# AdamCodd/local-hyperDB

Hardware: AMD Instinct MI355X
Metric: queries/sec, N=10M d=384 fp16 top-100 (single-query stream; p50 latency alongside) (higher is better)
Workload: dtype f16; 1 GPU; N=10000000 d=384 fp16 Q=1 cosine_similarity top-100, row-sharded x1; rows_per_gpu=10000000, accumulate=f32, exchange=none

## Files before the change

### local-hyperdb_amd/csrc/hdb_api.hip

```cpp
#include "hdb_common.h"
#include "hdb_quant.h"
#include "hdb_ws.h"
#include "hdb_plan.h"
#include "../../include/hyperdb_hip.h"
#include <string>
#include <cmath>
#include <cstring>
#include <cstdio>
#include <algorithm>
#include <vector>
#include <chrono>
#include <atomic>

static thread_local std::string g_err;
static int fail(int code, const std::string& msg) { g_err = msg; return code; }
#define HIP_TRY(expr)                                                                              \
    do {                                                                                           \
        hipError_t e_ = (expr);                                                                    \
        if (e_ != hipSuccess)                                                                      \
            return fail(HDB_ERR_HIP, std::string(#expr) + ": " + hipGetErrorString(e_));           \
    } while (0)
#define LAUNCH_TRY(expr)                                                                           \
    do {                                                                                           \
        int e_ = (expr);                                                                           \
        if (e_ != 0) return fail(HDB_ERR_HIP, std::string(#expr) + ": " + hipGetErrorString((hipError_t)e_)); \
    } while (0)

struct hdb_index {
    const void* V = nullptr;
    int64_t n = 0;
    int32_t d = 0;
    int dtype = HDB_F32;
    int device = 0;
    int64_t row_base = 0;
    float* inv_norm = nullptr;
    float* sqnorm = nullptr;
    int64_t cache_rows = 0;
    int* nan_flag = nullptr;
    hipStream_t build_stream = nullptr;
    uint32_t* bits = nullptr;
    int64_t bits_npad = 0;
    int W = 0;
    bool bits_valid = false;
    int64_t bits_done = 0;
    float* pscale = nullptr;
    int64_t pscale_rows = 0;
    bool pscale_valid = false;
    int64_t pscale_done = 0;
    const float* bias = nullptr;
    const uint8_t* mask = nullptr;
    const int64_t* rows = nullptr;
    int64_t subset_m = 0;
    float* mbias = nullptr;
    int64_t mbias_rows = 0;
    char* fctl = nullptr;
    uint32_t fused_epoch = 0;
    char* bctl = nullptr;
    char* rec = nullptr;
    size_t rec_bytes = 0;
    int qmode = HDB_QUANT_NONE;
    int8_t* qcodes = nullptr;
    float* qaux = nullptr;
    int64_t q_rows = 0;
    int32_t qP = 0;
    int* qstat = nullptr;
    uint8_t* pnib = nullptr;
    uint32_t* pbit = nullptr;
    float* prec = nullptr;
    int32_t pU = 0;
    bool plane_declined = false;
    bool qauto = false;
    bool qauto_declined = false;
    char* ws = nullptr;
    size_t ws_bytes = 0;
    hdb_options opt;
    int flags_host = -1;
    TopkStats st;
    int64_t st_host_direct = 0;
    const uint32_t* qb_cnt = nullptr;
    int qb_cnt_n = 0;
    int64_t ht_pre_ns = 0, ht_launch_ns = 0, ht_wait_ns = 0, ht_calls = 0;
    std::chrono::steady_clock::time_point ht_l0, ht_l1;
    int64_t ht_attr_ns = 0;
    int64_t profile = 0;
    std::vector<hipEvent_t> ev_pool;
    size_t ev_used = 0;
};

static int ensure_ws(hdb_index* ix, size_t bytes) {
    if (bytes <= ix->ws_bytes) return HDB_OK;
    if (ix->ws) { HIP_TRY(hipDeviceSynchronize()); HIP_TRY(hipFree(ix->ws)); ix->ws = nullptr; ix->ws_bytes = 0; }
    bytes = align_up(bytes + (bytes >> 2), 1 << 20);
    HIP_TRY(hipMalloc((void**)&ix->ws, bytes));
    ix->ws_bytes = bytes;
    return HDB_OK;
}
template <typename WS, typename... Ext>
static int ws_lay(hdb_index* ix, WS& w, Ext... ext) {
    const int rc = ensure_ws(ix, ws_bytes_for<WS>(ext...));
    if (rc) return rc;
    Bump b(ix->ws, ix->ws_bytes);
    w.lay(b, ext...);
    if (b.off > b.cap) return fail(HDB_ERR_NOMEM, "workspace: a layout ran past the size it reported");
    return HDB_OK;
}

extern "C" int hdb_version(void) { return 103; }
extern "C" const char* hdb_last_error(void) { return g_err.c_str(); }

static int build_caches(hdb_index* ix, hipStream_t st) {
    if (ix->n > ix->cache_rows) {
        if (ix->inv_norm) { HIP_TRY(hipDeviceSynchronize()); HIP_TRY(hipFree(ix->inv_norm)); HIP_TRY(hipFree(ix->sqnorm)); }
        const int64_t rows = ix->n + ix->n / 4 + 64;
        HIP_TRY(hipMalloc((void**)&ix->inv_norm, rows * sizeof(float)));
        HIP_TRY(hipMalloc((void**)&ix->sqnorm, rows * sizeof(float)));
        ix->cache_rows = rows;
    }
    HIP_TRY(hipMemsetAsync(ix->nan_flag, 0, sizeof(int), st));
    if (ix->n > 0) LAUNCH_TRY(hdb_launch_rownorm(ix->V, ix->n, ix->d, ix->dtype, ix->inv_norm, ix->sqnorm, ix->nan_flag, st));
    ix->flags_host = -1;
    ix->bits_valid = false; ix->bits_done = 0;
    ix->pscale_valid = false; ix->pscale_done = 0;
    ix->build_stream = st;
    return HDB_OK;
}

static double quant_gamma(int d) {
    const double u = std::ldexp(1.0, -24), m = (double)(d + 8) * u;
    return m / (1.0 - m) * (1.0 + std::ldexp(1.0, -20));
}
static double quant_gamma_m(int d) { return (double)(d + 8) * std::ldexp(1.0, -22); }
static double quant_gamma_rows(int d) { return std::max(quant_gamma(d), quant_gamma_m(d)); }
static size_t quant_elem(const hdb_index* ix) { return (size_t)hdb_elem_bytes(ix->dtype); }
#define HDB_QSTAT_WORDS 4
static hipError_t qstat_alloc(hdb_index* ix, hipStream_t st) {
    if (ix->qstat) return hipSuccess;
    const hipError_t e = hipMalloc((void**)&ix->qstat, HDB_QSTAT_WORDS * sizeof(int));
    if (e != hipSuccess) { ix->qstat = nullptr; return e; }
    return hipMemsetAsync(ix->qstat, 0, HDB_QSTAT_WORDS * sizeof(int), st);
}
static void plane_free(hdb_index* ix) {
    if (ix->pnib) (void)hipFree(ix->pnib);
    if (ix->pbit) (void)hipFree(ix->pbit);
    if (ix->prec) (void)hipFree(ix->prec);
    ix->pnib = nullptr; ix->pbit = nullptr; ix->prec = nullptr;
}
static void quant_free(hdb_index* ix) {
    if (ix->qcodes) (void)hipFree(ix->qcodes);
    if (ix->qaux) (void)hipFree(ix->qaux);
    ix->qcodes = nullptr; ix->qaux = nullptr; ix->q_rows = 0;
    plane_free(ix);
}
static size_t plane_row_bytes(int P) { return (size_t)hdb_quant_plane_units(P) * 20 + 16; }
static bool plane_alloc(hdb_index* ix, int64_t rows, uint8_t** nib, uint32_t** bit, float** rec) {
    const size_t U = (size_t)hdb_quant_plane_units(ix->qP);
    *nib = nullptr; *bit = nullptr; *rec = nullptr;
    if (hipMalloc((void**)nib, (size_t)rows * U * 16) == hipSuccess && hipMalloc((void**)bit, (size_t)rows * U * 4) == hipSuccess &&
        hipMalloc((void**)rec, (size_t)rows * 16) == hipSuccess) return true;
    (void)hipGetLastError();
    if (*nib) (void)hipFree(*nib);
    if (*bit) (void)hipFree(*bit);
    if (*rec) (void)hipFree(*rec);
    *nib = nullptr; *bit = nullptr; *rec = nullptr;
    return false;
}
static int plane_rows(hdb_index* ix, int64_t row0, int64_t m, hipStream_t st) {
    if (!plane_possible(ix->d) || ix->plane_declined) return HDB_OK;
    if (!ix->pnib && !plane_wanted(ix->d, ix->opt)) return HDB_OK;
    if (!ix->pnib) {
        size_t free_b = 0, total_b = 0;
        if (hipMemGetInfo(&free_b, &total_b) != hipSuccess) { (void)hipGetLastError(); ix->plane_declined = true; return HDB_OK; }
        if (free_b < (size_t)ix->q_rows * plane_row_bytes(ix->qP) + ((size_t)1 << 30)) { ix->plane_declined = true; return HDB_OK; }
        if (!plane_alloc(ix, ix->q_rows, &ix->pnib, &ix->pbit, &ix->prec)) { ix->plane_declined = true; return HDB_OK; }
        ix->pU = hdb_quant_plane_units(ix->qP);
        m = row0 + m; row0 = 0;
    }
    LAUNCH_TRY(hdb_launch_quant_plane_rows(ix->qcodes, ix->qaux, row0, m, ix->d, ix->qP, ix->pnib, ix->pbit, ix->prec, st));
    return HDB_OK;
}
static int quant_reserve(hdb_index* ix, int64_t need, int64_t keep, hipStream_t st, bool tight = false) {
    if (need <= ix->q_rows && ix->qcodes) return HDB_OK;
    const int64_t rows = tight ? need + 64 : need + need / 2 + 64;
    int8_t* c2 = nullptr; float* a2 = nullptr;
    HIP_TRY(hipMalloc((void**)&c2, (size_t)rows * ix->qP));
    hipError_t e = hipMalloc((void**)&a2, (size_t)rows * 3 * sizeof(float));
    if (e != hipSuccess) { (void)hipFree(c2); return fail(HDB_ERR_NOMEM, std::string("hdb_index_quantize: ") + hipGetErrorString(e)); }
    if (keep > 0 && ix->qcodes) {
        HIP_TRY(hipMemcpyAsync(c2, ix->qcodes, (size_t)keep * ix->qP, hipMemcpyDeviceToDevice, st));
        HIP_TRY(hipMemcpyAsync(a2, ix->qaux, (size_t)keep * 3 * sizeof(float), hipMemcpyDeviceToDevice, st));
    }
    HIP_TRY(hipStreamSynchronize(st));
    quant_free(ix);
    ix->qcodes = c2; ix->qaux = a2; ix->q_rows = rows;
    return HDB_OK;
}
static int quant_rows(hdb_index* ix, int64_t row0, int64_t m, hipStream_t st) {
    if (m <= 0) return HDB_OK;
    const char* src = (const char*)ix->V + (size_t)row0 * ix->d * quant_elem(ix);
    LAUNCH_TRY(hdb_launch_quant_rows(src, m, ix->d, ix->dtype, ix->qP, ix->qcodes + (size_t)row0 * ix->qP, ix->qaux + (size_t)row0 * 3,
                                     ix->nan_flag, quant_gamma_rows(ix->d), st));
    return plane_rows(ix, row0, m, st);
}

extern "C" int hdb_index_quantize(hdb_index* ix, int mode, void* stream) {
    if (!ix) return fail(HDB_ERR_ARG, "hdb_index_quantize: null index");
    if (mode != HDB_QUANT_NONE && mode != HDB_QUANT_I8) return fail(HDB_ERR_ARG, "hdb_index_quantize: mode must be HDB_QUANT_NONE or HDB_QUANT_I8");
    HIP_TRY(hipSetDevice(ix->device));
    hipStream_t st = (hipStream_t)stream;
    if (mode == HDB_QUANT_NONE) {
        if (ix->qcodes) HIP_TRY(hipStreamSynchronize(st));
        quant_free(ix);
        ix->qmode = HDB_QUANT_NONE;
        ix->qauto = false;
        ix->opt.auto_quant = 0;
        return HDB_OK;
    }
    if (ix->dtype == HDB_BF16) return fail(HDB_ERR_UNSUPPORTED, "hdb_index_quantize: bfloat16 (bf16) matrices have no int8 shadow");
    if (ix->dtype != HDB_F16 && ix->dtype != HDB_F32) return fail(HDB_ERR_UNSUPPORTED, "hdb_index_quantize: only float16 / float32 matrices have an int8 shadow");
    HIP_TRY(qstat_alloc(ix, st));
    ix->qP = (int32_t)align_up((size_t)ix->d, 16);
    ix->plane_declined = false;
    int rc = quant_reserve(ix, std::max<int64_t>(ix->n, 1), 0, st);
    if (rc) return rc;
    rc = quant_rows(ix, 0, ix->n, st);
    if (rc) return rc;
    ix->qmode = HDB_QUANT_I8;
    ix->qauto = false;
    ix->build_stream = st;
    return HDB_OK;
}

static bool quant_auto_build(hdb_index* ix, size_t ws_need, hipStream_t st) {
    if (ix->qauto_declined) return false;
    const int32_t P = (int32_t)align_up((size_t)ix->d, 16);
    const size_t shadow = (size_t)(ix->n + 64) * ((size_t)P + 12);
    size_t free_b = 0, total_b = 0;
    if (hipMemGetInfo(&free_b, &total_b) != hipSuccess) { (void)hipGetLastError(); ix->qauto_declined = true; return false; }
    const size_t ws_grow = ws_need > ix->ws_bytes ? ws_need + (ws_need >> 2) + ((size_t)1 << 20) : 0;
    if (free_b < shadow + ws_grow + ((size_t)1 << 30)) { ix->qauto_declined = true; return false; }
    const size_t plane = plane_possible(ix->d) ? (size_t)(ix->n + 64) * plane_row_bytes(P) : 0;
    ix->plane_declined = plane_wanted(ix->d, ix->opt) && free_b < shadow + plane + ws_grow + ((size_t)1 << 30);
    if (qstat_alloc(ix, st) != hipSuccess && !ix->qstat) { (void)hipGetLastError(); ix->qauto_declined = true; return false; }
    ix->qP = P;
    if (quant_reserve(ix, std::max<int64_t>(ix->n, 1), 0, st, true) != HDB_OK || quant_rows(ix, 0, ix->n, st) != HDB_OK) {
        (void)hipGetLastError();
        quant_free(ix);
        ix->qauto_declined = true;
        return false;
    }
    ix->qmode = HDB_QUANT_I8;
    ix->qauto = true;
    return true;
}

extern "C" int hdb_index_create(hdb_index** out, const void* dev_V, int64_t n, int32_t d, int dtype, int device,
                                int64_t row_base, void* stream) {
    if (!out) return fail(HDB_ERR_ARG, "hdb_index_create: out is null");
    if (n < 0 || d <= 0) return fail(HDB_ERR_ARG, "hdb_index_create: need n >= 0 and d > 0");
    if (n > 0 && !dev_V) return fail(HDB_ERR_ARG, "hdb_index_create: matrix pointer is null");
    if (dtype != HDB_F16 && dtype != HDB_F32 && dtype != HDB_F64 && dtype != HDB_BF16) return fail(HDB_ERR_ARG, "hdb_index_create: dtype must be f16/f32/f64/bf16");
    if (n >= ((int64_t)1 << 32) - 1) return fail(HDB_ERR_ARG, "hdb_index_create: at most 2^32-2 rows per shard");
    if ((int64_t)d * 8 > 60 * 1024) return fail(HDB_ERR_ARG, "hdb_index_create: d too large for the query LDS tile");
    HIP_TRY(hipSetDevice(device));
    hdb_index* ix = new hdb_index();
    ix->V = dev_V; ix->n = n; ix->d = d; ix->dtype = dtype; ix->device = device; ix->row_base = row_base;
    hipError_t e = hipMalloc((void**)&ix->nan_flag, sizeof(int));
    if (e != hipSuccess) { delete ix; return fail(HDB_ERR_HIP, std::string("hipMalloc: ") + hipGetErrorString(e)); }
    int rc = build_caches(ix, (hipStream_t)stream);
    if (rc != HDB_OK) { hdb_index_destroy(ix); return rc; }
    *out = ix;
    return HDB_OK;
}

extern "C" int hdb_index_update(hdb_index* ix, const void* dev_V, int64_t n, void* stream) {
    if (!ix) return fail(HDB_ERR_ARG, "hdb_index_update: null index");
    if (n < 0 || (n > 0 && !dev_V)) return fail(HDB_ERR_ARG, "hdb_index_update: bad matrix");
    if (n >= ((int64_t)1 << 32) - 1) return fail(HDB_ERR_ARG, "hdb_index_update: at most 2^32-2 rows per shard");
    HIP_TRY(hipSetDevice(ix->device));
    ix->V = dev_V; ix->n = n;
    ix->bias = nullptr; ix->mask = nullptr; ix->rows = nullptr; ix->subset_m = 0;
    ix->qauto_declined = false;
    ix->plane_declined = false;
    int rc = build_caches(ix, (hipStream_t)stream);
    if (rc == HDB_OK && ix->qmode == HDB_QUANT_I8) {
        rc = quant_reserve(ix, std::max<int64_t>(n, 1), 0, (hipStream_t)stream);
        if (rc == HDB_OK) rc = quant_rows(ix, 0, n, (hipStream_t)stream);
    }
    return rc;
}

extern "C" int hdb_index_rebase(hdb_index* ix, const void* dev_V) {
    if (!ix) return fail(HDB_ERR_ARG, "hdb_index_rebase: null index");
    if (ix->n > 0 && !dev_V) return fail(HDB_ERR_ARG, "hdb_index_rebase: matrix pointer is null");
    ix->V = dev_V;
    return HDB_OK;
}

extern "C" int hdb_index_set_row_base(hdb_index* ix, int64_t row_base) {
    if (!ix) return fail(HDB_ERR_ARG, "hdb_index_set_row_base: null index");
    if (row_base < 0) return fail(HDB_ERR_ARG, "hdb_index_set_row_base: row_base must be >= 0");
    ix->row_base = row_base;
    return HDB_OK;
}

extern "C" int hdb_index_extend(hdb_index* ix, int64_t new_n, void* stream) {
    if (!ix) return fail(HDB_ERR_ARG, "hdb_index_extend: null index");
    if (new_n < ix->n) return fail(HDB_ERR_ARG, "hdb_index_extend: new_n must not shrink the matrix (use hdb_index_update)");
    if (new_n >= ((int64_t)1 << 32) - 1) return fail(HDB_ERR_ARG, "hdb_index_extend: at most 2^32-2 rows per shard");
    if (new_n == ix->n) return HDB_OK;
    if (!ix->V) return fail(HDB_ERR_ARG, "hdb_index_extend: no matrix registered");
    HIP_TRY(hipSetDevice(ix->device));
    hipStream_t st = (hipStream_t)stream;
    const int64_t old_n = ix->n;
    if (new_n > ix->cache_rows) {
        const int64_t rows = new_n + new_n / 2 + 64;
        float *inv2 = nullptr, *sq2 = nullptr;
        HIP_TRY(hipMalloc((void**)&inv2, rows * sizeof(float)));
        HIP_TRY(hipMalloc((void**)&sq2, rows * sizeof(float)));
        if (old_n > 0) {
            HIP_TRY(hipMemcpyAsync(inv2, ix->inv_norm, old_n * sizeof(float), hipMemcpyDeviceToDevice, st));
            HIP_TRY(hipMemcpyAsync(sq2, ix->sqnorm, old_n * sizeof(float), hipMemcpyDeviceToDevice, st));
        }
        HIP_TRY(hipStreamSynchronize(st));
        if (ix->inv_norm) { HIP_TRY(hipFree(ix->inv_norm)); HIP_TRY(hipFree(ix->sqnorm)); }
        ix->inv_norm = inv2; ix->sqnorm = sq2; ix->cache_rows = rows;
    }
    const size_t elem = (size_t)hdb_elem_bytes(ix->dtype);
    const char* tail = (const char*)ix->V + (size_t)old_n * ix->d * elem;
    LAUNCH_TRY(hdb_launch_rownorm(tail, new_n - old_n, ix->d, ix->dtype, ix->inv_norm + old_n, ix->sqnorm + old_n, ix->nan_flag, st));
    ix->n = new_n;
    if (ix->qmode == HDB_QUANT_I8) {
        int rc = quant_reserve(ix, new_n, old_n, st);
        if (rc == HDB_OK) rc = quant_rows(ix, old_n, new_n - old_n, st);
        if (rc) return rc;
    }
    ix->flags_host = -1;
    ix->bits_valid = false;
    ix->pscale_valid = false;
    ix->bias = nullptr; ix->mask = nullptr;
    ix->rows = nullptr; ix->subset_m = 0;
    ix->build_stream = st;
    return HDB_OK;
}

extern "C" int hdb_index_gather(hdb_index* ix, const int64_t* dev_rows, int64_t m, void* dev_V_out, void* stream) {
    if (!ix) return fail(HDB_ERR_ARG, "hdb_index_gather: null index");
    if (m < 0 || m > ix->n) return fail(HDB_ERR_ARG, "hdb_index_gather: m must be in [0, n]");
    if (m > 0 && (!dev_rows || !dev_V_out)) return fail(HDB_ERR_ARG, "hdb_index_gather: null argument");
    if (m > 0 && dev_V_out == ix->V) return fail(HDB_ERR_ARG, "hdb_index_gather: the gather is out of place");
    HIP_TRY(hipSetDevice(ix->device));
    hipStream_t st = (hipStream_t)stream;
    const size_t elem = (size_t)hdb_elem_bytes(ix->dtype);
    float *inv2 = nullptr, *sq2 = nullptr;
    const int64_t rows = m + m / 4 + 64;
    HIP_TRY(hipMalloc((void**)&inv2, rows * sizeof(float)));
    HIP_TRY(hipMalloc((void**)&sq2, rows * sizeof(float)));
    HIP_TRY(hipMemsetAsync(ix->nan_flag, 0, sizeof(int), st));
    int rc = hdb_launch_gather_rows(ix->V, dev_rows, m, (int)(ix->d * elem), dev_V_out, ix->inv_norm, ix->sqnorm, inv2, sq2,
                                    ix->nan_flag, st);
    int8_t* qc2 = nullptr; float* qa2 = nullptr;
    if (rc == 0 && ix->qmode == HDB_QUANT_I8) {
        rc = (int)hipMalloc((void**)&qc2, (size_t)rows * ix->qP);
        if (rc == 0) rc = (int)hipMalloc((void**)&qa2, (size_t)rows * 3 * sizeof(float));
        if (rc == 0) rc = hdb_launch_quant_gather(ix->qcodes, ix->qaux, dev_rows, m, ix->qP, qc2, qa2, st);
    }
    if (rc == 0) rc = (int)hipStreamSynchronize(st);
    if (rc != 0) {
        (void)hipFree(inv2); (void)hipFree(sq2);
        if (qc2) (void)hipFree(qc2);
        if (qa2) (void)hipFree(qa2);
        return fail(HDB_ERR_HIP, std::string("hdb_index_gather: ") + hipGetErrorString((hipError_t)rc));
    }
    if (ix->qmode == HDB_QUANT_I8) { quant_free(ix); ix->qcodes = qc2; ix->qaux = qa2; ix->q_rows = rows; }
    if (ix->inv_norm) { (void)hipFree(ix->inv_norm); (void)hipFree(ix->sqnorm); }
    ix->inv_norm = inv2; ix->sqnorm = sq2; ix->cache_rows = rows;
    ix->V = dev_V_out; ix->n = m;
    if (ix->qmode == HDB_QUANT_I8) {
        const int rcp = plane_rows(ix, 0, m, st);
        if (rcp != HDB_OK) return rcp;
    }
    ix->flags_host = -1;
    ix->bits_valid = false; ix->pscale_valid = false; ix->bits_done = 0; ix->pscale_done = 0;
    ix->bias = nullptr; ix->mask = nullptr; ix->rows = nullptr; ix->subset_m = 0;
    ix->build_stream = st;
    return HDB_OK;
}

extern "C" void hdb_index_destroy(hdb_index* ix) {
    if (!ix) return;
    (void)hipSetDevice(ix->device);
    (void)hipDeviceSynchronize();
    if (ix->inv_norm) (void)hipFree(ix->inv_norm);
    if (ix->sqnorm) (void)hipFree(ix->sqnorm);
    if (ix->nan_flag) (void)hipFree(ix->nan_flag);
    if (ix->bits) (void)hipFree(ix->bits);
    if (ix->pscale) (void)hipFree(ix->pscale);
    if (ix->mbias) (void)hipFree(ix->mbias);
    if (ix->fctl) (void)hipFree(ix->fctl);
    if (ix->bctl) (void)hipFree(ix->bctl);
    if (ix->ws) (void)hipFree(ix->ws);
    if (ix->rec) (void)hipFree(ix->rec);
    quant_free(ix);
    if (ix->qstat) (void)hipFree(ix->qstat);
    for (hipEvent_t e : ix->ev_pool) (void)hipEventDestroy(e);
    delete ix;
}

extern "C" int hdb_index_has_nan(hdb_index* ix, int* out_flag) {
    if (!ix || !out_flag) return fail(HDB_ERR_ARG, "hdb_index_has_nan: null argument");
    HIP_TRY(hipSetDevice(ix->device));
    int h = 0;
    HIP_TRY(hipMemcpyAsync(&h, ix->nan_flag, sizeof(int), hipMemcpyDeviceToHost, ix->build_stream));
    HIP_TRY(hipStreamSynchronize(ix->build_stream));
    ix->flags_host = h;
    *out_flag = h & 1;
    return HDB_OK;
}
static int matrix_is_finite(hdb_index* ix, bool* out) {
    if (ix->flags_host < 0) { int f = 0; int rc = hdb_index_has_nan(ix, &f); if (rc != HDB_OK) return rc; }
    *out = ix->flags_host == 0;
    return HDB_OK;
}

extern "C" int hdb_index_set_bias(hdb_index* ix, const float* dev_bias) {
    if (!ix) return fail(HDB_ERR_ARG, "hdb_index_set_bias: null index");
    ix->bias = dev_bias;
    return HDB_OK;
}

extern "C" int hdb_index_set_row_mask(hdb_index* ix, const uint8_t* dev_mask) {
    if (!ix) return fail(HDB_ERR_ARG, "hdb_index_set_row_mask: null index");
    ix->mask = dev_mask;
    ix->rows = nullptr; ix->subset_m = 0;
    return HDB_OK;
}

extern "C" int hdb_index_set_row_subset(hdb_index* ix, const uint8_t* dev_mask, const int64_t* dev_rows, int64_t m) {
    if (!ix) return fail(HDB_ERR_ARG, "hdb_index_set_row_subset: null index");
    if (dev_rows && !dev_mask) return fail(HDB_ERR_ARG, "hdb_index_set_row_subset: a row list needs its mask");
    if (dev_rows && (m < 1 || m > ix->n)) return fail(HDB_ERR_ARG, "hdb_index_set_row_subset: m must be in [1, n]");
    ix->mask = dev_mask;
    ix->rows = dev_rows; ix->subset_m = dev_rows ? m : 0;
    return HDB_OK;
}

extern "C" int hdb_set_option(hdb_index* ix, const char* name, int64_t value) {
    if (!ix || !name) return fail(HDB_ERR_ARG, "hdb_set_option: null argument");
    if (!strcmp(name, "max_blocks")) ix->opt.max_blocks = value;
    else if (!strcmp(name, "force_exact")) ix->opt.force_exact = value;
    else if (!strcmp(name, "sample_target")) ix->opt.sample_target = value;
    else if (!strcmp(name, "mfma_min_q")) ix->opt.mfma_min_q = value;
    else if (!strcmp(name, "use_mfma")) ix->opt.use_mfma = value;
    else if (!strcmp(name, "exact_bytes")) ix->opt.exact_bytes = std::max<int64_t>(1 << 20, value);
    else if (!strcmp(name, "finalize_threads")) { if (value == 256 || value == 512 || value == 1024) ix->opt.finalize_threads = value; }
    else if (!strcmp(name, "mfma_variant")) { if (value == 16 || value == 32 || value == 64) ix->opt.mfma_variant = value; }
    else if (!strcmp(name, "host_direct")) ix->opt.host_direct = value;
    else if (!strcmp(name, "use_fused")) ix->opt.use_fused = value;
    else if (!strcmp(name, "use_batch1")) ix->opt.use_batch1 = value;
    else if (!strcmp(name, "use_local")) ix->opt.use_local = value;
    else if (!strcmp(name, "local_max_q")) ix->opt.local_max_q = value;
    else if (!strcmp(name, "local_max_tiles")) ix->opt.local_max_tiles = std::max<int64_t>(1, value);
    else if (!strcmp(name, "local_small")) ix->opt.local_small = value;
    else if (!strcmp(name, "local_m")) ix->opt.local_m = std::max<int64_t>(0, std::min<int64_t>(value, 64));
    else if (!strcmp(name, "use_l1_tile")) ix->opt.use_l1_tile = value;
    else if (!strcmp(name, "l1_packed")) ix->opt.l1_packed = value;
    else if (!strcmp(name, "host_poll")) ix->opt.host_poll = value;
    else if (!strcmp(name, "dyn_tiles")) ix->opt.dyn_tiles = value;
    else if (!strcmp(name, "dyn_min_mb")) ix->opt.dyn_min_mb = std::max<int64_t>(0, value);
    else if (!strcmp(name, "dyn_heavy")) ix->opt.dyn_heavy = value;
    else if (!strcmp(name, "fused_timeout_us")) ix->opt.fused_timeout_us = std::max<int64_t>(1, value);
    else if (!strcmp(name, "bits_fused")) ix->opt.bits_fused = value;
    else if (!strcmp(name, "bits_local")) ix->opt.bits_local = value;
    else if (!strcmp(name, "fused_max_q")) ix->opt.fused_max_q = value;
    else if (!strcmp(name, "f32_min_q")) ix->opt.f32_min_q = value;
    else if (!strcmp(name, "f32_split")) ix->opt.f32_split = value;
    else if (!strcmp(name, "f32_split_min_q")) ix->opt.f32_split_min_q = value;
    else if (!strcmp(name, "bf16_ks_min_q")) ix->opt.bf16_ks_min_q = value;
    else if (!strcmp(name, "bits_max_q")) ix->opt.bits_max_q = value;
    else if (!strcmp(name, "use_quant")) ix->opt.use_quant = value;
    else if (!strcmp(name, "quant_min_n")) ix->opt.quant_min_n = value;
    else if (!strcmp(name, "auto_quant")) ix->opt.auto_quant = value;
    else if (!strcmp(name, "quant_batch_min_n")) ix->opt.quant_batch_min_n = value;
    else if (!strcmp(name, "quant_batch_kernel")) ix->opt.quant_batch_kernel = value ? 1 : 0;
    else if (!strcmp(name, "quant_max_k")) ix->opt.quant_max_k = std::max<int64_t>(1, std::min<int64_t>(value, 128));
    else if (!strcmp(name, "use_plane")) ix->opt.use_plane = value;
    else if (!strcmp(name, "plane_min_n")) ix->opt.plane_min_n = value;
    else if (!strcmp(name, "plane_cap_rows")) ix->opt.plane_cap_rows = std::max<int64_t>(0, value);
    else if (!strcmp(name, "use_subset")) ix->opt.use_subset = value;
    else if (!strcmp(name, "subset_min_n")) ix->opt.subset_min_n = value < 0 ? -1 : value;
    else if (!strcmp(name, "subset_ratio")) ix->opt.subset_ratio = value < 0 ? -1 : std::max<int64_t>(1, value);
    else if (!strcmp(name, "profile")) { ix->profile = value; ix->ev_used = 0; }
    else if (!strcmp(name, "host_timing_reset")) { ix->ht_pre_ns = ix->ht_launch_ns = ix->ht_wait_ns = ix->ht_calls = ix->ht_attr_ns = 0; }
    else return fail(HDB_ERR_ARG, std::string("hdb_set_option: unknown option ") + name);
    return HDB_OK;
}

extern "C" int hdb_get_stat(hdb_index* ix, const char* name, int64_t* value) {
    if (!ix || !name || !value) return fail(HDB_ERR_ARG, "hdb_get_stat: null argument");
    if (!strcmp(name, "sample_rows")) *value = ix->st.sample_rows;
    else if (!strcmp(name, "sample_m")) *value = ix->st.sample_m;
    else if (!strcmp(name, "path")) *value = ix->st.path;
    else if (!strcmp(name, "chunks")) *value = ix->st.chunks;
    else if (!strcmp(name, "mfma")) *value = ix->st.mfma;
    else if (!strcmp(name, "f32_split")) *value = ix->st.f32s;
    else if (!strcmp(name, "host_direct")) *value = ix->st_host_direct;
    else if (!strcmp(name, "fused")) *value = ix->st.fused;
    else if (!strcmp(name, "local")) *value = ix->st.local;
    else if (!strcmp(name, "cand_cap")) *value = HDB_CAND_CAP;
    else if (!strcmp(name, "quant")) *value = ix->st.quant;
    else if (!strcmp(name, "quant_auto")) *value = (ix->qmode == HDB_QUANT_I8 && ix->qauto) ? 1 : 0;
    else if (!strcmp(name, "quant_bytes")) *value = ix->qmode == HDB_QUANT_I8 ? ix->n * (int64_t)(ix->qP + 12) : 0;
    else if (!strcmp(name, "plane")) *value = ix->st.plane;
    else if (!strcmp(name, "subset")) *value = ix->st.subset;
    else if (!strcmp(name, "subset_rows")) *value = ix->subset_m;
    else if (!strcmp(name, "plane_bytes")) *value = (ix->qmode == HDB_QUANT_I8 && ix->pnib) ? ix->n * (int64_t)plane_row_bytes(ix->qP) : 0;
    else if (!strcmp(name, "plane_survivors") || !strcmp(name, "plane_overflows")) {
        int h[HDB_QSTAT_WORDS] = {0, 0, 0, 0};
        if (ix->qstat) {
            HIP_TRY(hipSetDevice(ix->device));
            HIP_TRY(hipDeviceSynchronize());
            HIP_TRY(hipMemcpy(h, ix->qstat, sizeof(h), hipMemcpyDeviceToHost));
        }
        *value = name[6] == 's' ? (ix->st.plane ? (int64_t)(uint32_t)h[1] : 0) : (int64_t)(uint32_t)h[2];
    }
    else if (!strcmp(name, "quant_cands")) {
        int h = 0;
        if (ix->st.quant && ix->qstat) {
            HIP_TRY(hipSetDevice(ix->device));
            HIP_TRY(hipDeviceSynchronize());
            HIP_TRY(hipMemcpy(&h, ix->qstat, sizeof(int), hipMemcpyDeviceToHost));
        }
        *value = h;
    }
    else if (!strcmp(name, "quant_cands_min") || !strcmp(name, "quant_cands_median")) {
        int64_t v = 0;
        if (ix->st.quant && ix->qb_cnt && ix->qb_cnt_n > 0) {
            HIP_TRY(hipSetDevice(ix->device));
            HIP_TRY(hipDeviceSynchronize());
            std::vector<uint32_t> raw((size_t)ix->qb_cnt_n * HDB_CNT_STRIDE), c((size_t)ix->qb_cnt_n);
            HIP_TRY(hipMemcpy(raw.data(), ix->qb_cnt, raw.size() * sizeof(uint32_t), hipMemcpyDeviceToHost));
            for (int q = 0; q < ix->qb_cnt_n; ++q) c[q] = raw[(size_t)q * HDB_CNT_STRIDE];
            std::sort(c.begin(), c.end());
            v = name[13] == 'i' ? c.front() : c[c.size() / 2];
        }
        *value = v;
    }
    else if (!strcmp(name, "n")) *value = ix->n;
    else if (!strcmp(name, "ws_bytes")) *value = (int64_t)ix->ws_bytes;
    else if (!strcmp(name, "scan_launches")) *value = (int64_t)(ix->ev_used / 2);
    else if (!strcmp(name, "host_pre_ns")) *value = ix->ht_pre_ns;
    else if (!strcmp(name, "host_launch_ns")) *value = ix->ht_launch_ns;
    else if (!strcmp(name, "host_wait_ns")) *value = ix->ht_wait_ns;
    else if (!strcmp(name, "host_calls")) *value = ix->ht_calls;
    else if (!strcmp(name, "host_attr_ns")) *value = ix->ht_attr_ns;
    else if (!strcmp(name, "scan_time_ns")) {
        double total_ms = 0.0;
        for (size_t i = 0; i + 1 < ix->ev_used; i += 2) {
            if (hipEventSynchronize(ix->ev_pool[i + 1]) != hipSuccess) return fail(HDB_ERR_HIP, "hipEventSynchronize failed");
            float ms = 0.f;
            if (hipEventElapsedTime(&ms, ix->ev_pool[i], ix->ev_pool[i + 1]) != hipSuccess) return fail(HDB_ERR_HIP, "hipEventElapsedTime failed");
            total_ms += ms;
        }
        *value = (int64_t)(total_ms * 1.0e6);
    }
    else return fail(HDB_ERR_ARG, std::string("hdb_get_stat: unknown stat ") + name);
    return HDB_OK;
}

static void prof_begin(hdb_index* ix, hipStream_t st) {
    if (!ix->profile) return;
    if (ix->ev_used + 2 > ix->ev_pool.size()) {
        if (ix->ev_pool.size() >= 16384) return;
        for (int i = 0; i < 2; ++i) { hipEvent_t e; if (hipEventCreate(&e) != hipSuccess) return; ix->ev_pool.push_back(e); }
    }
    (void)hipEventRecord(ix->ev_pool[ix->ev_used], st);
}
static void prof_end(hdb_index* ix, hipStream_t st) {
    if (!ix->profile || ix->ev_used + 2 > ix->ev_pool.size()) return;
    (void)hipEventRecord(ix->ev_pool[ix->ev_used + 1], st);
    ix->ev_used += 2;
}

static bool metric_ok(int metric) { return metric >= HDB_DOT && metric <= HDB_EUCLIDEAN_DIST; }

static int ensure_pscale(hdb_index* ix, hipStream_t st) {
    if (ix->pscale_valid) return HDB_OK;
    const size_t elem = (size_t)hdb_elem_bytes(ix->dtype);
    int64_t keep = ix->pscale ? std::min(ix->pscale_done, ix->n) : 0;
    if (ix->n > ix->pscale_rows) {
        const int64_t rows = ix->n + ix->n / 4 + 64;
        float* p2 = nullptr;
        HIP_TRY(hipMalloc((void**)&p2, rows * sizeof(float)));
        if (keep > 0) HIP_TRY(hipMemcpyAsync(p2, ix->pscale, keep * sizeof(float), hipMemcpyDeviceToDevice, st));
        if (ix->pscale) { HIP_TRY(hipDeviceSynchronize()); HIP_TRY(hipFree(ix->pscale)); }
        ix->pscale = p2; ix->pscale_rows = rows;
    }
    if (ix->n > keep)
        LAUNCH_TRY(hdb_launch_rowstats((const char*)ix->V + (size_t)keep * ix->d * elem, ix->n - keep, ix->d, ix->dtype, ix->pscale + keep, st));
    ix->pscale_done = ix->n;
    ix->pscale_valid = true;
    return HDB_OK;
}

static int ensure_bits(hdb_index* ix, hipStream_t st) {
    if (ix->bits_valid) return HDB_OK;
    const int W = (ix->d + 31) / 32;
    if (W > 512) return fail(HDB_ERR_UNSUPPORTED, "hamming: d > 16384 not supported");
    const size_t elem = (size_t)hdb_elem_bytes(ix->dtype);
    const int64_t npad = align_up((size_t)std::max<int64_t>(ix->n, 4), 256);
    int64_t keep = (ix->bits && ix->W == W) ? std::min(ix->bits_done, ix->n) : 0;
    if (!ix->bits || ix->bits_npad < npad || ix->W != W) {
        const int64_t cap = align_up((size_t)(npad + npad / 4), 256);
        uint32_t* b2 = nullptr;
        HIP_TRY(hipMalloc((void**)&b2, (size_t)cap * W * sizeof(uint32_t)));
        HIP_TRY(hipMemsetAsync(b2, 0, (size_t)cap * W * sizeof(uint32_t), st));
        if (keep > 0) HIP_TRY(hipMemcpyAsync(b2, ix->bits, (size_t)align_up((size_t)keep, 256) * W * sizeof(uint32_t), hipMemcpyDeviceToDevice, st));
        if (ix->bits) { HIP_TRY(hipDeviceSynchronize()); HIP_TRY(hipFree(ix->bits)); }
        ix->bits = b2; ix->bits_npad = cap; ix->W = W;
    } else if (keep == 0) {
        HIP_TRY(hipMemsetAsync(ix->bits, 0, (size_t)ix->bits_npad * W * sizeof(uint32_t), st));
    }
    if (ix->n > keep)
        LAUNCH_TRY(hdb_launch_signpack((const char*)ix->V + (size_t)keep * ix->d * elem, ix->n - keep, ix->d, ix->dtype, keep, ix->bits, st));
    ix->bits_done = ix->n;
    ix->bits_valid = true;
    return HDB_OK;
}

static void base_args(const hdb_index* ix, ScanArgs& a, const void* Q, int metric) {
    memset(&a, 0, sizeof(a));
    a.V = ix->V; a.n = ix->n; a.d = ix->d; a.Q = Q; a.metric = metric;
    a.inv_norm = ix->inv_norm; a.mask = ix->mask;
    a.tile_stride = 1; a.ntiles = (ix->n + 15) / 16;
    a.cap = HDB_CAND_CAP;
    a.dyn_min_bytes = ix->opt.dyn_min_mb << 20; a.dyn_heavy = (int32_t)ix->opt.dyn_heavy;
}

struct QueryBufs { const float* qinv; const float* qsq; const uint32_t* qbits; const void* q16; const float* qscl; };
static int run_scan(hdb_index* ix, ScanArgs& a, int mode, int cq, const QueryBufs& qb, bool l1tile, bool mfma, hipStream_t st) {
    a.qinv = qb.qinv;
    if (is_bits_metric(a.metric)) {
        LAUNCH_TRY(hdb_launch_hamming(&a, mode, cq, ix->bits, ix->bits_npad, ix->W, qb.qbits, st));
    } else if (l1tile && cq >= 2 && a.tile_stride == 1) {
        ScanArgs al = a; al.dyn_heavy = ix->opt.l1_packed ? 0 : 77;
        LAUNCH_TRY(hdb_launch_l1_tile(&al, ix->dtype, mode, cq, (int)ix->opt.max_blocks, st));
    } else if (mfma) {
        LAUNCH_TRY(hdb_launch_mfma_scan(&a, ix->dtype, mode, cq, qb.q16, ix->sqnorm, qb.qsq, qb.qscl, (int)ix->opt.max_blocks, (int)ix->opt.mfma_variant, st, nullptr));
    } else {
        LAUNCH_TRY(hdb_launch_scan(&a, ix->dtype, mode, cq, (int)ix->opt.max_blocks, st));
    }
    return HDB_OK;
}

extern "C" int hdb_scores(hdb_index* ix, const void* dev_q, int metric, float* dev_out, void* stream) {
    if (!ix || !dev_q || !dev_out) return fail(HDB_ERR_ARG, "hdb_scores: null argument");
    if (!metric_ok(metric)) return fail(HDB_ERR_UNSUPPORTED, "hdb_scores: metric not built");
    if (ix->n == 0) return HDB_OK;
    HIP_TRY(hipSetDevice(ix->device));
    hipStream_t st = (hipStream_t)stream;
    const int W = (ix->d + 31) / 32;
    ScoresWs w;
    int rc = ws_lay(ix, w, ix->d, W);
    if (rc) return rc;
    float* qinv = w.qinv; float* qsq = w.qsq; int* qnan = w.qnan; uint32_t* qbits = w.qbits; void* qc = w.qc;
    LAUNCH_TRY(hdb_launch_qprep(dev_q, 1, ix->d, ix->dtype == HDB_F64, qinv, qsq, qnan, nullptr, nullptr, st));
    if (is_bits_metric(metric)) {
        rc = ensure_bits(ix, st); if (rc) return rc;
        LAUNCH_TRY(hdb_launch_qsign(dev_q, 1, ix->d, ix->dtype == HDB_F64, W, qbits, st));
    }
    ScanArgs a; base_args(ix, a, dev_q, metric);
    if (metric == HDB_PEARSON) {
        rc = ensure_pscale(ix, st); if (rc) return rc;
        LAUNCH_TRY(hdb_launch_qcentre(dev_q, 1, ix->d, ix->dtype == HDB_F64, qc, qinv, st));
        a.Q = qc; a.metric = HDB_COSINE; a.inv_norm = ix->pscale;
    }
    a.mask = nullptr;
    a.raw = 1;
    a.scores = dev_out; a.ld = ix->n;
    QueryBufs qb{qinv, qsq, qbits, nullptr, nullptr};
    return run_scan(ix, a, 0, 1, qb, false, false, st);
}

struct TopkArgs { const void* Q; int32_t nq, k; int metric; int64_t* idx; float* score; int32_t* status; hipStream_t st; };
static TopkFacts topk_facts(const hdb_index* ix) {
    return {ix->n, ix->d, ix->dtype, ix->qmode, ix->qauto, ix->qauto_declined, ix->pnib != nullptr, ix->plane_declined,
            ix->mask != nullptr, ix->bias != nullptr, hdb_cu_count(), ix->subset_m};
}

static int quant_pitch(const hdb_index* ix) { return (int)align_up((size_t)ix->d, 16); }
static size_t quant_ws_bytes(const hdb_index* ix, int nq, uint32_t pl_cap, bool mflavour) {
    return ws_bytes_for<QuantWs>(nq, quant_pitch(ix), (int)ix->d, quant_ld_max(ix->n, ix->d), pl_cap, mflavour);
}
static int quant_ws_lay(hdb_index* ix, QuantWs& w, int nq, uint32_t pl_cap, bool mflavour) {
    return ws_lay(ix, w, nq, quant_pitch(ix), (int)ix->d, quant_ld_max(ix->n, ix->d), pl_cap, mflavour);
}
static size_t quant_batch_ws_bytes(const hdb_index* ix, int cq) {
    return ws_bytes_for<QuantBatchWs>(cq, quant_pitch(ix), (int)ix->d, quant_batch_sample(ix->n).ld_s, quant_batch_wld());
}
static int quant_batch_ws_lay(hdb_index* ix, QuantBatchWs& w, int cq) {
    return ws_lay(ix, w, cq, quant_pitch(ix), (int)ix->d, quant_batch_sample(ix->n).ld_s, quant_batch_wld());
}
static void quant_base_args(const hdb_index* ix, QuantArgs& a, const int8_t* qcodes, const float* qaux, const float* qinv, int metric, int nq) {
    memset(&a, 0, sizeof(a));
    a.codes = ix->qcodes; a.n = ix->n; a.d = ix->d; a.P = ix->qP; a.aux = ix->qaux; a.sqnorm = ix->sqnorm; a.inv_norm = ix->inv_norm;
    a.qcodes = qcodes; a.qaux = qaux; a.qinv = qinv; a.bias = ix->bias; a.mask = ix->mask; a.metric = metric; a.nq = nq;
    a.gamma = (float)quant_gamma(ix->d);
}
static int quant_query_prep(hdb_index* ix, const float* Q, int nq, const QuantWs& w, bool mflavour, int* stat, uint32_t* cnt_init,
                            uint32_t* pl_cnt, hipStream_t st) {
    if (mflavour) {
        LAUNCH_TRY(hdb_launch_quant_qprep_m(Q, nq, ix->d, ix->qP, w.qinv, w.qsq, w.qnan, w.q16, w.qscl, w.qcodes, w.qaux, stat, cnt_init, pl_cnt, st));
    } else {
        LAUNCH_TRY(hdb_launch_qprep(Q, nq, ix->d, false, w.qinv, w.qsq, w.qnan, nullptr, nullptr, st));
        LAUNCH_TRY(hdb_launch_quant_qprep(Q, nq, ix->d, ix->qP, w.qcodes, w.qaux, stat, pl_cnt, st));
    }
    return HDB_OK;
}

static int shadow_prepare(hdb_index* ix, const TopkPlan& p, int nq, hipStream_t st, bool* declined) {
    if (p.build_needed) {
        const size_t ws_need = p.path == HDB_PATH_QUANT ? quant_ws_bytes(ix, nq, 0, true) : quant_batch_ws_bytes(ix, p.cq_max);
        if (!quant_auto_build(ix, ws_need, st)) { *declined = true; return HDB_OK; }
    }
    if (p.plane_wanted && !ix->pnib) {
        const int rc = plane_rows(ix, 0, ix->n, st);
        if (rc) return rc;
        *declined = ix->pnib == nullptr;
    }
    return HDB_OK;
}

static int quant_topk(hdb_index* ix, const TopkArgs& c, const TopkPlan& p) {
    const void* dev_Q = c.Q; const int32_t nq = c.nq, k = c.k; const int metric = c.metric; hipStream_t st = c.st;
    int64_t* dev_idx = c.idx; float* dev_score = c.score; int32_t* dev_status = c.status;
    const uint32_t kk = p.kk; const bool mflavour = p.mflavour, use_pl = p.plane_wanted;
    const int64_t n = ix->n;
    const uint32_t m = 16;
    const QuantSample sp = p.qs;
    QuantWs w;
    int rc = quant_ws_lay(ix, w, nq, (nq == 1 && ix->pnib) ? p.pl_cap : 0, mflavour);
    if (rc) return rc;
    const uint32_t pl_cap = p.pl_cap;
    uint32_t* pl_cnt = use_pl ? reinterpret_cast<uint32_t*>(ix->qstat) + 1 : nullptr;
    const size_t crow = (size_t)nq * HDB_CAND_CAP;
    const int nsub = p.nsub;
    rc = quant_query_prep(ix, (const float*)dev_Q, nq, w, mflavour, ix->qstat, nsub ? w.cnt : nullptr, pl_cnt, st);
    if (rc) return rc;
    QuantArgs a; quant_base_args(ix, a, w.qcodes, w.qaux, w.qinv, metric, nq);
    a.ntiles = sp.s_tiles; a.tile_stride = sp.s_stride; a.scores = w.sbuf; a.ld = sp.ld_s;
    a.wmax = w.wmax; a.nsub = nsub; a.thr_out = w.thr;
    LAUNCH_TRY(hdb_launch_quant_scan(&a, 0, (int)ix->opt.max_blocks, st));
    if (!nsub) LAUNCH_TRY(hdb_launch_sample_thr(w.sbuf, sp.s_rows, sp.ld_s, nq, m, w.thr, w.cnt, nullptr, st));
    a.ntiles = (n + 15) / 16; a.tile_stride = 1; a.scores = nullptr; a.ld = 0;
    a.thr = w.thr; a.cnt = w.cnt; a.cand = w.cand; a.cap = HDB_CAND_CAP;
    prof_begin(ix, st);
    if (use_pl) {
        a.pl_nib = ix->pnib; a.pl_bit = ix->pbit; a.pl_rec = ix->prec; a.pl_units = ix->pU;
        a.pl_list = w.pl_list; a.pl_cnt = pl_cnt; a.pl_cap = pl_cap;
        LAUNCH_TRY(hdb_launch_quant_plane_scan(&a, 0, (int)ix->opt.max_blocks, st));
        a.nsub = 0; a.wmax = nullptr;
        LAUNCH_TRY(hdb_launch_quant_scan_one(&a, 1, (int)ix->opt.max_blocks, st));
    } else {
        LAUNCH_TRY(hdb_launch_quant_scan(&a, 1, (int)ix->opt.max_blocks, st));
    }
    prof_end(ix, st);
    if (mflavour) {
        const bool has_bias = ix->bias != nullptr || ix->mask != nullptr;
        LAUNCH_TRY(hdb_launch_quant_cgather(ix->V, ix->d * 2, ix->inv_norm, ix->bias, ix->mask, w.cand, w.cnt, HDB_CAND_CAP, nq, w.G,
                                            metric == HDB_COSINE ? w.ginv : nullptr, has_bias ? w.gbias : nullptr, st));
        ScanArgs s; memset(&s, 0, sizeof(s));
        s.V = w.G; s.n = (int64_t)crow; s.d = ix->d; s.Q = dev_Q; s.metric = metric; s.inv_norm = w.ginv; s.qinv = w.qinv;
        s.bias = has_bias ? w.gbias : nullptr; s.mask = nullptr; s.nq = nq;
        s.tile_stride = 1; s.ntiles = (int64_t)crow / hdb_mfma_tile_rows(ix->dtype, ix->d); s.cap = HDB_CAND_CAP;
        s.scores = w.gsc; s.ld = (int64_t)crow;
        LAUNCH_TRY(hdb_launch_mfma_scan(&s, ix->dtype, 0, nq, w.q16, w.ginv, w.qsq, w.qscl, (int)ix->opt.max_blocks, (int)ix->opt.mfma_variant, st, nullptr));
    } else {
        LAUNCH_TRY(hdb_launch_quant_rescore(ix->V, ix->d, ix->dtype, (const float*)dev_Q, nq, metric, ix->inv_norm, w.qinv, ix->bias, ix->mask,
                                            w.cand, w.cnt, HDB_CAND_CAP, st));
    }
    LAUNCH_TRY(hdb_launch_quant_finalize(w.cand, w.cnt, HDB_CAND_CAP, nq, (uint32_t)k, kk, ix->row_base, dev_idx, dev_score, dev_status, w.qnan,
                                         w.qaux, w.thr, ix->qstat, mflavour ? w.cand : nullptr, w.gsc, (int64_t)crow, st));
    return HDB_OK;
}

extern "C" int hdb_debug_quant_bounds(hdb_index* ix, const float* dev_q, int metric, float* dev_hi, float* dev_hi5, void* stream) {
    if (!ix || !dev_q || !dev_hi || !dev_hi5) return fail(HDB_ERR_ARG, "hdb_debug_quant_bounds: null argument");
    if (metric != HDB_DOT && metric != HDB_COSINE) return fail(HDB_ERR_ARG, "hdb_debug_quant_bounds: dot or cosine");
    if (ix->qmode != HDB_QUANT_I8 || !ix->pnib || ix->n < 1) return fail(HDB_ERR_UNSUPPORTED, "hdb_debug_quant_bounds: the index has no 5-bit plane");
    HIP_TRY(hipSetDevice(ix->device));
    hipStream_t st = (hipStream_t)stream;
    QuantWs w;
    int rc = quant_ws_lay(ix, w, 1, plane_list_cap(ix->opt, ix->n), true);
    if (rc) return rc;
    rc = quant_query_prep(ix, dev_q, 1, w, ix->qauto, nullptr, nullptr, nullptr, st);
    if (rc) return rc;
    QuantArgs a; quant_base_args(ix, a, w.qcodes, w.qaux, w.qinv, metric, 1);
    a.ntiles = (ix->n + 15) / 16; a.tile_stride = 1;
    a.pl_nib = ix->pnib; a.pl_bit = ix->pbit; a.pl_rec = ix->prec; a.pl_units = ix->pU;
    a.dbg = dev_hi;
    LAUNCH_TRY(hdb_launch_quant_scan_one(&a, 2, (int)ix->opt.max_blocks, st));
    a.dbg = dev_hi5;
    LAUNCH_TRY(hdb_launch_quant_plane_scan(&a, 1, (int)ix->opt.max_blocks, st));
    return HDB_OK;
}

static int quant_batch_topk(hdb_index* ix, const TopkArgs& c, const TopkPlan& p) {
    const void* dev_Q = c.Q; const int32_t nq = c.nq, k = c.k; const int metric = c.metric; hipStream_t st = c.st;
    int64_t* dev_idx = c.idx; float* dev_score = c.score; int32_t* dev_status = c.status;
    const uint32_t kk = p.kk;
    const int64_t n = ix->n;
    const int P = ix->qP;
    const uint32_t m = HDB_QB_SAMPLE_M;
    const QuantSample sp = p.qs;
    const int64_t s_tiles = sp.s_tiles, s_stride = sp.s_stride, s_rows = sp.s_rows, ld_s = sp.ld_s;
    const int cq_max = p.cq_max;
    QuantBatchWs w;
    const int rc = quant_batch_ws_lay(ix, w, cq_max);
    if (rc) return rc;
    const int64_t wld = quant_batch_wld();
    float* const qinv = w.qinv; float* const qsq = w.qsq; int* const qnan = w.qnan; float* const qscl = w.qscl;
    int8_t* const qcodes = w.qcodes; float* const qaux = w.qaux; float* const thr = w.thr; uint32_t* const cnt = w.cnt;
    unsigned long long* const cand = w.cand; void* const q16 = w.q16; float* const wbuf = w.wbuf;
    for (int q0 = 0; q0 < nq; q0 += cq_max) {
        const int cq = std::min(cq_max, nq - q0);
        const float* Qc = (const float*)dev_Q + (size_t)q0 * ix->d;
        LAUNCH_TRY(hdb_launch_quant_qprep_m(Qc, cq, ix->d, P, qinv, qsq, qnan, q16, qscl, qcodes, qaux, q0 == 0 ? ix->qstat : nullptr, cnt, nullptr, st));
        QuantArgs a; quant_base_args(ix, a, qcodes, qaux, qinv, metric, cq);
        a.thr = thr; a.cnt = cnt; a.cand = cand; a.cap = HDB_CAND_CAP;
        if (p.qb_int8) {
            a.ntiles = s_tiles; a.tile_stride = s_stride;
            const int sblocks = hdb_qb_scan_blocks(s_tiles, cq, hdb_cu_count(), (int)ix->opt.max_blocks);
            LAUNCH_TRY(hdb_launch_qb_scan(&a, 0, wbuf, wld, (int)ix->opt.max_blocks, st));
            LAUNCH_TRY(hdb_launch_qb_thr(wbuf, hdb_qb_slots(sblocks, cq), wld, cq, m, thr, st));
            a.ntiles = (n + 15) / 16; a.tile_stride = 1;
            prof_begin(ix, st);
            LAUNCH_TRY(hdb_launch_qb_scan(&a, 1, nullptr, 0, (int)ix->opt.max_blocks, st));
            prof_end(ix, st);
        } else {
            for (int g0 = 0; g0 < cq; g0 += 4) {
                QuantArgs g = a;
                g.nq = std::min(4, cq - g0);
                g.qcodes = qcodes + (size_t)g0 * P; g.qaux = qaux + (size_t)g0 * HDB_QQ_WORDS; g.qinv = qinv + g0;
                g.thr = thr + g0; g.cnt = cnt + (size_t)g0 * HDB_CNT_STRIDE; g.cand = cand + (size_t)g0 * HDB_CAND_CAP;
                g.ntiles = s_tiles; g.tile_stride = s_stride; g.scores = wbuf; g.ld = ld_s;
                LAUNCH_TRY(hdb_launch_quant_scan(&g, 0, (int)ix->opt.max_blocks, st));
                LAUNCH_TRY(hdb_launch_qb_thr(wbuf, s_rows, ld_s, g.nq, m, thr + g0, st));
                g.ntiles = (n + 15) / 16; g.tile_stride = 1; g.scores = nullptr; g.ld = 0;
                prof_begin(ix, st);
                LAUNCH_TRY(hdb_launch_quant_scan(&g, 1, (int)ix->opt.max_blocks, st));
                prof_end(ix, st);
            }
        }
        LAUNCH_TRY(hdb_launch_qb_rescore(ix->V, ix->d, q16, qscl, qinv, ix->inv_norm, ix->bias, ix->mask, metric, cand, cnt, HDB_CAND_CAP, cq, st));
        LAUNCH_TRY(hdb_launch_quant_finalize(cand, cnt, HDB_CAND_CAP, cq, (uint32_t)k, kk, ix->row_base, dev_idx + (int64_t)q0 * k,
                                             dev_score + (int64_t)q0 * k, dev_status + q0, qnan, qaux, thr, ix->qstat, nullptr, nullptr, 0, st));
    }
    ix->qb_cnt = cnt; ix->qb_cnt_n = nq - (nq - 1) / cq_max * cq_max;
    return HDB_OK;
}

static uint32_t next_epoch(hdb_index* ix) {
    ix->fused_epoch = (ix->fused_epoch + 1) & 0x7FFFFFFFu;
    if (ix->fused_epoch == 0) ix->fused_epoch = 1;
    return ix->fused_epoch;
}
static uint32_t timeout_ticks(const hdb_index* ix) { return (uint32_t)std::min<int64_t>(ix->opt.fused_timeout_us * 100, 0x7FFFFFFF); }
static int ensure_ctl(char** ctl, size_t bytes) {
    if (*ctl) return HDB_OK;
    HIP_TRY(hipMalloc((void**)ctl, bytes));
    HIP_TRY(hipMemset(*ctl, 0, bytes));
    return HDB_OK;
}

static int run_empty(const TopkArgs& c) {
    HIP_TRY(hipMemsetAsync(c.idx, 0xFF, (size_t)c.nq * c.k * sizeof(int64_t), c.st));
    HIP_TRY(hipMemsetAsync(c.score, 0xFF, (size_t)c.nq * c.k * sizeof(float), c.st));
    if (c.status) HIP_TRY(hipMemsetAsync(c.status, 0, (size_t)c.nq * sizeof(int32_t), c.st));
    return HDB_OK;
}

struct TopkEnv {
    TopkWs w; size_t sort_temp;
    const void* Qeff; int metric_eff;
    const float* bias_eff; const uint8_t* mask_eff;
};
static int topk_begin(hdb_index* ix, const TopkArgs& c, const TopkPlan& p, TopkEnv& e) {
    hipStream_t st = c.st;
    const bool f64 = ix->dtype == HDB_F64;
    const int64_t n = ix->n;
    e.sort_temp = 0;
    if (p.sort_n > 0) LAUNCH_TRY(hdb_sort_temp_bytes(p.sort_n, &e.sort_temp));
    TopkWs& w = e.w;
    int rc = ws_lay(ix, w, (int)c.nq, (int)ix->d, p.W, p.cq_max, p.ld_scores, p.ld_ks, p.sort_n, e.sort_temp);
    if (rc) return rc;
    if (p.prep)
        LAUNCH_TRY(hdb_launch_qprep2(c.Q, c.nq, ix->d, f64, w.qinv, w.qsq, w.qnan, p.q16_in_prep ? w.q16 : nullptr, w.qscl, p.fold_small ? w.thr : nullptr,
                                     p.fold_small ? w.cnt : nullptr, (p.fold_small && p.bits) ? w.qbits : nullptr, p.W, st));
    if (p.bits) {
        rc = ensure_bits(ix, st); if (rc) return rc;
        if (p.prep && !p.fold_small) LAUNCH_TRY(hdb_launch_qsign(c.Q, c.nq, ix->d, f64, p.W, w.qbits, st));
    }
    e.Qeff = c.Q; e.metric_eff = c.metric;
    if (p.pearson) {
        rc = ensure_pscale(ix, st); if (rc) return rc;
        if (p.prep) LAUNCH_TRY(hdb_launch_qcentre(c.Q, c.nq, ix->d, f64, w.qc, w.qinv, st));
        e.Qeff = w.qc; e.metric_eff = HDB_COSINE;
    }
    e.bias_eff = ix->bias; e.mask_eff = ix->mask;
    if (p.mask_fold) {
        if (n > ix->mbias_rows) {
            if (ix->mbias) { HIP_TRY(hipDeviceSynchronize()); HIP_TRY(hipFree(ix->mbias)); ix->mbias = nullptr; }
            const int64_t rows = n + n / 4 + 64;
            HIP_TRY(hipMalloc((void**)&ix->mbias, rows * sizeof(float)));
            ix->mbias_rows = rows;
        }
        LAUNCH_TRY(hdb_launch_maskbias(ix->mask, ix->bias, n, ix->mbias, st));
        e.bias_eff = ix->mbias; e.mask_eff = nullptr;
    }
    return HDB_OK;
}

static int run_full_sort(hdb_index* ix, const TopkArgs& c, const TopkPlan& p) {
    TopkEnv e;
    int rc = topk_begin(ix, c, p, e); if (rc) return rc;
    for (int q0 = 0; q0 < c.nq; ++q0) {
        QueryBufs qb{e.w.qinv, e.w.qsq, e.w.qbits, nullptr, nullptr};
        ScanArgs s2; base_args(ix, s2, e.Qeff, e.metric_eff);
        if (p.pearson) s2.inv_norm = ix->pscale;
        s2.q0 = q0; s2.bias = ix->bias; s2.scores = e.w.sc1; s2.ld = p.ld_n;
        rc = run_scan(ix, s2, 0, 1, qb, false, false, c.st); if (rc) return rc;
        LAUNCH_TRY(hdb_launch_full_sort(e.w.sc1, ix->n, c.k, ix->row_base, e.w.work, e.w.temp, e.sort_temp, c.idx + (int64_t)q0 * c.k,
                                        c.score + (int64_t)q0 * c.k, c.st));
    }
    if (c.status) LAUNCH_TRY(hdb_launch_status_nan(e.w.qnan, c.nq, c.status, c.st));
    return HDB_OK;
}

static int run_fused(hdb_index* ix, const TopkArgs& c, const TopkPlan& p) {
    TopkEnv e;
    int rc = topk_begin(ix, c, p, e); if (rc) return rc;
    rc = ensure_ctl(&ix->fctl, hdb_mfma_fused_ctl_bytes()); if (rc) return rc;
    ScanArgs a; base_args(ix, a, c.Q, c.metric);
    a.bias = e.bias_eff; a.mask = nullptr;
    if (c.metric == HDB_EUCLIDEAN) a.inv_norm = ix->sqnorm;
    if (p.pearson) a.inv_norm = ix->pscale;
    a.ntiles = (ix->n + p.tile_rows - 1) / p.tile_rows;
    a.thr = e.w.thr; a.cnt = e.w.cnt; a.cand = e.w.cand; a.nq = c.nq;
    FusedArgs fa; memset(&fa, 0, sizeof(fa));
    fa.Qraw = static_cast<const float*>(c.Q); fa.nq = c.nq;
    fa.s_tiles = p.s_tiles; fa.s_stride = p.s_stride;
    fa.epoch = next_epoch(ix);
    fa.timeout_ticks = timeout_ticks(ix);
    fa.ctl = reinterpret_cast<uint32_t*>(ix->fctl);
    fa.cand = e.w.cand; fa.cap = HDB_CAND_CAP; fa.k = (uint32_t)c.k; fa.kk = p.kk; fa.row_base = ix->row_base;
    fa.idx_out = c.idx; fa.score_out = c.score; fa.status = c.status; fa.thr_out = e.w.thr;
    fa.local = p.local ? 1 : 0; fa.local_slot = p.local_slot; fa.local_m = p.local_m;
    prof_begin(ix, c.st);
    ix->ht_l0 = std::chrono::steady_clock::now();
    LAUNCH_TRY(hdb_launch_mfma_fused(&a, ix->dtype, &fa, (int)ix->opt.max_blocks, c.st));
    ix->ht_l1 = std::chrono::steady_clock::now();
    prof_end(ix, c.st);
    return HDB_OK;
}

static int run_bits1(hdb_index* ix, const TopkArgs& c, const TopkPlan& p) {
    TopkEnv e;
    int rc = topk_begin(ix, c, p, e); if (rc) return rc;
    rc = ensure_ctl(&ix->bctl, hdb_mfma_batch_ctl_bytes(hdb_cu_count())); if (rc) return rc;
    for (int q0 = 0; q0 < c.nq; q0 += 4) {
        const int cq = std::min(4, c.nq - q0);
        BitsArgs ba; memset(&ba, 0, sizeof(ba));
        ba.bits = ix->bits; ba.npad = ix->bits_npad; ba.W = p.W; ba.n = ix->n; ba.d = ix->d;
        ba.Qraw = static_cast<const float*>(c.Q) + (size_t)q0 * ix->d; ba.nq = cq;
        ba.ntiles = (ix->n + 15) / 16; ba.s_tiles = p.s_tiles; ba.s_stride = p.s_stride;
        ba.bias = ix->bias; ba.mask = ix->mask;
        ba.local = p.bits_local;
        ba.epoch = next_epoch(ix);
        ba.timeout_ticks = timeout_ticks(ix);
        ba.ctl = reinterpret_cast<uint32_t*>(ix->bctl);
        ba.cand = e.w.cand; ba.cap = HDB_CAND_CAP; ba.k = (uint32_t)c.k; ba.kk = p.kk; ba.row_base = ix->row_base;
        ba.idx_out = c.idx + (int64_t)q0 * c.k; ba.score_out = c.score + (int64_t)q0 * c.k; ba.status = c.status + q0;
        prof_begin(ix, c.st);
        ix->ht_l0 = std::chrono::steady_clock::now();
        LAUNCH_TRY(hdb_launch_bits_fused(&ba, c.metric == HDB_JACCARD ? 1 : 0, (int)ix->opt.max_blocks, c.st));
        ix->ht_l1 = std::chrono::steady_clock::now();
        prof_end(ix, c.st);
    }
    return HDB_OK;
}

static int run_batch1(hdb_index* ix, const TopkArgs& c, const TopkPlan& p) {
    TopkEnv e;
    int rc = topk_begin(ix, c, p, e); if (rc) return rc;
    rc = ensure_ctl(&ix->bctl, hdb_mfma_batch_ctl_bytes(hdb_cu_count())); if (rc) return rc;
    const size_t qrow = (size_t)ix->d * 4;
    for (int q0 = 0; q0 < c.nq; q0 += p.cq_max) {
        const int cq = std::min(p.cq_max, c.nq - q0);
        ScanArgs a; base_args(ix, a, c.Q, e.metric_eff);
        if (p.pearson) a.inv_norm = ix->pscale;
        a.bias = e.bias_eff; a.mask = nullptr; a.q0 = 0; a.nq = cq; a.f32_split = p.f32s ? 1 : 0;
        a.ntiles = (ix->n + p.tile_rows - 1) / p.tile_rows;
        a.cand = e.w.cand;
        a.tile_ctr = ix->opt.dyn_tiles ? reinterpret_cast<uint32_t*>(ix->bctl) + HDB_BATCH_CTL_TILE : nullptr;
        BatchArgs fa; memset(&fa, 0, sizeof(fa));
        fa.Qraw = static_cast<const char*>(c.Q) + (size_t)q0 * qrow;
        fa.s_tiles = p.s_tiles; fa.s_stride = p.s_stride; fa.centre = p.pearson ? 1 : 0;
        fa.epoch = next_epoch(ix);
        fa.timeout_ticks = timeout_ticks(ix);
        fa.ctl = reinterpret_cast<uint32_t*>(ix->bctl);
        fa.k = (uint32_t)c.k; fa.kk = p.kk; fa.row_base = ix->row_base;
        fa.idx_out = c.idx + (int64_t)q0 * c.k; fa.score_out = c.score + (int64_t)q0 * c.k; fa.status = c.status + q0;
        prof_begin(ix, c.st);
        ix->ht_l0 = std::chrono::steady_clock::now();
        LAUNCH_TRY(hdb_launch_mfma_scan(&a, ix->dtype, 2, cq, nullptr, ix->sqnorm, nullptr, nullptr, (int)ix->opt.max_blocks, (int)ix->opt.mfma_variant, c.st, &fa));
        ix->ht_l1 = std::chrono::steady_clock::now();
        prof_end(ix, c.st);
    }
    return HDB_OK;
}

static int run_pipeline(hdb_index* ix, const TopkArgs& c, const TopkPlan& p) {
    TopkEnv e;
    int rc = topk_begin(ix, c, p, e); if (rc) return rc;
    const void* dev_Q = c.Q; const int32_t nq = c.nq, k = c.k; const int metric = c.metric; hipStream_t st = c.st;
    int64_t* dev_idx = c.idx; float* dev_score = c.score; int32_t* dev_status = c.status;
    const TopkWs& w = e.w;
    float* const qinv = w.qinv; float* const qsq = w.qsq; int* const qnan = w.qnan; float* const qscl = w.qscl;
    uint32_t* const qbits = w.qbits; void* const q16 = w.q16;
    float* const thr = w.thr; uint32_t* const cnt = w.cnt; uint32_t* const tile_ctr = w.tile_ctr; uint32_t* const hist = w.hist;
    uint32_t* const tie_info = w.tie_info; unsigned long long* const cand = w.cand; float* const sbuf = w.sbuf; float* const kbuf = w.kbuf;
    const void* Qeff = e.Qeff; const int metric_eff = e.metric_eff; const float* bias_eff = e.bias_eff; const uint8_t* mask_eff = e.mask_eff;
    const bool small = p.small, exact = p.exact, mfma = p.mfma, f32s = p.f32s, fold_small = p.fold_small, f16_queries = p.f16_queries, is_pearson = p.pearson, q16_in_prep = p.q16_in_prep;
    const int64_t n = p.subset ? ix->subset_m : ix->n, s_tiles = p.s_tiles, s_stride = p.s_stride, s_rows = p.s_rows, ld_s = p.ld_s, ld_n = p.ld_n;
    const uint32_t kk = p.kk, m = p.m; const int cq_max = p.cq_max, tile_rows = p.tile_rows, npass = p.npass;
    bool q16_ready = q16_in_prep;
    for (int q0 = 0; q0 < nq; q0 += cq_max) {
        const int cq = std::min(cq_max, nq - q0);
        if (f16_queries && !q16_ready) { LAUNCH_TRY(hdb_launch_q_to_f16((const float*)Qeff, nq, ix->d, q16, qscl, st)); q16_ready = true; }
        QueryBufs qb{qinv, qsq, qbits, f16_queries ? q16 : Qeff, f16_queries ? qscl : nullptr};
        ScanArgs a; base_args(ix, a, Qeff, metric_eff);
        if (is_pearson) a.inv_norm = ix->pscale;
        a.q0 = q0; a.bias = bias_eff; a.mask = mask_eff; a.f32_split = f32s ? 1 : 0;
        a.thr = thr; a.cnt = cnt; a.cand = cand;
        a.ntiles = (n + tile_rows - 1) / tile_rows;
        if (p.subset) { a.rows = ix->rows; a.m = ix->subset_m; a.mask = nullptr; a.bias = ix->bias; }
        a.ks_partial_out = kbuf; a.ks_ld = ld_n;

        if (small) {
            if (!fold_small) LAUNCH_TRY(hdb_launch_fill_thr(thr, cnt, cq, -INFINITY, st));
            rc = run_scan(ix, a, 1, cq, qb, p.l1tile, mfma, st); if (rc) return rc;
        } else if (!exact) {
            ScanArgs s = a;
            s.ntiles = s_tiles; s.tile_stride = s_stride; s.scores = sbuf; s.ld = ld_s;
            rc = run_scan(ix, s, 0, cq, qb, p.l1tile, mfma, st); if (rc) return rc;
            if (m <= 16) {
                LAUNCH_TRY(hdb_launch_sample_thr(sbuf, s_rows, ld_s, cq, m, thr, cnt, tile_ctr, st));
                if (mfma && ix->opt.dyn_tiles) a.tile_ctr = tile_ctr;
            } else {
                HIP_TRY(hipMemsetAsync(hist, 0, (size_t)cq * 4 * HDB_RADIX_BINS * 4, st));
                for (int ps = 0; ps < 4; ++ps) LAUNCH_TRY(hdb_launch_hist(sbuf, s_rows, ld_s, cq, hist, ps, m, st));
                LAUNCH_TRY(hdb_launch_thr(hist, cq, 4, m, (uint32_t)s_rows, thr, cnt, st));
            }
            prof_begin(ix, st);
            rc = run_scan(ix, a, 1, cq, qb, p.l1tile, mfma, st); if (rc) return rc;
            prof_end(ix, st);
        } else {
            ScanArgs s = a;
            s.scores = sbuf; s.ld = ld_n;
            prof_begin(ix, st);
            rc = run_scan(ix, s, 0, cq, qb, p.l1tile, mfma, st); if (rc) return rc;
            prof_end(ix, st);
            HIP_TRY(hipMemsetAsync(cnt, 0, (size_t)((char*)hist - (char*)cnt) + (size_t)cq * 4 * HDB_RADIX_BINS * 4, st));
            for (int ps = 0; ps < npass; ++ps) LAUNCH_TRY(hdb_launch_hist(sbuf, n, ld_n, cq, hist, ps, kk, st));
            LAUNCH_TRY(hdb_launch_collect(sbuf, n, ld_n, cq, hist, npass, kk, cnt, cand, HDB_CAND_CAP, tie_info, st));
            if (p.subset) LAUNCH_TRY(hdb_launch_list_rows(cand, cnt, HDB_CAND_CAP, cq, ix->rows, ix->subset_m, st));
        }
        if (mfma && metric == HDB_EUCLIDEAN)
            LAUNCH_TRY(hdb_launch_rescore_euclid(cand, cnt, HDB_CAND_CAP, cq, ix->V, ix->dtype, ix->d, (const float*)dev_Q, qsq, q0, ix->bias, st));
        LAUNCH_TRY(hdb_launch_finalize(cand, cnt, HDB_CAND_CAP, cq, (uint32_t)k, kk, ix->row_base,
                                       dev_idx + (int64_t)q0 * k, dev_score + (int64_t)q0 * k,
                                       dev_status ? dev_status + q0 : nullptr, qnan + q0, (int)ix->opt.finalize_threads,
                                       a.f32_split ? HDB_Q_UNDERFLOW : 0, st));
    }
    return HDB_OK;
}

static int topk_impl(hdb_index* ix, const void* dev_Q, int32_t nq, int32_t k, int metric, int64_t* dev_idx,
                     float* dev_score, int32_t* dev_status, void* stream, bool exact) {
    if (!ix || !dev_idx || !dev_score) return fail(HDB_ERR_ARG, "hdb_topk: null argument");
    if (nq < 0 || k < 0) return fail(HDB_ERR_ARG, "hdb_topk: nq and k must be >= 0");
    if (nq == 0 || k == 0) return HDB_OK;
    if (!dev_Q) return fail(HDB_ERR_ARG, "hdb_topk: query pointer is null");
    if (metric == HDB_EUCLIDEAN_DIST || !metric_ok(metric)) return fail(HDB_ERR_UNSUPPORTED, "hdb_topk: metric not built");
    if (metric == HDB_PEARSON && ix->d < 1) return fail(HDB_ERR_ARG, "hdb_topk: pearson needs d >= 1");
    HIP_TRY(hipSetDevice(ix->device));
    const TopkArgs c{dev_Q, nq, k, metric, dev_idx, dev_score, dev_status, (hipStream_t)stream};
    const TopkCall call{nq, k, metric, dev_status != nullptr, exact};
    int frc = HDB_OK;
    auto finite = [&] { bool f = false; if (frc == HDB_OK) frc = matrix_is_finite(ix, &f); return f; };
    TopkPlan p = plan_topk(topk_facts(ix), ix->opt, call, finite);
    if (frc != HDB_OK) return frc;
    if (p.shadow()) {
        bool declined = false;
        const int rc = shadow_prepare(ix, p, nq, c.st, &declined);
        if (rc) return rc;
        if (declined) p = plan_topk(topk_facts(ix), ix->opt, call, finite);
        if (frc != HDB_OK) return frc;
    }
    ix->st = p.stats;
    ix->qb_cnt = nullptr; ix->qb_cnt_n = 0;
    switch (p.path) {
    case HDB_PATH_EMPTY: return run_empty(c);
    case HDB_PATH_QUANT: return quant_topk(ix, c, p);
    case HDB_PATH_QUANT_BATCH: return quant_batch_topk(ix, c, p);
    case HDB_PATH_FUSED: return run_fused(ix, c, p);
    case HDB_PATH_BITS1: return run_bits1(ix, c, p);
    case HDB_PATH_BATCH1: return run_batch1(ix, c, p);
    case HDB_PATH_FULL_SORT: return run_full_sort(ix, c, p);
    case HDB_PATH_PIPELINE: return run_pipeline(ix, c, p);
    }
    return fail(HDB_ERR_ARG, "hdb_topk: no path");
}

extern "C" int hdb_topk(hdb_index* ix, const void* dev_Q, int32_t nq, int32_t k, int metric, int64_t* dev_idx,
                        float* dev_score, int32_t* dev_status, void* stream) {
    return topk_impl(ix, dev_Q, nq, k, metric, dev_idx, dev_score, dev_status, stream, false);
}

static void merge_host_records(const char* const* recs, int32_t parts, int32_t nq, int32_t k, void* out_record) {
    int64_t* oi = reinterpret_cast<int64_t*>(out_record);
    float* os = reinterpret_cast<float*>(static_cast<char*>(out_record) + (int64_t)nq * k * 8);
    int32_t* ost = reinterpret_cast<int32_t*>(static_cast<char*>(out_record) + (int64_t)nq * k * 12);
    std::vector<int32_t> pos((size_t)parts);
    for (int32_t q = 0; q < nq; ++q) {
        int32_t st = 0;
        for (int32_t p = 0; p < parts; ++p) {
            st |= reinterpret_cast<const int32_t*>(recs[p] + (int64_t)nq * k * 12)[q];
            pos[p] = 0;
        }
        for (int32_t i = 0; i < k; ++i) {
            int32_t best = -1; int64_t bi = -1; float bs = 0.f;
            for (int32_t p = 0; p < parts; ++p) {
                if (pos[p] >= k) continue;
                const int64_t ci = reinterpret_cast<const int64_t*>(recs[p])[(int64_t)q * k + pos[p]];
                if (ci < 0) { pos[p] = k; continue; }
                const float cs = reinterpret_cast<const float*>(recs[p] + (int64_t)nq * k * 8)[(int64_t)q * k + pos[p]];
                if (best < 0 || cs > bs || (cs == bs && ci < bi)) { best = p; bi = ci; bs = cs; }
            }
            if (best < 0) { oi[(int64_t)q * k + i] = -1; os[(int64_t)q * k + i] = -INFINITY; }
            else { oi[(int64_t)q * k + i] = bi; os[(int64_t)q * k + i] = bs; ++pos[best]; }
        }
        ost[q] = st;
    }
}

extern "C" int hdb_merge_topk_host(const void* records, int32_t parts, int32_t nq, int32_t k, void* out_record) {
    if (!records || !out_record || parts <= 0 || nq < 0 || k < 0) return fail(HDB_ERR_ARG, "hdb_merge_topk_host: bad argument");
    const int64_t nb = hdb_packed_bytes(nq, k);
    std::vector<const char*> recs((size_t)parts);
    for (int32_t p = 0; p < parts; ++p) recs[p] = static_cast<const char*>(records) + p * nb;
    merge_host_records(recs.data(), parts, nq, k, out_record);
    return HDB_OK;
}

extern "C" int hdb_host_exchange_merge(void* shm, int64_t stride, int32_t world, int32_t rank, uint64_t seq, const void* record,
                                       int32_t nq, int32_t k, void* out_record, double timeout_s) {
    if (!shm || !record || !out_record || world <= 0 || rank < 0 || rank >= world || stride < 64 || nq < 0 || k < 0)
        return fail(HDB_ERR_ARG, "hdb_host_exchange_merge: bad argument");
    const int64_t nb = hdb_packed_bytes(nq, k);
    if (nb + 64 > stride) return fail(HDB_ERR_ARG, "hdb_host_exchange_merge: record larger than a slot");
    char* base = static_cast<char*>(shm) + (int64_t)(seq & 1) * world * stride;
    char* mine = base + (int64_t)rank * stride;
    memcpy(mine + 64, record, (size_t)nb);
    __atomic_store_n(reinterpret_cast<uint64_t*>(mine), seq, __ATOMIC_RELEASE);
    std::vector<const char*> recs((size_t)world);
    const auto t0 = std::chrono::steady_clock::now();
    for (int32_t r = 0; r < world; ++r) {
        const uint64_t* sp = reinterpret_cast<const uint64_t*>(base + (int64_t)r * stride);
        uint32_t spins = 0;
        while (__atomic_load_n(sp, __ATOMIC_ACQUIRE) != seq) {
            __builtin_ia32_pause();
            if ((++spins & 0xFFFFu) == 0 &&
                std::chrono::duration<double>(std::chrono::steady_clock::now() - t0).count() > timeout_s)
                return fail(HDB_ERR_HIP, "hdb_host_exchange_merge: a rank did not publish its record in time");
        }
        recs[r] = base + (int64_t)r * stride + 64;
    }
    merge_host_records(recs.data(), world, nq, k, out_record);
    return HDB_OK;
}

extern "C" int hdb_topk_host(hdb_index* ix, const void* dev_Q, int32_t nq, int32_t k, int metric, void* host_record, void* stream) {
    if (!ix || !host_record) return fail(HDB_ERR_ARG, "hdb_topk_host: null argument");
    if (nq <= 0 || k <= 0) return fail(HDB_ERR_ARG, "hdb_topk_host: nq and k must be positive");
    const auto ht0 = std::chrono::steady_clock::now();
    HIP_TRY(hipSetDevice(ix->device));
    hipStream_t st = (hipStream_t)stream;
    const size_t bytes = (size_t)hdb_packed_bytes(nq, k);
    bool direct = false;
    if (ix->opt.host_direct) {
        hipPointerAttribute_t attr;
        if (hipPointerGetAttributes(&attr, host_record) == hipSuccess) direct = attr.type == hipMemoryTypeHost && attr.devicePointer == host_record;
        else (void)hipGetLastError();
        ix->ht_attr_ns += std::chrono::duration_cast<std::chrono::nanoseconds>(std::chrono::steady_clock::now() - ht0).count();
    }
    ix->st_host_direct = direct ? 1 : 0;
    char* rec = static_cast<char*>(host_record);
    if (!direct) {
        if (bytes > ix->rec_bytes) {
            if (ix->rec) { HIP_TRY(hipDeviceSynchronize()); HIP_TRY(hipFree(ix->rec)); ix->rec = nullptr; }
            HIP_TRY(hipMalloc((void**)&ix->rec, bytes * 2));
            ix->rec_bytes = bytes * 2;
        }
        rec = ix->rec;
    }
    int64_t* d_idx = reinterpret_cast<int64_t*>(rec);
    float* d_sc = reinterpret_cast<float*>(rec + (size_t)nq * k * 8);
    int32_t* d_st = reinterpret_cast<int32_t*>(rec + (size_t)nq * k * 12);
    constexpr int32_t SENTINEL = 0x7FFFFFFF;
    volatile int32_t* poll = reinterpret_cast<volatile int32_t*>(static_cast<char*>(host_record) + (size_t)nq * k * 12);
    if (direct && ix->opt.host_poll) for (int q = 0; q < nq; ++q) poll[q] = SENTINEL;
    ix->ht_l0 = ix->ht_l1 = std::chrono::steady_clock::now();
    int rc = topk_impl(ix, dev_Q, nq, k, metric, d_idx, d_sc, d_st, stream, false);
    if (rc) return rc;
    if (!direct) HIP_TRY(hipMemcpyAsync(host_record, rec, bytes, hipMemcpyDeviceToHost, st));
    bool polled = false;
    if (direct && ix->opt.host_poll && (ix->st.fused || ix->st.path != 3)) {
        const auto t0 = std::chrono::steady_clock::now();
        for (unsigned spins = 0;; ++spins) {
            bool done = true;
            for (int q = 0; q < nq; ++q) done &= poll[q] != SENTINEL;
            if (done) { polled = true; break; }
            if ((spins & 1023) == 1023 && std::chrono::steady_clock::now() - t0 > std::chrono::milliseconds(200)) break;
            __builtin_ia32_pause();
        }
        std::atomic_thread_fence(std::memory_order_acquire);
    }
    if (!polled) HIP_TRY(hipStreamSynchronize(st));
    {
        const auto ht3 = std::chrono::steady_clock::now();
        using ns = std::chrono::nanoseconds;
        ix->ht_pre_ns += std::chrono::duration_cast<ns>(ix->ht_l0 - ht0).count();
        ix->ht_launch_ns += std::chrono::duration_cast<ns>(ix->ht_l1 - ix->ht_l0).count();
        ix->ht_wait_ns += std::chrono::duration_cast<ns>(ht3 - ix->ht_l1).count();
        ix->ht_calls++;
    }
    const int32_t* h_st = reinterpret_cast<const int32_t*>(static_cast<const char*>(host_record) + (size_t)nq * k * 12);
    bool any_bad = false;
    for (int q = 0; q < nq; ++q) any_bad |= (h_st[q] & (HDB_Q_UNDERFLOW | HDB_Q_OVERFLOW)) != 0;
    if (!any_bad) return HDB_OK;
    const size_t qbytes = (size_t)ix->d * (ix->dtype == HDB_F64 ? 8 : 4);
    std::vector<char> bad(nq);
    for (int q = 0; q < nq; ++q) bad[q] = (h_st[q] & (HDB_Q_UNDERFLOW | HDB_Q_OVERFLOW)) != 0;
    const int64_t quant_first = ix->st.quant;
    for (int q = 0; q < nq; ++q) {
        if (!bad[q]) continue;
        rc = topk_impl(ix, static_cast<const char*>(dev_Q) + (size_t)q * qbytes, 1, k, metric, d_idx + (size_t)q * k,
                       d_sc + (size_t)q * k, d_st + q, stream, true);
        if (rc) return rc;
    }
    ix->st.quant = quant_first;
    if (!direct) HIP_TRY(hipMemcpyAsync(host_record, rec, bytes, hipMemcpyDeviceToHost, st));
    HIP_TRY(hipStreamSynchronize(st));
    return HDB_OK;
}

extern "C" int hdb_topk_exact(hdb_index* ix, const void* dev_Q, int32_t nq, int32_t k, int metric, int64_t* dev_idx,
                              float* dev_score, int32_t* dev_status, void* stream) {
    return topk_impl(ix, dev_Q, nq, k, metric, dev_idx, dev_score, dev_status, stream, true);
}

extern "C" int hdb_merge_topk(const int64_t* dev_idx_parts, const float* dev_score_parts, int32_t parts, int32_t nq,
                              int32_t k, int64_t* dev_idx, float* dev_score, int device, void* stream) {
    if (!dev_idx_parts || !dev_score_parts || !dev_idx || !dev_score) return fail(HDB_ERR_ARG, "hdb_merge_topk: null argument");
    if (parts <= 0 || nq < 0 || k < 0) return fail(HDB_ERR_ARG, "hdb_merge_topk: bad sizes");
    if (nq == 0 || k == 0) return HDB_OK;
    if ((int64_t)parts * k > HDB_CAND_CAP) return fail(HDB_ERR_UNSUPPORTED, "hdb_merge_topk: parts*k exceeds 8192");
    HIP_TRY(hipSetDevice(device));
    LAUNCH_TRY(hdb_launch_merge(dev_idx_parts, (int64_t)nq * k * 8, dev_score_parts, (int64_t)nq * k * 4, nullptr, 0, parts, nq,
                                (uint32_t)k, dev_idx, dev_score, nullptr, stream));
    return HDB_OK;
}

extern "C" int64_t hdb_packed_bytes(int32_t nq, int32_t k) {
    const int64_t raw = (int64_t)nq * k * 12 + (int64_t)nq * 4;
    return (raw + 15) / 16 * 16;
}

extern "C" int hdb_merge_topk_packed(const void* dev_gathered, int32_t parts, int32_t nq, int32_t k, int64_t* dev_idx,
                                     float* dev_score, int32_t* dev_status, int device, void* stream) {
    if (!dev_gathered || !dev_idx || !dev_score) return fail(HDB_ERR_ARG, "hdb_merge_topk_packed: null argument");
    if (parts <= 0 || nq < 0 || k < 0) return fail(HDB_ERR_ARG, "hdb_merge_topk_packed: bad sizes");
    if (nq == 0 || k == 0) return HDB_OK;
    if ((int64_t)parts * k > HDB_CAND_CAP) return fail(HDB_ERR_UNSUPPORTED, "hdb_merge_topk_packed: parts*k exceeds 8192");
    HIP_TRY(hipSetDevice(device));
    const int64_t stride = hdb_packed_bytes(nq, k);
    const char* base = (const char*)dev_gathered;
    LAUNCH_TRY(hdb_launch_merge(base, stride, base + (int64_t)nq * k * 8, stride, base + (int64_t)nq * k * 12, stride, parts, nq,
                                (uint32_t)k, dev_idx, dev_score, dev_status, stream));
    return HDB_OK;
}

extern "C" int hdb_recency_bias(const double* dev_ts, int64_t n, double recency_bias, double ts_max, float* dev_out,
                                int device, void* stream) {
    if (n < 0 || (n > 0 && (!dev_ts || !dev_out))) return fail(HDB_ERR_ARG, "hdb_recency_bias: null argument");
    if (n == 0) return HDB_OK;
    HIP_TRY(hipSetDevice(device));
    LAUNCH_TRY(hdb_launch_recency(dev_ts, n, recency_bias, ts_max, dev_out, stream));
    return HDB_OK;
}

extern "C" int hdb_recency_bias_twice(const double* dev_ts, const uint8_t* dev_mask, int64_t n, double recency_bias, double ts_max,
                                      double ts_min, float* dev_out, int device, void* stream) {
    if (n < 0 || (n > 0 && (!dev_ts || !dev_out))) return fail(HDB_ERR_ARG, "hdb_recency_bias_twice: null argument");
    if (n == 0) return HDB_OK;
    HIP_TRY(hipSetDevice(device));
    const double first_max = recency_bias >= 0.0 ? recency_bias * std::exp(-ts_max + ts_max) : recency_bias * std::exp(-ts_max + ts_min);
    LAUNCH_TRY(hdb_launch_recency2(dev_ts, dev_mask, n, recency_bias, ts_max, first_max, dev_out, stream));
    return HDB_OK;
}

#include <thread>
#include <mutex>
#include <condition_variable>

struct hdb_group {
    int parts = 0;
    std::vector<hdb_index*> ix;
    std::vector<hipStream_t> st;
    std::vector<void*> qdev;
    std::vector<size_t> qcap;
    std::vector<char> shared_dev;
    char* gather = nullptr; size_t gather_bytes = 0;
    char* qpin = nullptr; size_t qpin_bytes = 0;
    std::vector<std::thread> th;
    std::mutex mu;
    std::condition_variable cv_job, cv_done;
    std::atomic<uint64_t> job_seq{0};
    std::atomic<int> pending{0};
    std::atomic<bool> stop{false};
    size_t q_bytes = 0;
    int nq = 0, k = 0, metric = 0; size_t stride = 0;
    std::vector<int> rc;
    std::vector<std::string> err;
};

static constexpr long HDB_GROUP_SPIN_US = 200;

static void group_worker(hdb_group* g, int p) {
    (void)hipSetDevice(g->ix[p]->device);
    uint64_t seen = 0;
    for (;;) {
        bool got = false;
        const auto t0 = std::chrono::steady_clock::now();
        for (unsigned spins = 0;; ++spins) {
            if (g->stop.load(std::memory_order_acquire)) return;
            if (g->job_seq.load(std::memory_order_acquire) != seen) { got = true; break; }
            __builtin_ia32_pause();
            if ((spins & 255u) == 255u && std::chrono::steady_clock::now() - t0 > std::chrono::microseconds(HDB_GROUP_SPIN_US)) break;
        }
        if (!got) {
            std::unique_lock<std::mutex> lk(g->mu);
            g->cv_job.wait(lk, [&] { return g->stop.load(std::memory_order_acquire) || g->job_seq.load(std::memory_order_acquire) != seen; });
            if (g->stop.load(std::memory_order_acquire)) return;
        }
        seen = g->job_seq.load(std::memory_order_acquire);
        int rc = HDB_OK;
        std::string msg;
        hdb_index* ix = g->ix[p];
        hipStream_t st = g->st[p];
        if (ix->n > 0) {
            const void* dq = g->qpin;
            if (g->nq > 4) {
                hipError_t e = hipSuccess;
                if (g->q_bytes > g->qcap[p]) {
                    if (g->qdev[p]) { (void)hipStreamSynchronize(st); (void)hipFree(g->qdev[p]); g->qdev[p] = nullptr; g->qcap[p] = 0; }
                    e = hipMalloc(&g->qdev[p], g->q_bytes * 2);
                    if (e == hipSuccess) g->qcap[p] = g->q_bytes * 2;
                }
                if (e == hipSuccess) e = hipMemcpyAsync(g->qdev[p], g->qpin, g->q_bytes, hipMemcpyHostToDevice, st);
                if (e != hipSuccess) { rc = HDB_ERR_HIP; msg = std::string("hdb_group: query upload: ") + hipGetErrorString(e); }
                dq = g->qdev[p];
            }
            if (rc == HDB_OK) {
                const int64_t saved = ix->opt.use_fused;
                if (g->shared_dev[p]) ix->opt.use_fused = 0;
                rc = hdb_topk_host(ix, dq, g->nq, g->k, g->metric, g->gather + (size_t)p * g->stride, st);
                ix->opt.use_fused = saved;
                if (rc != HDB_OK) msg = hdb_last_error();
            }
        } else {
            char* rec = g->gather + (size_t)p * g->stride;
            int64_t* ri = reinterpret_cast<int64_t*>(rec);
            float* rs = reinterpret_cast<float*>(rec + (size_t)g->nq * g->k * 8);
            int32_t* rst = reinterpret_cast<int32_t*>(rec + (size_t)g->nq * g->k * 12);
            for (size_t i = 0; i < (size_t)g->nq * g->k; ++i) { ri[i] = -1; rs[i] = -INFINITY; }
            for (int q = 0; q < g->nq; ++q) rst[q] = 0;
        }
        g->rc[p] = rc; g->err[p] = msg;
        if (g->pending.fetch_sub(1, std::memory_order_acq_rel) == 1) {
            { std::lock_guard<std::mutex> lk(g->mu); }
            g->cv_done.notify_all();
        }
    }
}

extern "C" void hdb_group_destroy(hdb_group* g) {
    if (!g) return;
    g->stop.store(true, std::memory_order_release);
    { std::lock_guard<std::mutex> lk(g->mu); }
    g->cv_job.notify_all();
    for (auto& t : g->th) if (t.joinable()) t.join();
    for (int p = 0; p < (int)g->st.size(); ++p) {
        (void)hipSetDevice(g->ix[p]->device);
        if (g->st[p]) { (void)hipStreamSynchronize(g->st[p]); (void)hipStreamDestroy(g->st[p]); }
        if (p < (int)g->qdev.size() && g->qdev[p]) (void)hipFree(g->qdev[p]);
    }
    if (g->gather) (void)hipHostFree(g->gather);
    if (g->qpin) (void)hipHostFree(g->qpin);
    delete g;
}

extern "C" int hdb_group_create(hdb_group** out, hdb_index* const* shards, int32_t parts) {
    if (!out || !shards) return fail(HDB_ERR_ARG, "hdb_group_create: null argument");
    if (parts < 1 || parts > 64) return fail(HDB_ERR_ARG, "hdb_group_create: 1..64 shards");
    for (int p = 0; p < parts; ++p) {
        if (!shards[p]) return fail(HDB_ERR_ARG, "hdb_group_create: null shard");
        if (shards[p]->d != shards[0]->d || shards[p]->dtype != shards[0]->dtype)
            return fail(HDB_ERR_ARG, "hdb_group_create: shards must share d and dtype");
    }
    hdb_group* g = new hdb_group();
    g->parts = parts;
    g->ix.assign(shards, shards + parts);
    g->st.assign(parts, nullptr); g->qdev.assign(parts, nullptr); g->qcap.assign(parts, 0);
    g->rc.assign(parts, 0); g->err.assign(parts, std::string());
    g->shared_dev.assign(parts, 0);
    for (int p = 0; p < parts; ++p)
        for (int r = 0; r < parts; ++r)
            if (r != p && g->ix[r]->device == g->ix[p]->device) g->shared_dev[p] = 1;
    hipError_t e = hipSuccess;
    for (int p = 0; p < parts && e == hipSuccess; ++p) {
        e = hipSetDevice(g->ix[p]->device);
        if (e == hipSuccess) e = hipStreamCreateWithFlags(&g->st[p], hipStreamNonBlocking);
    }
    if (e != hipSuccess) { hdb_group_destroy(g); return fail(HDB_ERR_HIP, std::string("hdb_group_create: ") + hipGetErrorString(e)); }
    for (int p = 0; p < parts; ++p) g->th.emplace_back(group_worker, g, p);
    *out = g;
    return HDB_OK;
}

static int group_pinned(char** buf, size_t* have, size_t need) {
    if (need <= *have) return HDB_OK;
    if (*buf) { HIP_TRY(hipHostFree(*buf)); *buf = nullptr; *have = 0; }
    need = align_up(need * 2, 4096);
    HIP_TRY(hipHostMalloc((void**)buf, need, hipHostMallocPortable | hipHostMallocMapped));
    *have = need;
    return HDB_OK;
}

extern "C" int hdb_group_topk_host(hdb_group* g, const void* host_Q, int32_t nq, int32_t k, int metric, void* host_record) {
    if (!g || !host_Q || !host_record) return fail(HDB_ERR_ARG, "hdb_group_topk_host: null argument");
    if (nq <= 0 || k <= 0) return fail(HDB_ERR_ARG, "hdb_group_topk_host: nq and k must be positive");
    const size_t bytes = (size_t)hdb_packed_bytes(nq, k);
    const size_t qelem = g->ix[0]->dtype == HDB_F64 ? 8 : 4;
    const size_t q_bytes = (size_t)g->ix[0]->d * qelem * nq;
    if (bytes * g->parts > g->gather_bytes || q_bytes > g->qpin_bytes) {
        HIP_TRY(hipSetDevice(g->ix[0]->device));
        int rc = group_pinned(&g->gather, &g->gather_bytes, bytes * g->parts); if (rc) return rc;
        rc = group_pinned(&g->qpin, &g->qpin_bytes, q_bytes); if (rc) return rc;
    }
    memcpy(g->qpin, host_Q, q_bytes);
    g->q_bytes = q_bytes; g->nq = nq; g->k = k; g->metric = metric; g->stride = bytes;
    g->pending.store(g->parts, std::memory_order_release);
    g->job_seq.fetch_add(1, std::memory_order_acq_rel);
    { std::lock_guard<std::mutex> lk(g->mu); }
    g->cv_job.notify_all();
    {
        const auto t0 = std::chrono::steady_clock::now();
        bool done = false;
        for (unsigned spins = 0;; ++spins) {
            if (g->pending.load(std::memory_order_acquire) == 0) { done = true; break; }
            __builtin_ia32_pause();
            if ((spins & 255u) == 255u && std::chrono::steady_clock::now() - t0 > std::chrono::milliseconds(5)) break;
        }
        if (!done) {
            std::unique_lock<std::mutex> lk(g->mu);
            g->cv_done.wait(lk, [&] { return g->pending.load(std::memory_order_acquire) == 0; });
        }
    }
    for (int p = 0; p < g->parts; ++p)
        if (g->rc[p] != HDB_OK) return fail(g->rc[p], "shard " + std::to_string(p) + ": " + g->err[p]);
    std::vector<const char*> recs((size_t)g->parts);
    for (int p = 0; p < g->parts; ++p) recs[p] = g->gather + (size_t)p * g->stride;
    merge_host_records(recs.data(), g->parts, nq, k, host_record);
    return HDB_OK;
}
```

### local-hyperdb_amd/csrc/hdb_launch.h

```cpp
#pragma once
#include <stddef.h>
#include <stdint.h>

struct ScanArgs;
struct FusedArgs;
struct BatchArgs;
struct BitsArgs;
struct QuantArgs;

#define HDB_ANYD_DECL(name) int name(const ScanArgs* args, int dpad, int mode, int nq_launch, const void* q, const float* sqnorm, \
                                     const float* qsq, const float* qscl, int blocks, void* stream)
#define HDB_GEOM_DECL(name) int name(const ScanArgs* args, int mode, int nq_launch, const void* q16, const float* sqnorm, \
                                     const float* qsq, const float* qscl, int blocks, int variant, void* stream, const BatchArgs* f)

extern "C" {
int hdb_launch_scan(const ScanArgs* args, int dtype, int mode, int nq_launch, int max_blocks, void* stream);
int hdb_launch_list_rows(unsigned long long* cand, const uint32_t* cnt, uint32_t cap, int nq, const int64_t* rows, int64_t m, void* stream);
int hdb_launch_rownorm(const void* V, int64_t n, int d, int dtype, float* inv_norm, float* sqnorm, int* nan_flag, void* stream);
int hdb_launch_qprep(const void* Q, int nq, int d, bool f64, float* qinv, float* qsq, int* qnan, void* q16, float* qscl, void* stream);
int hdb_launch_qprep2(const void* Q, int nq, int d, bool f64, float* qinv, float* qsq, int* qnan, void* q16, float* qscl,
                      float* thr_init, uint32_t* cnt_init, uint32_t* qbits, int W, void* stream);
int hdb_launch_signpack(const void* V, int64_t n, int d, int dtype, int64_t row0, uint32_t* bits, void* stream);
int hdb_launch_qsign(const void* Q, int nq, int d, bool f64, int W, uint32_t* qbits, void* stream);
int hdb_launch_hamming(const ScanArgs* args, int mode, int nq_launch, const uint32_t* bits, int64_t npad, int W,
                       const uint32_t* qbits, void* stream);
int hdb_launch_maskbias(const uint8_t* mask, const float* bias, int64_t n, float* out, void* stream);
int hdb_launch_recency(const double* ts, int64_t n, double rb, double ts_max, float* out, void* stream);
int hdb_launch_recency2(const double* ts, const uint8_t* mask, int64_t n, double rb, double ts_max, double first_max, float* out, void* stream);
int hdb_launch_rowstats(const void* V, int64_t n, int d, int dtype, float* pscale, void* stream);
int hdb_launch_qcentre(const void* Q, int nq, int d, bool f64, void* Qc, float* qscale, void* stream);

int hdb_launch_hist(const float* scores, int64_t n, int64_t ld, int nq, uint32_t* hist, int pass, uint32_t k, void* stream);
int hdb_launch_thr(const uint32_t* hist, int nq, int npass, uint32_t m, uint32_t sample_n, float* thr, uint32_t* cnt, void* stream);
int hdb_launch_fill_thr(float* thr, uint32_t* cnt, int nq, float v, void* stream);
int hdb_launch_sample_thr(const float* scores, int64_t n, int64_t ld, int nq, uint32_t m, float* thr, uint32_t* cnt, uint32_t* tile_ctr, void* stream);
int hdb_launch_collect(const float* scores, int64_t n, int64_t ld, int nq, const uint32_t* hist, int npass, uint32_t k, uint32_t* cnt,
                       unsigned long long* cand, uint32_t cap, uint32_t* tie_info, void* stream);
int hdb_launch_finalize(const unsigned long long* cand, const uint32_t* cnt, uint32_t cap, int nq, uint32_t k, uint32_t kk,
                        int64_t row_base, int64_t* idx_out, float* score_out, int32_t* status, const int* qnan, int threads, int inf_status, void* stream);
int hdb_launch_status_nan(const int* qnan, int nq, int32_t* status, void* stream);
int hdb_launch_merge(const void* idx_base, int64_t idx_stride, const void* score_base, int64_t score_stride,
                     const void* status_base, int64_t status_stride, int parts, int nq, uint32_t k, int64_t* idx_out,
                     float* score_out, int32_t* status_out, void* stream);

int hdb_sort_temp_bytes(int64_t n, size_t* bytes);
int hdb_launch_full_sort(const float* scores, int64_t n, int64_t k, int64_t row_base, uint32_t* work, void* temp, size_t temp_bytes,
                         int64_t* idx_out, float* score_out, void* stream);
int hdb_launch_gather_rows(const void* V, const int64_t* rows, int64_t m, int row_bytes, void* out, const float* inv_in,
                           const float* sq_in, float* inv_out, float* sq_out, int* nan_flag, void* stream);

size_t hdb_mfma_batch_ctl_bytes(int wgs);
int hdb_launch_mfma_scan(const ScanArgs* args, int dtype, int mode, int nq_launch, const void* q16, const float* sqnorm,
                         const float* qsq, const float* qscl, int max_blocks, int variant, void* stream, const BatchArgs* f);
int hdb_launch_q_to_f16(const float* Q, int nq, int d, void* q16, float* qscl, void* stream);
int hdb_launch_rescore_euclid(unsigned long long* cand, const uint32_t* cnt, uint32_t cap, int nq_launch, const void* V, int dtype, int d,
                              const float* Q, const float* qsq, int q0, const float* bias, void* stream);
HDB_GEOM_DECL(hdb_launch_mfma_scan_f16_d384);
HDB_GEOM_DECL(hdb_launch_mfma_scan_f16_narrow);
HDB_GEOM_DECL(hdb_launch_mfma_scan_f16_mid);
HDB_GEOM_DECL(hdb_launch_mfma_scan_f16_1k);
int hdb_launch_mfma_scan_f16_wide(const ScanArgs* args, int mode, int nq_launch, const void* q16, const float* sqnorm,
                                  const float* qsq, const float* qscl, int blocks, void* stream, const BatchArgs* f);
int hdb_launch_mfma_scan_f16_qt2(const ScanArgs* args, int mode, int nq_launch, const void* q16, const float* sqnorm,
                                 const float* qsq, const float* qscl, int blocks, void* stream, const BatchArgs* f);
int hdb_launch_mfma_scan_f32(const ScanArgs* args, int mode, int nq_launch, const void* q, const float* sqnorm,
                             const float* qsq, int blocks, void* stream, const BatchArgs* f);
int hdb_launch_mfma_scan_f32_wide(const ScanArgs* args, int mode, int nq_launch, const void* q, const float* sqnorm,
                                  const float* qsq, int blocks, void* stream, const BatchArgs* f);
int hdb_launch_mfma_scan_f32s(const ScanArgs* args, int mode, int nq_launch, const void* q, const float* sqnorm,
                              const float* qsq, int blocks, void* stream, const BatchArgs* f);
int hdb_launch_mfma_scan_f32s_wide(const ScanArgs* args, int mode, int nq_launch, const void* q, const float* sqnorm,
                                   const float* qsq, int blocks, void* stream, const BatchArgs* f);
int hdb_launch_mfma_scan_bf16(const ScanArgs* args, int mode, int nq_launch, const void* q, const float* sqnorm,
                              const float* qsq, int blocks, void* stream);
int hdb_launch_mfma_scan_bf16_wide(const ScanArgs* args, int mode, int nq_launch, const void* q, const float* sqnorm,
                                   const float* qsq, int blocks, void* stream);
int hdb_launch_mfma_ksplit(const ScanArgs* args, int dtype, int mode, int nq_launch, const void* q, const float* sqnorm,
                           const float* qsq, const float* qscl, int blocks, void* stream);
int hdb_launch_mfma_kslice_f32s(const ScanArgs* a, int dslice, int mode, int nq_launch, const void* q, const float* sqnorm,
                                const float* qsq, int blocks, void* stream);
int hdb_launch_mfma_kslice_bf16(const ScanArgs* a, int dslice, int mode, int nq_launch, const void* q, const float* sqnorm,
                                const float* qsq, int blocks, void* stream);
int hdb_launch_mfma_kslice_bf16_wide(const ScanArgs* a, int dslice, int mode, int nq_launch, const void* q, const float* sqnorm,
                                     const float* qsq, int blocks, void* stream);
HDB_ANYD_DECL(hdb_launch_mfma_anyd_a); HDB_ANYD_DECL(hdb_launch_mfma_anyd_b);
HDB_ANYD_DECL(hdb_launch_mfma_anyd_c); HDB_ANYD_DECL(hdb_launch_mfma_anyd_d);
HDB_ANYD_DECL(hdb_launch_mfma_anyd_e); HDB_ANYD_DECL(hdb_launch_mfma_anyd_f);

size_t hdb_mfma_fused_ctl_bytes(void);
int hdb_launch_mfma_fused(const ScanArgs* args, int dtype, const FusedArgs* fa, int max_blocks, void* stream);
int hdb_launch_mfma_fused_wide(const ScanArgs* args, const FusedArgs* fa, int blocks, void* stream);
int hdb_launch_bits_fused(const BitsArgs* args, int jaccard, int max_blocks, void* stream);
int hdb_launch_l1_tile(const ScanArgs* args, int dtype, int mode, int nq_launch, int max_blocks, void* stream);

int hdb_launch_quant_rows(const void* V, int64_t n, int d, int dtype, int P, int8_t* codes, float* aux, int* nan_flag, double gamma,
                          void* stream);
int hdb_launch_quant_gather(const int8_t* codes, const float* aux, const int64_t* rows, int64_t m, int P, int8_t* codes_out,
                            float* aux_out, void* stream);
int hdb_launch_quant_qprep(const float* Q, int nq, int d, int P, int8_t* qcodes, float* qaux, int* stat, uint32_t* pl_cnt, void* stream);
int hdb_launch_quant_qprep_m(const float* Q, int nq, int d, int P, float* qinv, float* qsq, int* qnan, void* q16, float* qscl,
                             int8_t* qcodes, float* qaux, int* stat, uint32_t* cnt_init, uint32_t* pl_cnt, void* stream);
int hdb_launch_quant_plane_rows(const int8_t* codes, const float* aux, int64_t row0, int64_t m, int d, int P, uint8_t* nib, uint32_t* bitw,
                                float* rec, void* stream);
int hdb_launch_quant_plane_scan(const QuantArgs* args, int dbg, int max_blocks, void* stream);
int hdb_launch_quant_scan(const QuantArgs* args, int mode, int max_blocks, void* stream);
int hdb_launch_quant_scan_one(const QuantArgs* args, int mode, int max_blocks, void* stream);
int hdb_launch_quant_rescore(const void* V, int d, int dtype, const float* Q, int nq, int metric, const float* inv_norm,
                             const float* qinv, const float* bias, const uint8_t* mask, unsigned long long* cand,
                             const uint32_t* cnt, uint32_t cap, void* stream);
int hdb_launch_quant_cgather(const void* V, int row_bytes, const float* inv_norm, const float* bias, const uint8_t* mask,
                             const unsigned long long* cand, const uint32_t* cnt, uint32_t cap, int nq, void* G, float* ginv, float* gbias,
                             void* stream);
int hdb_launch_quant_finalize(const unsigned long long* cand, const uint32_t* cnt, uint32_t cap, int nq, uint32_t k, uint32_t kk,
                              int64_t row_base, int64_t* idx_out, float* score_out, int32_t* status, const int* qnan,
                              const float* qaux, const float* thr, int* stat, unsigned long long* cand_rw, const float* sc, int64_t ld,
                              void* stream);

int hdb_launch_qb_scan(const QuantArgs* args, int mode, float* wstat, int64_t wld, int max_blocks, void* stream);
int hdb_launch_qb_thr(const float* vals, int64_t n, int64_t ld, int nq, uint32_t m, float* thr, void* stream);
int hdb_launch_qb_rescore(const void* V, int d, const void* q16, const float* qscl, const float* qinv, const float* inv_norm,
                          const float* bias, const uint8_t* mask, int metric, unsigned long long* cand, const uint32_t* cnt,
                          uint32_t cap, int nq, void* stream);
}
```

### local-hyperdb_amd/csrc/hdb_quant.h

```cpp
#pragma once
#include <stdint.h>

#define HDB_QROW_S 0
#define HDB_QROW_E 1
#define HDB_QROW_T 2
#define HDB_QQ_S 0
#define HDB_QQ_N 1
#define HDB_QQ_D 2
#define HDB_QQ_SQ 3
#define HDB_QQ_BAD 4
#define HDB_QQ_CN 5
#define HDB_QQ_CS 6
#define HDB_QQ_WORDS 8

struct QuantArgs {
    const int8_t* codes;
    int64_t n;
    int32_t d;
    int32_t P;
    const float* aux;
    const float* sqnorm;
    const float* inv_norm;
    const int8_t* qcodes;
    const float* qaux;
    const float* qinv;
    const float* bias;
    const uint8_t* mask;
    int32_t metric;
    int32_t nq;
    float gamma;
    int64_t ntiles;
    int64_t tile_stride;
    float* scores; int64_t ld;
    const float* thr; uint32_t* cnt; unsigned long long* cand; uint32_t cap;
    uint32_t* wmax; int32_t nsub; float* thr_out;
    const uint8_t* pl_nib; const uint32_t* pl_bit; const float* pl_rec; int32_t pl_units;
    uint32_t* pl_list; uint32_t* pl_cnt; uint32_t pl_cap;
    float* dbg;
};
#define HDB_QUANT_NSUB_MAX 4096
```

### local-hyperdb_amd/csrc/hdb_quant.hip

```cpp
#include "hdb_common.h"
#include "hdb_quant.h"
#include "hdb_finalize.h"
#include "../../include/hyperdb_hip.h"

__device__ __forceinline__ float hq_up(double x) {
    x = x * (1.0 + 0x1p-40);
    float f = (float)x;
    if ((double)f < x) f = nextafterf(f, INFINITY);
    return f;
}

__device__ __forceinline__ float hq_f(__half v) { return __half2float(v); }
__device__ __forceinline__ float hq_f(float v) { return v; }

template <typename T> struct HqElem;
template <> struct HqElem<__half> { static constexpr int EPC = 8; };
template <> struct HqElem<float> { static constexpr int EPC = 4; };

__device__ __forceinline__ void hq_unpack(const uint4& raw, float (&x)[8], __half*) {
    const __half2* h = reinterpret_cast<const __half2*>(&raw);
#pragma unroll
    for (int i = 0; i < 4; ++i) { float2 f = __half22float2(h[i]); x[2 * i] = f.x; x[2 * i + 1] = f.y; }
}
__device__ __forceinline__ void hq_unpack(const uint4& raw, float (&x)[4], float*) {
    x[0] = __uint_as_float(raw.x); x[1] = __uint_as_float(raw.y);
    x[2] = __uint_as_float(raw.z); x[3] = __uint_as_float(raw.w);
}

__device__ __forceinline__ int hq_code(double x, float s) {
    if (!(s > 0.f)) return 0;
    double c = rint(x / (double)s);
    c = c > 127.0 ? 127.0 : (c < -127.0 ? -127.0 : c);
    return (int)c;
}

template <typename T>
__global__ __launch_bounds__(256) void hdb_quant_rows_kernel(const T* V, int64_t n, int d, int P, int8_t* codes, float* aux,
                                                             int* nan_flag, double gamma) {
    const int lane = threadIdx.x & 63;
    const int64_t wave = ((int64_t)blockIdx.x * 256 + threadIdx.x) >> 6;
    const int64_t nwaves = ((int64_t)gridDim.x * 256) >> 6;
    for (int64_t r = wave; r < n; r += nwaves) {
        const T* row = V + r * (int64_t)d;
        float amax = 0.f;
        double ss = 0.0;
        bool has_nan = false, has_inf = false;
        for (int e = lane; e < d; e += 64) {
            const float x = hq_f(row[e]);
            if (x != x) has_nan = true;
            else if (x - x != 0.f) has_inf = true;
            amax = fmaxf(amax, fabsf(x));
            ss += (double)x * (double)x;
        }
#pragma unroll
        for (int o = 32; o > 0; o >>= 1) { amax = fmaxf(amax, __shfl_xor(amax, o, 64)); ss += __shfl_xor(ss, o, 64); }
        const bool nanr = __ballot(has_nan) != 0ull, infr = __ballot(has_inf) != 0ull;
        const bool bad = nanr || infr;
        const float s = bad ? 0.f : amax / 127.f;
        double ee = 0.0, cc = 0.0;
        for (int e = lane; e < P; e += 64) {
            int c = 0;
            if (e < d && !bad) {
                const double x = (double)hq_f(row[e]);
                c = hq_code(x, s);
                const double eps = x - (double)s * (double)c;
                ee += eps * eps;
                cc += (double)c * (double)c;
            }
            codes[r * (int64_t)P + e] = (int8_t)c;
        }
#pragma unroll
        for (int o = 32; o > 0; o >>= 1) { ee += __shfl_xor(ee, o, 64); cc += __shfl_xor(cc, o, 64); }
        if (lane == 0) {
            if (nanr) atomicOr(nan_flag, 1);
            else if (infr) atomicOr(nan_flag, 2);
            aux[3 * r + HDB_QROW_S] = s;
            aux[3 * r + HDB_QROW_E] = bad ? 0.f : hq_up(sqrt(ee) + gamma * sqrt(ss));
            aux[3 * r + HDB_QROW_T] = bad ? 0.f : hq_up((double)s * sqrt(cc));
        }
    }
}

__global__ __launch_bounds__(256) void hdb_quant_gather_kernel(const int8_t* codes, const float* aux, const int64_t* rows, int64_t m,
                                                               int P, int8_t* codes_out, float* aux_out) {
    const int lane = threadIdx.x & 63;
    const int64_t wave = ((int64_t)blockIdx.x * 256 + threadIdx.x) >> 6;
    const int64_t nwaves = ((int64_t)gridDim.x * 256) >> 6;
    for (int64_t j = wave; j < m; j += nwaves) {
        const int64_t r = rows[j];
        for (int c = lane * 16; c < P; c += 64 * 16)
            *reinterpret_cast<uint4*>(codes_out + j * (int64_t)P + c) = *reinterpret_cast<const uint4*>(codes + r * (int64_t)P + c);
        if (lane < 3) aux_out[3 * j + lane] = aux[3 * r + lane];
    }
}

__global__ __launch_bounds__(64) void hdb_quant_qprep_kernel(const float* Q, int nq, int d, int P, int8_t* qcodes, float* qaux, int* stat,
                                                             uint32_t* pl_cnt) {
    const int q = blockIdx.x, lane = threadIdx.x;
    if (q >= nq) return;
    if (q == 0 && lane == 0 && stat) stat[0] = 0;
    if (q == 0 && lane == 0 && pl_cnt) pl_cnt[0] = 0u;
    const float* qr = Q + (int64_t)q * d;
    float amax = 0.f;
    bool bad = false;
    for (int e = lane; e < d; e += 64) {
        const float x = qr[e];
        if (!(x - x == 0.f)) bad = true;
        amax = fmaxf(amax, fabsf(x));
    }
#pragma unroll
    for (int o = 32; o > 0; o >>= 1) amax = fmaxf(amax, __shfl_xor(amax, o, 64));
    bad = __ballot(bad) != 0ull;
    const float s = bad ? 0.f : amax / 127.f;
    double nn = 0.0, dd = 0.0;
    int cs = 0, c2 = 0;
    for (int e = lane; e < P; e += 64) {
        int c = 0;
        if (e < d && !bad) {
            const double x = (double)qr[e];
            c = hq_code(x, s);
            const double del = x - (double)s * (double)c;
            nn += x * x;
            dd += del * del;
        }
        qcodes[(int64_t)q * P + e] = (int8_t)c;
        cs += c; c2 += c * c;
    }
#pragma unroll
    for (int o = 32; o > 0; o >>= 1) {
        nn += __shfl_xor(nn, o, 64); dd += __shfl_xor(dd, o, 64);
        cs += __shfl_xor(cs, o, 64); c2 += __shfl_xor(c2, o, 64);
    }
    if (lane == 0) {
        float* o = qaux + (int64_t)q * HDB_QQ_WORDS;
        const float sq = (float)nn;
        const bool big = !(sq - sq == 0.f);
        o[HDB_QQ_S] = s;
        o[HDB_QQ_N] = bad ? 0.f : hq_up(sqrt(nn));
        o[HDB_QQ_D] = bad ? 0.f : hq_up(sqrt(dd));
        o[HDB_QQ_SQ] = sq;
        o[HDB_QQ_BAD] = (bad || big) ? 1.f : 0.f;
        o[HDB_QQ_CN] = hq_up(sqrt((double)c2));
        o[HDB_QQ_CS] = (float)cs;
        o[7] = 0.f;
    }
}

__global__ __launch_bounds__(64) void hdb_quant_qprep_m_kernel(const float* Q, int nq, int d, int P, float* qinv, float* qsq, int* qnan,
                                                               _Float16* q16, float* qscl, int8_t* qcodes, float* qaux, int* stat,
                                                               uint32_t* cnt_init, uint32_t* pl_cnt) {
    const int q = blockIdx.x, lane = threadIdx.x;
    if (q >= nq) return;
    if (q == 0 && lane == 0 && stat) stat[0] = 0;
    if (q == 0 && lane == 0 && pl_cnt) pl_cnt[0] = 0u;
    if (lane == 0 && cnt_init) cnt_init[q * HDB_CNT_STRIDE] = 0u;
    const float* qr = Q + (int64_t)q * d;
    float s = 0.f, amax = 0.f;
    bool bad = false;
    for (int e = lane; e < d; e += 64) {
        const float x = qr[e];
        s = fma(x, x, s);
        amax = fmaxf(amax, fabsf(x));
        if (!(x - x == 0.f)) bad = true;
    }
#pragma unroll
    for (int o = 32; o > 0; o >>= 1) amax = fmaxf(amax, __shfl_xor(amax, o, 64));
    const float scale = hdb_q16_scale(amax);
    const float inv_scale = 1.f / scale;
    float amax2 = 0.f;
    for (int e = lane; e < d; e += 64) {
        const _Float16 h = (_Float16)(qr[e] * scale);
        q16[(int64_t)q * d + e] = h;
        const float xr = (float)h * inv_scale;
        if (!(xr - xr == 0.f)) bad = true;
        amax2 = fmaxf(amax2, fabsf(xr));
    }
#pragma unroll
    for (int o = 32; o > 0; o >>= 1) { s += __shfl_xor(s, o, 64); amax2 = fmaxf(amax2, __shfl_xor(amax2, o, 64)); }
    bad = __ballot(bad) != 0ull;
    const float sq_ = bad ? 0.f : amax2 / 127.f;
    double nn = 0.0, dd = 0.0;
    int cs = 0, c2 = 0;
    for (int e = lane; e < P; e += 64) {
        int c = 0;
        if (e < d && !bad) {
            const double x = (double)((float)(_Float16)(qr[e] * scale) * inv_scale);
            c = hq_code(x, sq_);
            const double del = x - (double)sq_ * (double)c;
            nn += x * x;
            dd += del * del;
        }
        qcodes[(int64_t)q * P + e] = (int8_t)c;
        cs += c; c2 += c * c;
    }
#pragma unroll
    for (int o = 32; o > 0; o >>= 1) {
        nn += __shfl_xor(nn, o, 64); dd += __shfl_xor(dd, o, 64);
        cs += __shfl_xor(cs, o, 64); c2 += __shfl_xor(c2, o, 64);
    }
    if (lane == 0) {
        const float ss = s;
        qsq[q] = ss;
        qinv[q] = (s == 0.f) ? 1.0f : (float)(1.f / sqrt(s));
        qnan[q] = (ss != ss) ? 1 : (ss - ss != 0.f) ? 2 : 0;
        qscl[q] = inv_scale;
        float* o = qaux + (int64_t)q * HDB_QQ_WORDS;
        const float sq = (float)nn;
        const bool big = !(sq - sq == 0.f);
        o[HDB_QQ_S] = sq_;
        o[HDB_QQ_N] = bad ? 0.f : hq_up(sqrt(nn));
        o[HDB_QQ_D] = bad ? 0.f : hq_up(sqrt(dd));
        o[HDB_QQ_SQ] = sq;
        o[HDB_QQ_BAD] = (bad || big) ? 1.f : 0.f;
        o[HDB_QQ_CN] = hq_up(sqrt((double)c2));
        o[HDB_QQ_CS] = (float)cs;
        o[7] = 0.f;
    }
}

#define HQ_STAGE_CAP 128
struct HqStage {
    unsigned long long buf[4][HQ_STAGE_CAP];
    unsigned int cnt[4];
    unsigned int base;
};

__device__ __forceinline__ int hq_dpp_i(int x, int ctrl_id) {
    switch (ctrl_id) {
    case 0: return __builtin_amdgcn_update_dpp(0, x, HDB_DPP_MIRROR, 0xF, 0xF, false);
    case 1: return __builtin_amdgcn_update_dpp(0, x, HDB_DPP_HALF_MIRROR, 0xF, 0xF, false);
    case 2: return __builtin_amdgcn_update_dpp(0, x, HDB_DPP_XOR2, 0xF, 0xF, false);
    default: return __builtin_amdgcn_update_dpp(0, x, HDB_DPP_XOR1, 0xF, 0xF, false);
    }
}
__device__ __forceinline__ int hq_rows4_sum(int a0, int a1, int a2, int a3, int l16) {
    const bool b3 = (l16 & 8) != 0, b2 = (l16 & 4) != 0;
    const int v01 = (b3 ? a1 : a0) + hq_dpp_i(b3 ? a0 : a1, 0);
    const int v23 = (b3 ? a3 : a2) + hq_dpp_i(b3 ? a2 : a3, 0);
    int w = (b2 ? v23 : v01) + hq_dpp_i(b2 ? v01 : v23, 1);
    w += hq_dpp_i(w, 2);
    w += hq_dpp_i(w, 3);
    return w;
}

template <int NQ>
__device__ __forceinline__ void hq_fold_thr(const QuantArgs& a, float (&q_thr)[NQ]) {
    __shared__ uint32_t s_top[4 * 16];
    __shared__ float s_thr[NQ];
    const int ln = threadIdx.x & 63, wv = threadIdx.x >> 6;
    for (int q = 0; q < NQ; ++q) {
        uint32_t c[HDB_QUANT_NSUB_MAX / 256];
#pragma unroll
        for (int j = 0; j < HDB_QUANT_NSUB_MAX / 256; ++j) {
            const int e = (int)threadIdx.x + 256 * j;
            c[j] = e < a.nsub ? a.wmax[(int64_t)q * a.nsub + e] : 0u;
        }
        for (int r = 0; r < 16; ++r) {
            uint32_t lm = 0u;
#pragma unroll
            for (int j = 0; j < HDB_QUANT_NSUB_MAX / 256; ++j) lm = max(lm, c[j]);
            uint32_t wm = lm;
#pragma unroll
            for (int o = 32; o > 0; o >>= 1) wm = max(wm, (uint32_t)__shfl_xor((int)wm, o, 64));
            const unsigned long long who = __ballot(lm == wm);
            if (ln == (int)__ffsll((long long)who) - 1) {
                bool gone = false;
#pragma unroll
                for (int j = 0; j < HDB_QUANT_NSUB_MAX / 256; ++j)
                    if (!gone && c[j] == wm) { c[j] = 0u; gone = true; }
            }
            if (ln == 0) s_top[wv * 16 + r] = wm;
        }
        __syncthreads();
        if (wv == 0) {
            uint32_t v = s_top[ln];
            uint32_t kth = 0u;
            for (int r = 0; r < 16; ++r) {
                uint32_t wm = v;
#pragma unroll
                for (int o = 32; o > 0; o >>= 1) wm = max(wm, (uint32_t)__shfl_xor((int)wm, o, 64));
                const unsigned long long who = __ballot(v == wm);
                if (ln == (int)__ffsll((long long)who) - 1) v = 0u;
                kth = wm;
            }
            if (ln == 0) {
                const float t = kth == 0u ? -INFINITY : hdb_key2f(kth);
                s_thr[q] = t;
                if (blockIdx.x == 0) a.thr_out[q] = t;
            }
        }
        __syncthreads();
    }
#pragma unroll
    for (int q = 0; q < NQ; ++q) q_thr[q] = s_thr[q];
}

template <int MODE, int NQ, int NJ, bool LIST = false>
__global__ __launch_bounds__(256) void hdb_quant_scan_kernel(QuantArgs a) {
    extern __shared__ __attribute__((aligned(16))) char smem[];
    int4* qs = reinterpret_cast<int4*>(smem);
    __shared__ HqStage stage;
    const int nch = a.P >> 4;
    static_assert(!LIST || (MODE == 1 && NQ == 1), "the list flavour is pass 2 of a one-query call");
    if (MODE == 1 && threadIdx.x < 4) stage.cnt[threadIdx.x] = 0u;
    for (int i = threadIdx.x; i < NQ * nch; i += 256) qs[i] = reinterpret_cast<const int4*>(a.qcodes)[i];
    float q_s[NQ], q_n[NQ], q_d[NQ], q_sq[NQ], q_inv[NQ], q_thr[NQ];
    bool q_bad[NQ];
#pragma unroll
    for (int q = 0; q < NQ; ++q) {
        const float* o = a.qaux + (int64_t)q * HDB_QQ_WORDS;
        q_s[q] = o[HDB_QQ_S]; q_n[q] = o[HDB_QQ_N]; q_d[q] = o[HDB_QQ_D]; q_sq[q] = o[HDB_QQ_SQ]; q_bad[q] = o[HDB_QQ_BAD] != 0.f;
        q_inv[q] = a.metric == HDB_COSINE ? a.qinv[q] : 1.f;
        q_thr[q] = (MODE == 1 && a.nsub == 0) ? a.thr[q] : 0.f;
    }
    __syncthreads();
    if (MODE == 1 && a.nsub > 0) hq_fold_thr<NQ>(a, q_thr);

    const int lane = threadIdx.x & 63, wave = threadIdx.x >> 6;
    const int g = lane >> 4, l16 = lane & 15;
    const int nj = NJ > 0 ? NJ : (nch + 15) >> 4;
    constexpr int G = NJ > 0 ? NJ : 2;
    const float absmin = 0x1p-100f * (float)(a.d + 8);
    const float g2 = 2.f * a.gamma;
    typedef unsigned int u32x4 __attribute__((ext_vector_type(4)));
    uint32_t wbest[NQ];
#pragma unroll
    for (int q = 0; q < NQ; ++q) wbest[q] = 0u;

    int64_t ntiles = a.ntiles;
    uint32_t pl_n = 0u;
    bool pl_list = false;
    if (LIST) {
        pl_n = a.pl_cnt[0];
        pl_list = pl_n <= a.pl_cap;
        if (pl_list) ntiles = ((int64_t)pl_n + 15) >> 4;
        else if (blockIdx.x == 0 && threadIdx.x == 0) atomicAdd(&a.pl_cnt[1], 1u);
    }
    for (int64_t t = (int64_t)blockIdx.x * 4 + wave; t < ntiles; t += (int64_t)gridDim.x * 4) {
        const int64_t r0 = hdb_tile_index(t, a.tile_stride) * 16 + 4 * g;
        int64_t rr[4];
#pragma unroll
        for (int u = 0; u < 4; ++u) {
            rr[u] = r0 + u;
            if (LIST && pl_list) rr[u] = (uint64_t)(r0 + u) < (uint64_t)pl_n ? (int64_t)a.pl_list[r0 + u] : a.n;
        }
        const int8_t* p[4];
#pragma unroll
        for (int u = 0; u < 4; ++u) p[u] = a.codes + min(rr[u], a.n - 1) * (int64_t)a.P;
        int acc[4][NQ];
#pragma unroll
        for (int u = 0; u < 4; ++u)
#pragma unroll
            for (int q = 0; q < NQ; ++q) acc[u][q] = 0;
        for (int j0 = 0; j0 < nj; j0 += G) {
            uint4 raw[G][4];
#pragma unroll
            for (int j = 0; j < G; ++j) {
                const int c = l16 + 16 * (j0 + j);
                const bool live = (j0 + j) < nj && c < nch;
#pragma unroll
                for (int u = 0; u < 4; ++u) {
                    if (live) {
                        const u32x4 v = __builtin_nontemporal_load(reinterpret_cast<const u32x4*>(p[u] + (int64_t)c * 16));
                        raw[j][u] = make_uint4(v.x, v.y, v.z, v.w);
                    } else {
                        raw[j][u] = make_uint4(0u, 0u, 0u, 0u);
                    }
                }
            }
            __builtin_amdgcn_sched_barrier(0);
#pragma unroll
            for (int j = 0; j < G; ++j) {
                const int c = l16 + 16 * (j0 + j);
                const int cc = c < nch ? c : 0;
#pragma unroll
                for (int q = 0; q < NQ; ++q) {
                    const int4 qv = qs[q * nch + cc];
#pragma unroll
                    for (int u = 0; u < 4; ++u) {
                        int s = acc[u][q];
                        s = __builtin_amdgcn_sdot4((int)raw[j][u].x, qv.x, s, false);
                        s = __builtin_amdgcn_sdot4((int)raw[j][u].y, qv.y, s, false);
                        s = __builtin_amdgcn_sdot4((int)raw[j][u].z, qv.z, s, false);
                        s = __builtin_amdgcn_sdot4((int)raw[j][u].w, qv.w, s, false);
                        acc[u][q] = s;
                    }
                }
            }
        }
        const int u_own = hdb_owned_row(l16);
        const int64_t row = LIST ? (u_own == 0 ? rr[0] : u_own == 1 ? rr[1] : u_own == 2 ? rr[2] : rr[3]) : r0 + u_own;
        int C[NQ];
#pragma unroll
        for (int q = 0; q < NQ; ++q) C[q] = hq_rows4_sum(acc[0][q], acc[1][q], acc[2][q], acc[3][q], l16);
        if ((l16 & 3) != 0) continue;
        const int64_t out_i = t * 16 + 4 * g + u_own;
        if (row >= a.n) {
            if (MODE == 0 && a.nsub == 0)
#pragma unroll
                for (int q = 0; q < NQ; ++q) a.scores[(int64_t)q * a.ld + out_i] = -INFINITY;
            continue;
        }
        const float s_r = a.aux[3 * row + HDB_QROW_S], e_r = a.aux[3 * row + HDB_QROW_E], t_r = a.aux[3 * row + HDB_QROW_T];
        const bool masked = a.mask && !a.mask[row];
        const float bias = a.bias ? a.bias[row] : 0.f;
        const float invn = a.metric == HDB_COSINE ? a.inv_norm[row] : 1.f;
        const float sqv = a.metric == HDB_EUCLIDEAN ? a.sqnorm[row] : 0.f;
#pragma unroll
        for (int q = 0; q < NQ; ++q) {
            float lo = -INFINITY, hi = -INFINITY;
            if (!q_bad[q] && !masked) {
                const float A = (q_s[q] * s_r) * (float)C[q];
                const float aA = fabsf(A);
                const float B = (q_n[q] * e_r + q_d[q] * t_r) * (1.f + 0x1p-10f) + aA * 0x1p-10f + absmin;
                if (a.metric == HDB_EUCLIDEAN) {
                    const float ctr = sqv + q_sq[q] - 2.f * A;
                    const float err = g2 * sqv + 2.f * B + 0x1p-10f * (sqv + q_sq[q] + 2.f * aA) + absmin;
                    const float elo = fmaxf(ctr - err, 0.f) * (1.f - g2 - 0x1p-10f);
                    const float ehi = (ctr + err) * (1.f + g2 + 0x1p-10f);
                    hi = (float)(1.f / (1.f + sqrt(elo)));
                    lo = (float)(1.f / (1.f + sqrt(ehi)));
                } else {
                    lo = A - B; hi = A + B;
                    if (a.metric == HDB_COSINE) { lo = lo * invn * q_inv[q]; hi = hi * invn * q_inv[q]; }
                }
                if (a.bias) { lo += bias; hi += bias; }
                lo = lo - fabsf(lo) * 0x1p-20f - 1e-30f;
                hi = hi + fabsf(hi) * 0x1p-20f + 1e-30f;
                if (lo != lo) lo = -INFINITY;
                if (hi != hi) hi = INFINITY;
            }
            if (MODE == 2) {
                a.dbg[row] = hi;
            } else if (MODE == 0) {
                if (a.nsub > 0) wbest[q] = max(wbest[q], hdb_f2key(lo));
                else a.scores[(int64_t)q * a.ld + out_i] = lo;
            } else if (!masked && !q_bad[q] && hi >= q_thr[q]) {
                const unsigned long long ent = hdb_pack(hi, (uint32_t)row);
                const unsigned int lp = atomicAdd(&stage.cnt[q], 1u);
                if (lp < HQ_STAGE_CAP) stage.buf[q][lp] = ent;
                else {
                    const uint32_t pos = atomicAdd(&a.cnt[q * HDB_CNT_STRIDE], 1u);
                    if (pos < a.cap) a.cand[(int64_t)q * a.cap + pos] = ent;
                }
            }
        }
    }
    if (MODE == 0 && a.nsub > 0) {
#pragma unroll
        for (int q = 0; q < NQ; ++q) {
            uint32_t wm = wbest[q];
#pragma unroll
            for (int o = 32; o > 0; o >>= 1) wm = max(wm, (uint32_t)__shfl_xor((int)wm, o, 64));
            if (lane == 0) a.wmax[(int64_t)q * a.nsub + blockIdx.x * 4 + wave] = wm;
        }
    }
    if (MODE == 1) {
        __syncthreads();
        for (int q = 0; q < NQ; ++q) {
            const unsigned int have = min(stage.cnt[q], (unsigned int)HQ_STAGE_CAP);
            if (have == 0u) continue;
            if (threadIdx.x == 0) stage.base = atomicAdd(&a.cnt[q * HDB_CNT_STRIDE], have);
            __syncthreads();
            const unsigned int base = stage.base;
            for (unsigned int e = threadIdx.x; e < have; e += blockDim.x)
                if (base + e < a.cap) a.cand[(int64_t)q * a.cap + base + e] = stage.buf[q][e];
            __syncthreads();
        }
    }
}

__global__ __launch_bounds__(256) void hdb_quant_plane_rows_kernel(const int8_t* codes, const float* aux, int64_t row0, int64_t m, int d, int P,
                                                                   int U, uint8_t* nib, uint32_t* bitw, float* rec) {
    const int lane = threadIdx.x & 63, g = lane >> 4, l16 = lane & 15;
    const int64_t wave = ((int64_t)blockIdx.x * 256 + threadIdx.x) >> 6;
    const int64_t nwaves = ((int64_t)gridDim.x * 256) >> 6;
    for (int64_t base = wave * 4; base < m; base += nwaves * 4) {
        const int64_t r = row0 + base + g;
        const bool valid = base + g < m;
        int ss = 0;
        if (valid && l16 < U) {
            const int8_t* src = codes + r * (int64_t)P + 32 * l16;
            uint4 raw[2];
            raw[0] = *reinterpret_cast<const uint4*>(src);
            raw[1] = (32 * l16 + 16 < P) ? *reinterpret_cast<const uint4*>(src + 16) : make_uint4(0u, 0u, 0u, 0u);
            const uint32_t* cw = reinterpret_cast<const uint32_t*>(raw);
            uint32_t nw[4] = {0u, 0u, 0u, 0u}, bw = 0u;
#pragma unroll
            for (int w = 0; w < 8; ++w) {
#pragma unroll
                for (int b = 0; b < 4; ++b) {
                    const int c = (int)(int8_t)((cw[w] >> (8 * b)) & 0xFFu);
                    const int h = c >> 3;
                    const uint32_t u5 = (uint32_t)(h + 16);
                    const int rho = c - (8 * h + 4);
                    if (32 * l16 + 4 * w + b < d) ss += rho * rho;
                    nw[w >> 1] |= (u5 >> 1) << (8 * b + 4 * (w & 1));
                    bw |= (u5 & 1u) << (8 * b + w);
                }
            }
            *reinterpret_cast<uint4*>(nib + (r * (int64_t)U + l16) * 16) = make_uint4(nw[0], nw[1], nw[2], nw[3]);
            bitw[r * (int64_t)U + l16] = bw;
        }
#pragma unroll
        for (int o = 8; o > 0; o >>= 1) ss += __shfl_xor(ss, o, 64);
        if (valid && l16 == 0) {
            const float R = sqrtf((float)ss) * (1.f + 0x1p-20f);
            *reinterpret_cast<float4*>(rec + 4 * r) = make_float4(aux[3 * r + HDB_QROW_S], aux[3 * r + HDB_QROW_E], aux[3 * r + HDB_QROW_T], R);
        }
    }
}

#define HQ_PL_STAGE 1024
template <int J, bool DBG>
__global__ __launch_bounds__(256) void hdb_quant_plane_scan_kernel(QuantArgs a) {
    extern __shared__ __attribute__((aligned(16))) char smem[];
    int4* qs = reinterpret_cast<int4*>(smem);
    __shared__ int part[4][2][64 * J];
    __shared__ uint32_t st_buf[HQ_PL_STAGE];
    __shared__ uint32_t st_cnt, st_base;
    const int U = a.pl_units, nch = a.P >> 4;
    if (threadIdx.x == 0) st_cnt = 0u;
    for (int i = threadIdx.x; i < 2 * U; i += 256) qs[i] = i < nch ? reinterpret_cast<const int4*>(a.qcodes)[i] : make_int4(0, 0, 0, 0);
    const float* qo = a.qaux;
    const float q_s = qo[HDB_QQ_S], q_n = qo[HDB_QQ_N], q_d = qo[HDB_QQ_D], q_cn = qo[HDB_QQ_CN];
    const int q_cs = (int)qo[HDB_QQ_CS];
    const bool q_bad = qo[HDB_QQ_BAD] != 0.f;
    const bool cosine = a.metric == HDB_COSINE;
    const float q_inv = cosine ? a.qinv[0] : 1.f;
    float thr1[1] = {(!DBG && a.nsub == 0) ? a.thr[0] : 0.f};
    __syncthreads();
    if (!DBG && a.nsub > 0) hq_fold_thr<1>(a, thr1);
    const float q_thr = thr1[0];

    const int lane = threadIdx.x & 63, wave = threadIdx.x >> 6;
    const int npieces = 16 * U;
    int qw[J][8];
    int prow[J];
#pragma unroll
    for (int j = 0; j < J; ++j) {
        const int f = lane + 64 * j;
        const int unit = f < npieces ? f % U : 0;
        prow[j] = f < npieces ? f / U : 16;
        const int4 x = qs[2 * unit], y = qs[2 * unit + 1];
        qw[j][0] = x.x; qw[j][1] = x.y; qw[j][2] = x.z; qw[j][3] = x.w;
        qw[j][4] = y.x; qw[j][5] = y.y; qw[j][6] = y.z; qw[j][7] = y.w;
    }
    const float absmin = 0x1p-100f * (float)(a.d + 8);
    typedef unsigned int u32x4 __attribute__((ext_vector_type(4)));
    typedef float f32x4 __attribute__((ext_vector_type(4)));
    const int64_t ntiles = a.ntiles;
    const int et = lane >> 4, er = lane & 15;

    for (int64_t t = ((int64_t)blockIdx.x * 4 + wave) * 2; t < ntiles; t += (int64_t)gridDim.x * 8) {
        u32x4 nv[2][J];
        uint32_t bv[2][J];
#pragma unroll
        for (int tt = 0; tt < 2; ++tt) {
            const int64_t rows_left = a.n - (t + tt) * 16;
            const uint8_t* nb = a.pl_nib + (t + tt) * (int64_t)npieces * 16;
            const uint32_t* bb = a.pl_bit + (t + tt) * (int64_t)npieces;
#pragma unroll
            for (int j = 0; j < J; ++j) {
                const int f = lane + 64 * j;
                if ((int64_t)prow[j] < rows_left && prow[j] < 16) {
                    nv[tt][j] = __builtin_nontemporal_load(reinterpret_cast<const u32x4*>(nb + (int64_t)f * 16));
                    bv[tt][j] = __builtin_nontemporal_load(bb + f);
                } else {
                    nv[tt][j] = u32x4{0u, 0u, 0u, 0u};
                    bv[tt][j] = 0u;
                }
            }
        }
        const int64_t row = (t + et) * 16 + er;
        const bool rvalid = lane < 32 && t + et < ntiles && row < a.n;
        f32x4 rc = f32x4{0.f, 0.f, 0.f, 0.f};
        float invn = 1.f, bias = 0.f;
        bool masked = false;
        if (rvalid) {
            rc = __builtin_nontemporal_load(reinterpret_cast<const f32x4*>(a.pl_rec) + row);
            if (cosine) invn = a.inv_norm[row];
            if (a.bias) bias = a.bias[row];
            if (a.mask) masked = !a.mask[row];
        }
        __builtin_amdgcn_sched_barrier(0);
#pragma unroll
        for (int tt = 0; tt < 2; ++tt) {
#pragma unroll
            for (int j = 0; j < J; ++j) {
                const uint32_t bw = bv[tt][j];
                const uint32_t w4[4] = {nv[tt][j].x, nv[tt][j].y, nv[tt][j].z, nv[tt][j].w};
                int s = 0;
#pragma unroll
                for (int i = 0; i < 4; ++i) {
                    const uint32_t lo = ((w4[i] << 1) & 0x1E1E1E1Eu) | ((bw >> (2 * i)) & 0x01010101u);
                    const uint32_t hi = ((w4[i] >> 3) & 0x1E1E1E1Eu) | ((bw >> (2 * i + 1)) & 0x01010101u);
                    s = __builtin_amdgcn_sdot4((int)lo, qw[j][2 * i], s, false);
                    s = __builtin_amdgcn_sdot4((int)hi, qw[j][2 * i + 1], s, false);
                }
                part[wave][tt][lane + 64 * j] = s;
            }
        }
        __builtin_amdgcn_fence(__ATOMIC_RELEASE, "wavefront");
        __builtin_amdgcn_wave_barrier();
        __builtin_amdgcn_fence(__ATOMIC_ACQUIRE, "wavefront");
        int S = 0;
        if (lane < 32)
            for (int i = 0; i < U; ++i) S += part[wave][et][er * U + i];
        __builtin_amdgcn_fence(__ATOMIC_RELEASE, "wavefront");
        __builtin_amdgcn_wave_barrier();
        if (!rvalid) continue;
        float hi5 = -INFINITY;
        const bool dead = masked || q_bad;
        if (!dead) {
            const float fc = (float)(8 * S - 124 * q_cs);
            const float Uf = q_cn * rc.w;
            float ch = fc + Uf, cl = fc - Uf;
            ch = ch + (fabsf(ch) * 0x1p-20f + 1.f);
            cl = cl - (fabsf(cl) * 0x1p-20f + 1.f);
            const float k = q_s * rc.x;
            const float A5 = k * ch, Al = k * cl;
            const float Amax = fmaxf(fabsf(A5), fabsf(Al));
            const float c0 = (q_n * rc.y + q_d * rc.z) * (1.f + 0x1p-10f);
            const float B5 = c0 + fabsf(A5) * 0x1p-10f + absmin;
            const float Bmax = c0 + Amax * 0x1p-10f + absmin;
            const float Mx = Amax + Bmax;
            float X = (A5 + B5) + (Mx * 0x1p-18f + 1e-30f);
            float mM = Mx * (1.f + 0x1p-17f);
            if (cosine) { X = X * invn * q_inv; mM = mM * invn * q_inv; }
            const float Z = mM + fabsf(bias);
            float h = X;
            if (a.bias) h += bias;
            hi5 = h + (Z * 0x1p-18f + 4e-30f);
            if (hi5 != hi5) hi5 = INFINITY;
        }
        if (DBG) {
            a.dbg[row] = hi5;
        } else if (!dead && !(hi5 < q_thr)) {
            const unsigned int lp = atomicAdd(&st_cnt, 1u);
            if (lp < HQ_PL_STAGE) st_buf[lp] = (uint32_t)row;
            else {
                const uint32_t pos = atomicAdd(&a.pl_cnt[0], 1u);
                if (pos < a.pl_cap) a.pl_list[pos] = (uint32_t)row;
            }
        }
    }
    if (!DBG) {
        __syncthreads();
        const unsigned int have = min(st_cnt, (unsigned int)HQ_PL_STAGE);
        if (have != 0u) {
            if (threadIdx.x == 0) st_base = atomicAdd(&a.pl_cnt[0], have);
            __syncthreads();
            const unsigned int base = st_base;
            for (unsigned int e = threadIdx.x; e < have; e += blockDim.x)
                if (base + e < a.pl_cap) a.pl_list[base + e] = st_buf[e];
        }
    }
}

struct RescoreArgs {
    const void* V; int32_t d; int32_t row_bytes; int32_t nchunks;
    const float* Q;
    int32_t metric;
    const float* inv_norm; const float* qinv; const float* bias; const uint8_t* mask;
    unsigned long long* cand; const uint32_t* cnt; uint32_t cap;
};

template <typename T, int ACC, bool VEC>
__global__ __launch_bounds__(256) void hdb_quant_rescore_kernel(RescoreArgs a) {
    using Acc = float;
    constexpr int EPC = HqElem<T>::EPC;
    const int q = blockIdx.y;
    const int lane = threadIdx.x & 63, wave = threadIdx.x >> 6;
    const int g = lane >> 4, l16 = lane & 15;
    const uint32_t total = min(a.cnt[q * HDB_CNT_STRIDE], a.cap);
    const float* qv = a.Q + (int64_t)q * a.d;
    const char* Vb = reinterpret_cast<const char*>(a.V);
    const T* Vt = reinterpret_cast<const T*>(a.V);
    for (uint32_t base = ((uint32_t)blockIdx.x * 4 + wave) * 4; base < total; base += gridDim.x * 16) {
        const uint32_t i = base + g;
        const bool valid = i < total;
        const unsigned long long ent = valid ? a.cand[(int64_t)q * a.cap + i] : 0ull;
        const uint32_t row = valid ? 0xFFFFFFFFu - (uint32_t)(ent & 0xFFFFFFFFull) : 0u;
        Acc acc = Acc(0);
        if constexpr (VEC) {
            const char* pr = Vb + (int64_t)row * a.row_bytes;
            const int nj = (a.nchunks + 15) >> 4;
            for (int j = 0; j < nj; ++j) {
                const int c = l16 + 16 * j;
                const bool live = c < a.nchunks;
                const int cc = live ? c : a.nchunks - 1;
                const uint4 raw = *reinterpret_cast<const uint4*>(pr + (int64_t)cc * 16);
                Acc x[EPC];
                hq_unpack(raw, x, (T*)nullptr);
#pragma unroll
                for (int e = 0; e < EPC; ++e) {
                    const Acc qe = qv[cc * EPC + e];
                    if (ACC == 1) {
                        const Acc df = live ? x[e] - qe : Acc(0);
                        acc += df * df;
                    } else {
                        acc += (live ? x[e] : Acc(0)) * qe;
                    }
                }
            }
        } else {
            for (int e = l16; e < a.d; e += 16) {
                const Acc qe = qv[e];
                const Acc x = (Acc)hq_f(Vt[(int64_t)row * a.d + e]);
                if (ACC == 1) { const Acc df = x - qe; acc += df * df; }
                else acc += x * qe;
            }
        }
        const Acc sum = hdb_rows4_sum(acc, acc, acc, acc, l16);
        if (valid && (l16 & 3) == 0 && hdb_owned_row(l16) == (int)(row & 3u)) {
            float s;
            if (a.metric == HDB_EUCLIDEAN) {
                s = (float)(Acc(1) / (Acc(1) + sqrt(sum)));
            } else if (a.metric == HDB_COSINE) {
                s = (float)sum * a.inv_norm[row] * a.qinv[q];
            } else {
                s = (float)sum;
            }
            if (a.bias) s += a.bias[row];
            const bool masked = a.mask && !a.mask[row];
            if (masked) s = -INFINITY;
            s = hdb_canon(s);
            a.cand[(int64_t)q * a.cap + i] = hdb_pack(s, row);
        }
    }
}

__global__ __launch_bounds__(256) void hdb_quant_cgather_kernel(const char* V, int row_bytes, const float* inv_norm, const float* bias,
                                                                const uint8_t* mask, const unsigned long long* cand, const uint32_t* cnt,
                                                                uint32_t cap, char* G, float* ginv, float* gbias) {
    const int q = blockIdx.y, lane = threadIdx.x & 63, wave = threadIdx.x >> 6;
    const uint32_t total = min(cnt[q * HDB_CNT_STRIDE], cap);
    for (uint32_t i = blockIdx.x * 4 + wave; i < total; i += gridDim.x * 4) {
        const int64_t slot = (int64_t)q * cap + i;
        const uint32_t row = 0xFFFFFFFFu - (uint32_t)(cand[slot] & 0xFFFFFFFFull);
        const char* src = V + (int64_t)row * row_bytes;
        char* dst = G + slot * row_bytes;
        for (int c = lane * 16; c < row_bytes; c += 64 * 16) *reinterpret_cast<uint4*>(dst + c) = *reinterpret_cast<const uint4*>(src + c);
        if (lane == 0) {
            if (ginv) ginv[slot] = inv_norm[row];
            if (gbias) gbias[slot] = mask ? (mask[row] ? (bias ? bias[row] : 0.f) : -INFINITY) : bias[row];
        }
    }
}

__global__ __launch_bounds__(1024) void hdb_quant_finalize_kernel(const unsigned long long* cand, const uint32_t* cnt, uint32_t cap, uint32_t k,
                                                                  uint32_t kk, int64_t row_base, int64_t* idx_out, float* score_out,
                                                                  int32_t* status, const int* qnan, const float* qaux, const float* thr,
                                                                  int* stat, unsigned long long* cand_rw, const float* sc, int64_t ld) {
    extern __shared__ __attribute__((aligned(16))) unsigned long long buf[];
    const int q = blockIdx.x;
    const uint32_t total = cnt[q * HDB_CNT_STRIDE];
    if (sc) {
        const uint32_t nc = min(total, cap);
        for (uint32_t i = threadIdx.x; i < nc; i += blockDim.x) {
            const int64_t slot = (int64_t)q * cap + i;
            const uint32_t row = 0xFFFFFFFFu - (uint32_t)(cand_rw[slot] & 0xFFFFFFFFull);
            cand_rw[slot] = hdb_pack(sc[(int64_t)q * ld + slot], row);
        }
        __threadfence_block();
        __syncthreads();
    }
    if (threadIdx.x == 0 && stat) atomicMax(stat, (int)min(total, 0x7FFFFFFFu));
    const int qn = qnan[q];
    const bool bad = qaux[(int64_t)q * HDB_QQ_WORDS + HDB_QQ_BAD] != 0.f;
    hdb_finalize_fast(buf, cand + (int64_t)q * cap, total, q, cap, k, kk, row_base, idx_out, score_out, status,
                      qn & 1, ((qn & 2) || bad) ? (int32_t)HDB_Q_UNDERFLOW : 0, thr + q, 1.f);
}

extern "C" int hdb_launch_quant_rows(const void* V, int64_t n, int d, int dtype, int P, int8_t* codes, float* aux, int* nan_flag,
                                     double gamma, void* stream) {
    if (n <= 0) return 0;
    hipStream_t st = (hipStream_t)stream;
    const int blocks = hdb_grid_for(n, 4, 8192);
    if (dtype == HDB_F16) hipLaunchKernelGGL(hdb_quant_rows_kernel<__half>, dim3(blocks), dim3(256), 0, st, (const __half*)V, n, d, P, codes, aux, nan_flag, gamma);
    else hipLaunchKernelGGL(hdb_quant_rows_kernel<float>, dim3(blocks), dim3(256), 0, st, (const float*)V, n, d, P, codes, aux, nan_flag, gamma);
    return (int)hipGetLastError();
}

extern "C" int hdb_launch_quant_gather(const int8_t* codes, const float* aux, const int64_t* rows, int64_t m, int P, int8_t* codes_out,
                                       float* aux_out, void* stream) {
    if (m <= 0) return 0;
    hipLaunchKernelGGL(hdb_quant_gather_kernel, dim3(hdb_grid_for(m, 4, 8192)), dim3(256), 0, (hipStream_t)stream, codes, aux, rows, m, P,
                       codes_out, aux_out);
    return (int)hipGetLastError();
}

extern "C" int hdb_launch_quant_qprep(const float* Q, int nq, int d, int P, int8_t* qcodes, float* qaux, int* stat, uint32_t* pl_cnt,
                                      void* stream) {
    hipLaunchKernelGGL(hdb_quant_qprep_kernel, dim3(nq), dim3(64), 0, (hipStream_t)stream, Q, nq, d, P, qcodes, qaux, stat, pl_cnt);
    return (int)hipGetLastError();
}

extern "C" int hdb_launch_quant_qprep_m(const float* Q, int nq, int d, int P, float* qinv, float* qsq, int* qnan, void* q16, float* qscl,
                                        int8_t* qcodes, float* qaux, int* stat, uint32_t* cnt_init, uint32_t* pl_cnt, void* stream) {
    hipLaunchKernelGGL(hdb_quant_qprep_m_kernel, dim3(nq), dim3(64), 0, (hipStream_t)stream, Q, nq, d, P, qinv, qsq, qnan, (_Float16*)q16,
                       qscl, qcodes, qaux, stat, cnt_init, pl_cnt);
    return (int)hipGetLastError();
}

extern "C" int hdb_launch_quant_cgather(const void* V, int row_bytes, const float* inv_norm, const float* bias, const uint8_t* mask,
                                        const unsigned long long* cand, const uint32_t* cnt, uint32_t cap, int nq, void* G, float* ginv,
                                        float* gbias, void* stream) {
    if (row_bytes % 16 != 0 || (reinterpret_cast<uintptr_t>(V) & 15) != 0) return (int)hipErrorInvalidValue;
    hipLaunchKernelGGL(hdb_quant_cgather_kernel, dim3(256, nq), dim3(256), 0, (hipStream_t)stream, (const char*)V, row_bytes, inv_norm, bias,
                       mask, cand, cnt, cap, (char*)G, ginv, gbias);
    return (int)hipGetLastError();
}

template <int MODE, int NQ>
static void hq_launch_scan_nq(const QuantArgs& a, int blocks, size_t lds, hipStream_t st) {
    const int nch = a.P >> 4;
    const int nj = (nch + 15) >> 4;
    if (nj == 1) hipLaunchKernelGGL((hdb_quant_scan_kernel<MODE, NQ, 1>), dim3(blocks), dim3(256), lds, st, a);
    else if (nj == 2) hipLaunchKernelGGL((hdb_quant_scan_kernel<MODE, NQ, 2>), dim3(blocks), dim3(256), lds, st, a);
    else if (nj == 3) hipLaunchKernelGGL((hdb_quant_scan_kernel<MODE, NQ, 3>), dim3(blocks), dim3(256), lds, st, a);
    else hipLaunchKernelGGL((hdb_quant_scan_kernel<MODE, NQ, 0>), dim3(blocks), dim3(256), lds, st, a);
}
template <int MODE>
static void hq_launch_scan_mode(const QuantArgs& a, int blocks, size_t lds, hipStream_t st) {
    switch (a.nq) {
    case 1: hq_launch_scan_nq<MODE, 1>(a, blocks, lds, st); break;
    case 2: hq_launch_scan_nq<MODE, 2>(a, blocks, lds, st); break;
    case 3: hq_launch_scan_nq<MODE, 3>(a, blocks, lds, st); break;
    default: hq_launch_scan_nq<MODE, 4>(a, blocks, lds, st); break;
    }
}
extern "C" int hdb_launch_quant_scan(const QuantArgs* args, int mode, int max_blocks, void* stream) {
    const QuantArgs& a = *args;
    if (a.nq < 1 || a.nq > 4 || (a.P & 15) != 0) return (int)hipErrorInvalidValue;
    const size_t lds = (size_t)a.nq * a.P;
    const int blocks = hdb_quant_scan_blocks(a.ntiles, max_blocks);
    if (a.nsub != 0 && (a.nsub > HDB_QUANT_NSUB_MAX || !a.wmax || (mode == 0 ? a.nsub != 4 * blocks : !a.thr_out))) return (int)hipErrorInvalidValue;
    if (mode == 0) hq_launch_scan_mode<0>(a, blocks, lds, (hipStream_t)stream);
    else hq_launch_scan_mode<1>(a, blocks, lds, (hipStream_t)stream);
    return (int)hipGetLastError();
}

extern "C" int hdb_launch_quant_plane_rows(const int8_t* codes, const float* aux, int64_t row0, int64_t m, int d, int P, uint8_t* nib,
                                           uint32_t* bitw, float* rec, void* stream) {
    if (m <= 0) return 0;
    const int U = hdb_quant_plane_units(P);
    if (U > 16 || (P & 15) != 0) return (int)hipErrorInvalidValue;
    hipLaunchKernelGGL(hdb_quant_plane_rows_kernel, dim3(hdb_grid_for(m, 16, 8192)), dim3(256), 0, (hipStream_t)stream, codes, aux, row0, m, d,
                       P, U, nib, bitw, rec);
    return (int)hipGetLastError();
}
extern "C" int hdb_launch_quant_plane_scan(const QuantArgs* args, int dbg, int max_blocks, void* stream) {
    const QuantArgs& a = *args;
    const int U = a.pl_units;
    if (a.nq != 1 || U < 1 || U > 16 || U != hdb_quant_plane_units(a.P) || (a.metric != HDB_DOT && a.metric != HDB_COSINE)) return (int)hipErrorInvalidValue;
    if (!dbg && a.nsub != 0 && (a.nsub > HDB_QUANT_NSUB_MAX || !a.wmax || !a.thr_out)) return (int)hipErrorInvalidValue;
    const size_t lds = (size_t)U * 32;
    const int blocks = hdb_grid_for((a.ntiles + 1) / 2, 4, max_blocks > 0 ? max_blocks : 1024);
    hipStream_t st = (hipStream_t)stream;
    const int J = (U + 3) / 4;
#define HQ_PLANE(J_) do { if (dbg) hipLaunchKernelGGL((hdb_quant_plane_scan_kernel<J_, true>), dim3(blocks), dim3(256), lds, st, a); \
                          else hipLaunchKernelGGL((hdb_quant_plane_scan_kernel<J_, false>), dim3(blocks), dim3(256), lds, st, a); } while (0)
    if (J == 1) HQ_PLANE(1); else if (J == 2) HQ_PLANE(2); else if (J == 3) HQ_PLANE(3); else HQ_PLANE(4);
#undef HQ_PLANE
    return (int)hipGetLastError();
}
extern "C" int hdb_launch_quant_scan_one(const QuantArgs* args, int mode, int max_blocks, void* stream) {
    const QuantArgs& a = *args;
    if (a.nq != 1 || (a.P & 15) != 0 || a.nsub != 0 || (mode != 1 && mode != 2)) return (int)hipErrorInvalidValue;
    const size_t lds = (size_t)a.P;
    const int blocks = hdb_quant_scan_blocks(a.ntiles, max_blocks);
    const int nj = ((a.P >> 4) + 15) >> 4;
    hipStream_t st = (hipStream_t)stream;
#define HQ_ONE(NJ_) do { if (mode == 1) hipLaunchKernelGGL((hdb_quant_scan_kernel<1, 1, NJ_, true>), dim3(blocks), dim3(256), lds, st, a); \
                         else hipLaunchKernelGGL((hdb_quant_scan_kernel<2, 1, NJ_, false>), dim3(blocks), dim3(256), lds, st, a); } while (0)
    if (nj == 1) HQ_ONE(1); else if (nj == 2) HQ_ONE(2); else if (nj == 3) HQ_ONE(3); else HQ_ONE(0);
#undef HQ_ONE
    return (int)hipGetLastError();
}

extern "C" int hdb_launch_quant_rescore(const void* V, int d, int dtype, const float* Q, int nq, int metric, const float* inv_norm,
                                        const float* qinv, const float* bias, const uint8_t* mask, unsigned long long* cand,
                                        const uint32_t* cnt, uint32_t cap, void* stream) {
    hipStream_t st = (hipStream_t)stream;
    RescoreArgs a;
    a.V = V; a.d = d; a.Q = Q; a.metric = metric; a.inv_norm = inv_norm; a.qinv = qinv; a.bias = bias; a.mask = mask;
    a.cand = cand; a.cnt = cnt; a.cap = cap;
    const int elem = hdb_elem_bytes(dtype);
    a.row_bytes = d * elem;
    a.nchunks = a.row_bytes / 16;
    const bool vec = (a.row_bytes % 16 == 0) && ((reinterpret_cast<uintptr_t>(V) & 15) == 0) && ((size_t)d * 4 <= 60 * 1024);
    const bool euc = metric == HDB_EUCLIDEAN;
    const dim3 grid((cap + 15) / 16 < 128 ? (cap + 15) / 16 : 128, nq);
#define HQ_RESCORE(T_, ACC_, VEC_) hipLaunchKernelGGL((hdb_quant_rescore_kernel<T_, ACC_, VEC_>), grid, dim3(256), 0, st, a)
    if (dtype == HDB_F16) {
        if (vec) { if (euc) HQ_RESCORE(__half, 1, true); else HQ_RESCORE(__half, 0, true); }
        else { if (euc) HQ_RESCORE(__half, 1, false); else HQ_RESCORE(__half, 0, false); }
    } else {
        if (vec) { if (euc) HQ_RESCORE(float, 1, true); else HQ_RESCORE(float, 0, true); }
        else { if (euc) HQ_RESCORE(float, 1, false); else HQ_RESCORE(float, 0, false); }
    }
#undef HQ_RESCORE
    return (int)hipGetLastError();
}

extern "C" int hdb_launch_quant_finalize(const unsigned long long* cand, const uint32_t* cnt, uint32_t cap, int nq, uint32_t k, uint32_t kk,
                                         int64_t row_base, int64_t* idx_out, float* score_out, int32_t* status, const int* qnan,
                                         const float* qaux, const float* thr, int* stat, unsigned long long* cand_rw, const float* sc,
                                         int64_t ld, void* stream) {
    const size_t lds = (size_t)cap * 16 + 2048 * 4 + 64;
    static unsigned long long attr_done = 0;
    hipError_t e = hdb_lds_attr_once(reinterpret_cast<const void*>(hdb_quant_finalize_kernel), (int)lds, &attr_done);
    if (e != hipSuccess) return (int)e;
    hipLaunchKernelGGL(hdb_quant_finalize_kernel, dim3(nq), dim3(1024), lds, (hipStream_t)stream, cand, cnt, cap, k, kk, row_base,
                       idx_out, score_out, status, qnan, qaux, thr, stat, cand_rw, sc, ld);
    return (int)hipGetLastError();
}
```

Measured before the change: 1834 queries/s.

## Fuse plane survivor rescoring and candidate row gather into the plane scan

The 5-bit plane scan no longer writes a survivor list for a second int8 scan kernel. Surviving rows are queued per wave, their int8 bounds are evaluated in the same kernel, and candidates are emitted directly. The candidate fp16 rows are also copied into the gather buffer at emission time, which removes the separate cgather kernel. This saves two kernel launches and the round trip through the survivor list on the single-query path. In exchange the plane kernel is more complex, uses more registers, and does scattered row copies inside the scan.

```diff
diff --git a/local-hyperdb_amd/csrc/hdb_api.hip b/local-hyperdb_amd/csrc/hdb_api.hip
--- a/local-hyperdb_amd/csrc/hdb_api.hip
+++ b/local-hyperdb_amd/csrc/hdb_api.hip
@@ -738,10 +738,10 @@
     const uint32_t m = 16;
     const QuantSample sp = p.qs;
     QuantWs w;
-    int rc = quant_ws_lay(ix, w, nq, (nq == 1 && ix->pnib) ? p.pl_cap : 0, mflavour);
+    int rc = quant_ws_lay(ix, w, nq, 0, mflavour);
     if (rc) return rc;
-    const uint32_t pl_cap = p.pl_cap;
-    uint32_t* pl_cnt = use_pl ? reinterpret_cast<uint32_t*>(ix->qstat) + 1 : nullptr;
+    uint32_t* qstat = reinterpret_cast<uint32_t*>(ix->qstat);
+    uint32_t* pl_cnt = use_pl ? qstat + 1 : nullptr;
     const size_t crow = (size_t)nq * HDB_CAND_CAP;
     const int nsub = p.nsub;
     rc = quant_query_prep(ix, (const float*)dev_Q, nq, w, mflavour, ix->qstat, nsub ? w.cnt : nullptr, pl_cnt, st);
@@ -753,21 +753,21 @@
     if (!nsub) LAUNCH_TRY(hdb_launch_sample_thr(w.sbuf, sp.s_rows, sp.ld_s, nq, m, w.thr, w.cnt, nullptr, st));
     a.ntiles = (n + 15) / 16; a.tile_stride = 1; a.scores = nullptr; a.ld = 0;
     a.thr = w.thr; a.cnt = w.cnt; a.cand = w.cand; a.cap = HDB_CAND_CAP;
+    const bool has_bias = ix->bias != nullptr || ix->mask != nullptr;
+    if (mflavour) {
+        a.V = (const char*)ix->V; a.row_bytes = ix->d * 2; a.G = w.G;
+        a.ginv = metric == HDB_COSINE ? w.ginv : nullptr; a.gbias = has_bias ? w.gbias : nullptr;
+    }
     prof_begin(ix, st);
     if (use_pl) {
         a.pl_nib = ix->pnib; a.pl_bit = ix->pbit; a.pl_rec = ix->prec; a.pl_units = ix->pU;
-        a.pl_list = w.pl_list; a.pl_cnt = pl_cnt; a.pl_cap = pl_cap;
+        a.pl_cnt = pl_cnt; a.pl_cap = p.pl_cap;
         LAUNCH_TRY(hdb_launch_quant_plane_scan(&a, 0, (int)ix->opt.max_blocks, st));
-        a.nsub = 0; a.wmax = nullptr;
-        LAUNCH_TRY(hdb_launch_quant_scan_one(&a, 1, (int)ix->opt.max_blocks, st));
     } else {
         LAUNCH_TRY(hdb_launch_quant_scan(&a, 1, (int)ix->opt.max_blocks, st));
     }
     prof_end(ix, st);
     if (mflavour) {
-        const bool has_bias = ix->bias != nullptr || ix->mask != nullptr;
-        LAUNCH_TRY(hdb_launch_quant_cgather(ix->V, ix->d * 2, ix->inv_norm, ix->bias, ix->mask, w.cand, w.cnt, HDB_CAND_CAP, nq, w.G,
-                                            metric == HDB_COSINE ? w.ginv : nullptr, has_bias ? w.gbias : nullptr, st));
         ScanArgs s; memset(&s, 0, sizeof(s));
         s.V = w.G; s.n = (int64_t)crow; s.d = ix->d; s.Q = dev_Q; s.metric = metric; s.inv_norm = w.ginv; s.qinv = w.qinv;
         s.bias = has_bias ? w.gbias : nullptr; s.mask = nullptr; s.nq = nq;
@@ -790,7 +790,7 @@
     HIP_TRY(hipSetDevice(ix->device));
     hipStream_t st = (hipStream_t)stream;
     QuantWs w;
-    int rc = quant_ws_lay(ix, w, 1, plane_list_cap(ix->opt, ix->n), true);
+    int rc = quant_ws_lay(ix, w, 1, 0, true);
     if (rc) return rc;
     rc = quant_query_prep(ix, dev_q, 1, w, ix->qauto, nullptr, nullptr, nullptr, st);
     if (rc) return rc;
diff --git a/local-hyperdb_amd/csrc/hdb_launch.h b/local-hyperdb_amd/csrc/hdb_launch.h
--- a/local-hyperdb_amd/csrc/hdb_launch.h
+++ b/local-hyperdb_amd/csrc/hdb_launch.h
@@ -108,9 +108,6 @@
 int hdb_launch_quant_rescore(const void* V, int d, int dtype, const float* Q, int nq, int metric, const float* inv_norm,
                              const float* qinv, const float* bias, const uint8_t* mask, unsigned long long* cand,
                              const uint32_t* cnt, uint32_t cap, void* stream);
-int hdb_launch_quant_cgather(const void* V, int row_bytes, const float* inv_norm, const float* bias, const uint8_t* mask,
-                             const unsigned long long* cand, const uint32_t* cnt, uint32_t cap, int nq, void* G, float* ginv, float* gbias,
-                             void* stream);
 int hdb_launch_quant_finalize(const unsigned long long* cand, const uint32_t* cnt, uint32_t cap, int nq, uint32_t k, uint32_t kk,
                               int64_t row_base, int64_t* idx_out, float* score_out, int32_t* status, const int* qnan,
                               const float* qaux, const float* thr, int* stat, unsigned long long* cand_rw, const float* sc, int64_t ld,
diff --git a/local-hyperdb_amd/csrc/hdb_quant.h b/local-hyperdb_amd/csrc/hdb_quant.h
--- a/local-hyperdb_amd/csrc/hdb_quant.h
+++ b/local-hyperdb_amd/csrc/hdb_quant.h
@@ -34,8 +34,9 @@
     float* scores; int64_t ld;
     const float* thr; uint32_t* cnt; unsigned long long* cand; uint32_t cap;
     uint32_t* wmax; int32_t nsub; float* thr_out;
+    const char* V; int32_t row_bytes; char* G; float* ginv; float* gbias;
     const uint8_t* pl_nib; const uint32_t* pl_bit; const float* pl_rec; int32_t pl_units;
-    uint32_t* pl_list; uint32_t* pl_cnt; uint32_t pl_cap;
+    uint32_t* pl_cnt; uint32_t pl_cap;
     float* dbg;
 };
 #define HDB_QUANT_NSUB_MAX 4096
diff --git a/local-hyperdb_amd/csrc/hdb_quant.hip b/local-hyperdb_amd/csrc/hdb_quant.hip
--- a/local-hyperdb_amd/csrc/hdb_quant.hip
+++ b/local-hyperdb_amd/csrc/hdb_quant.hip
@@ -295,156 +295,210 @@
     for (int q = 0; q < NQ; ++q) q_thr[q] = s_thr[q];
 }
 
-template <int MODE, int NQ, int NJ, bool LIST = false>
+template <int NQ>
+struct HqQuery {
+    float s[NQ], n[NQ], d[NQ], sq[NQ], inv[NQ];
+    bool bad[NQ];
+};
+template <int NQ>
+__device__ __forceinline__ void hq_query_load(const QuantArgs& a, HqQuery<NQ>& qc) {
+#pragma unroll
+    for (int q = 0; q < NQ; ++q) {
+        const float* o = a.qaux + (int64_t)q * HDB_QQ_WORDS;
+        qc.s[q] = o[HDB_QQ_S]; qc.n[q] = o[HDB_QQ_N]; qc.d[q] = o[HDB_QQ_D]; qc.sq[q] = o[HDB_QQ_SQ]; qc.bad[q] = o[HDB_QQ_BAD] != 0.f;
+        qc.inv[q] = a.metric == HDB_COSINE ? a.qinv[q] : 1.f;
+    }
+}
+
+template <int NQ, int NJ, int G, typename Sink>
+__device__ __forceinline__ bool hq_rows4_bounds(const QuantArgs& a, const int4* qs, const HqQuery<NQ>& qc, const int64_t (&rr)[4], int l16,
+                                                int64_t row, Sink&& sink) {
+    typedef unsigned int u32x4 __attribute__((ext_vector_type(4)));
+    const int nch = a.P >> 4;
+    const int nj = NJ > 0 ? NJ : (nch + 15) >> 4;
+    const int8_t* p[4];
+#pragma unroll
+    for (int u = 0; u < 4; ++u) p[u] = a.codes + min(rr[u], a.n - 1) * (int64_t)a.P;
+    int acc[4][NQ];
+#pragma unroll
+    for (int u = 0; u < 4; ++u)
+#pragma unroll
+        for (int q = 0; q < NQ; ++q) acc[u][q] = 0;
+    for (int j0 = 0; j0 < nj; j0 += G) {
+        uint4 raw[G][4];
+#pragma unroll
+        for (int j = 0; j < G; ++j) {
+            const int c = l16 + 16 * (j0 + j);
+            const bool live = (j0 + j) < nj && c < nch;
+#pragma unroll
+            for (int u = 0; u < 4; ++u) {
+                if (live) {
+                    const u32x4 v = __builtin_nontemporal_load(reinterpret_cast<const u32x4*>(p[u] + (int64_t)c * 16));
+                    raw[j][u] = make_uint4(v.x, v.y, v.z, v.w);
+                } else {
+                    raw[j][u] = make_uint4(0u, 0u, 0u, 0u);
+                }
+            }
+        }
+        __builtin_amdgcn_sched_barrier(0);
+#pragma unroll
+        for (int j = 0; j < G; ++j) {
+            const int c = l16 + 16 * (j0 + j);
+            const int cc = c < nch ? c : 0;
+#pragma unroll
+            for (int q = 0; q < NQ; ++q) {
+                const int4 qv = qs[q * nch + cc];
+#pragma unroll
+                for (int u = 0; u < 4; ++u) {
+                    int s = acc[u][q];
+                    s = __builtin_amdgcn_sdot4((int)raw[j][u].x, qv.x, s, false);
+                    s = __builtin_amdgcn_sdot4((int)raw[j][u].y, qv.y, s, false);
+                    s = __builtin_amdgcn_sdot4((int)raw[j][u].z, qv.z, s, false);
+                    s = __builtin_amdgcn_sdot4((int)raw[j][u].w, qv.w, s, false);
+                    acc[u][q] = s;
+                }
+            }
+        }
+    }
+    int C[NQ];
+#pragma unroll
+    for (int q = 0; q < NQ; ++q) C[q] = hq_rows4_sum(acc[0][q], acc[1][q], acc[2][q], acc[3][q], l16);
+    if ((l16 & 3) != 0 || row >= a.n) return false;
+    const float s_r = a.aux[3 * row + HDB_QROW_S], e_r = a.aux[3 * row + HDB_QROW_E], t_r = a.aux[3 * row + HDB_QROW_T];
+    const bool masked = a.mask && !a.mask[row];
+    const float bias = a.bias ? a.bias[row] : 0.f;
+    const float invn = a.metric == HDB_COSINE ? a.inv_norm[row] : 1.f;
+    const float sqv = a.metric == HDB_EUCLIDEAN ? a.sqnorm[row] : 0.f;
+    {
+#pragma clang fp contract(off)
+        const float absmin = 0x1p-100f * (float)(a.d + 8);
+        const float g2 = 2.f * a.gamma;
+#pragma unroll
+        for (int q = 0; q < NQ; ++q) {
+            float lo = -INFINITY, hi = -INFINITY;
+            if (!qc.bad[q] && !masked) {
+                const float A = (qc.s[q] * s_r) * (float)C[q];
+                const float aA = fabsf(A);
+                const float B = (qc.n[q] * e_r + qc.d[q] * t_r) * (1.f + 0x1p-10f) + aA * 0x1p-10f + absmin;
+                float l, h;
+                if (a.metric == HDB_EUCLIDEAN) {
+                    const float ctr = sqv + qc.sq[q] - 2.f * A;
+                    const float err = g2 * sqv + 2.f * B + 0x1p-10f * (sqv + qc.sq[q] + 2.f * aA) + absmin;
+                    const float elo = fmaxf(ctr - err, 0.f) * (1.f - g2 - 0x1p-10f);
+                    const float ehi = (ctr + err) * (1.f + g2 + 0x1p-10f);
+                    h = (float)(1.f / (1.f + sqrt(elo)));
+                    l = (float)(1.f / (1.f + sqrt(ehi)));
+                } else {
+                    l = A - B; h = A + B;
+                    if (a.metric == HDB_COSINE) { l = l * invn * qc.inv[q]; h = h * invn * qc.inv[q]; }
+                }
+                if (a.bias) { l += bias; h += bias; }
+                l = l - fabsf(l) * 0x1p-20f - 1e-30f;
+                h = h + fabsf(h) * 0x1p-20f + 1e-30f;
+                if (l != l) l = -INFINITY;
+                if (h != h) h = INFINITY;
+                lo = l; hi = h;
+            }
+            sink(q, lo, hi, masked);
+        }
+    }
+    return true;
+}
+
+__device__ __forceinline__ const QuantArgs& hq_args_in_memory() {
+    typedef const __attribute__((address_space(4))) QuantArgs* ArgPtr;
+    const uint64_t v = (uint64_t)__builtin_amdgcn_kernarg_segment_ptr();
+    uint32_t lo = (uint32_t)v, hi = (uint32_t)(v >> 32);
+    asm volatile("" : "+v"(lo), "+v"(hi));
+    lo = (uint32_t)__builtin_amdgcn_readfirstlane((int)lo); hi = (uint32_t)__builtin_amdgcn_readfirstlane((int)hi);
+    return *(const QuantArgs*)(ArgPtr)(((uint64_t)hi << 32) | lo);
+}
+
+__device__ __forceinline__ void hq_copy_row(const QuantArgs& a, int64_t slot, uint32_t row, int l, int nl) {
+    const char* src = a.V + (int64_t)row * a.row_bytes;
+    char* dst = a.G + slot * a.row_bytes;
+    for (int c = l * 16; c < a.row_bytes; c += nl * 16) *reinterpret_cast<uint4*>(dst + c) = *reinterpret_cast<const uint4*>(src + c);
+    if (l == 0) {
+        if (a.ginv) a.ginv[slot] = a.inv_norm[row];
+        if (a.gbias) a.gbias[slot] = a.mask ? (a.mask[row] ? (a.bias ? a.bias[row] : 0.f) : -INFINITY) : a.bias[row];
+    }
+}
+__device__ __forceinline__ void hq_emit(HqStage& stage, int q, float hi, int64_t row) {
+    const unsigned long long ent = hdb_pack(hi, (uint32_t)row);
+    const unsigned int lp = atomicAdd(&stage.cnt[q], 1u);
+    if (lp < HQ_STAGE_CAP) stage.buf[q][lp] = ent;
+    else {
+        const QuantArgs& a = hq_args_in_memory();
+        const uint32_t pos = atomicAdd(&a.cnt[q * HDB_CNT_STRIDE], 1u);
+        if (pos < a.cap) {
+            a.cand[(int64_t)q * a.cap + pos] = ent;
+            if (a.G) hq_copy_row(a, (int64_t)q * a.cap + pos, (uint32_t)row, 0, 1);
+        }
+    }
+}
+template <int NQ>
+__device__ __forceinline__ void hq_stage_flush(HqStage& stage) {
+    __syncthreads();
+    const QuantArgs& a = hq_args_in_memory();
+    for (int q = 0; q < NQ; ++q) {
+        const unsigned int have = min(stage.cnt[q], (unsigned int)HQ_STAGE_CAP);
+        if (have == 0u) continue;
+        if (threadIdx.x == 0) stage.base = atomicAdd(&a.cnt[q * HDB_CNT_STRIDE], have);
+        __syncthreads();
+        const unsigned int base = stage.base;
+        for (unsigned int e = threadIdx.x; e < have; e += blockDim.x)
+            if (base + e < a.cap) a.cand[(int64_t)q * a.cap + base + e] = stage.buf[q][e];
+        if (a.G)
+            for (unsigned int e = threadIdx.x >> 6; e < have; e += blockDim.x >> 6)
+                if (base + e < a.cap)
+                    hq_copy_row(a, (int64_t)q * a.cap + base + e, 0xFFFFFFFFu - (uint32_t)(stage.buf[q][e] & 0xFFFFFFFFull), threadIdx.x & 63, 64);
+        __syncthreads();
+    }
+}
+
+template <int MODE, int NQ, int NJ>
 __global__ __launch_bounds__(256) void hdb_quant_scan_kernel(QuantArgs a) {
+    static_assert(sizeof(QuantArgs) % 8 == 0, "the argument block is read back from the kernarg segment as laid out here");
     extern __shared__ __attribute__((aligned(16))) char smem[];
     int4* qs = reinterpret_cast<int4*>(smem);
     __shared__ HqStage stage;
     const int nch = a.P >> 4;
-    static_assert(!LIST || (MODE == 1 && NQ == 1), "the list flavour is pass 2 of a one-query call");
     if (MODE == 1 && threadIdx.x < 4) stage.cnt[threadIdx.x] = 0u;
     for (int i = threadIdx.x; i < NQ * nch; i += 256) qs[i] = reinterpret_cast<const int4*>(a.qcodes)[i];
-    float q_s[NQ], q_n[NQ], q_d[NQ], q_sq[NQ], q_inv[NQ], q_thr[NQ];
-    bool q_bad[NQ];
-#pragma unroll
-    for (int q = 0; q < NQ; ++q) {
-        const float* o = a.qaux + (int64_t)q * HDB_QQ_WORDS;
-        q_s[q] = o[HDB_QQ_S]; q_n[q] = o[HDB_QQ_N]; q_d[q] = o[HDB_QQ_D]; q_sq[q] = o[HDB_QQ_SQ]; q_bad[q] = o[HDB_QQ_BAD] != 0.f;
-        q_inv[q] = a.metric == HDB_COSINE ? a.qinv[q] : 1.f;
-        q_thr[q] = (MODE == 1 && a.nsub == 0) ? a.thr[q] : 0.f;
-    }
+    HqQuery<NQ> qc;
+    hq_query_load<NQ>(a, qc);
+    float q_thr[NQ];
+#pragma unroll
+    for (int q = 0; q < NQ; ++q) q_thr[q] = (MODE == 1 && a.nsub == 0) ? a.thr[q] : 0.f;
     __syncthreads();
     if (MODE == 1 && a.nsub > 0) hq_fold_thr<NQ>(a, q_thr);
 
     const int lane = threadIdx.x & 63, wave = threadIdx.x >> 6;
     const int g = lane >> 4, l16 = lane & 15;
-    const int nj = NJ > 0 ? NJ : (nch + 15) >> 4;
-    constexpr int G = NJ > 0 ? NJ : 2;
-    const float absmin = 0x1p-100f * (float)(a.d + 8);
-    const float g2 = 2.f * a.gamma;
-    typedef unsigned int u32x4 __attribute__((ext_vector_type(4)));
     uint32_t wbest[NQ];
 #pragma unroll
     for (int q = 0; q < NQ; ++q) wbest[q] = 0u;
 
-    int64_t ntiles = a.ntiles;
-    uint32_t pl_n = 0u;
-    bool pl_list = false;
-    if (LIST) {
-        pl_n = a.pl_cnt[0];
-        pl_list = pl_n <= a.pl_cap;
-        if (pl_list) ntiles = ((int64_t)pl_n + 15) >> 4;
-        else if (blockIdx.x == 0 && threadIdx.x == 0) atomicAdd(&a.pl_cnt[1], 1u);
-    }
+    const int64_t ntiles = a.ntiles;
     for (int64_t t = (int64_t)blockIdx.x * 4 + wave; t < ntiles; t += (int64_t)gridDim.x * 4) {
         const int64_t r0 = hdb_tile_index(t, a.tile_stride) * 16 + 4 * g;
-        int64_t rr[4];
-#pragma unroll
-        for (int u = 0; u < 4; ++u) {
-            rr[u] = r0 + u;
-            if (LIST && pl_list) rr[u] = (uint64_t)(r0 + u) < (uint64_t)pl_n ? (int64_t)a.pl_list[r0 + u] : a.n;
-        }
-        const int8_t* p[4];
-#pragma unroll
-        for (int u = 0; u < 4; ++u) p[u] = a.codes + min(rr[u], a.n - 1) * (int64_t)a.P;
-        int acc[4][NQ];
-#pragma unroll
-        for (int u = 0; u < 4; ++u)
-#pragma unroll
-            for (int q = 0; q < NQ; ++q) acc[u][q] = 0;
-        for (int j0 = 0; j0 < nj; j0 += G) {
-            uint4 raw[G][4];
-#pragma unroll
-            for (int j = 0; j < G; ++j) {
-                const int c = l16 + 16 * (j0 + j);
-                const bool live = (j0 + j) < nj && c < nch;
-#pragma unroll
-                for (int u = 0; u < 4; ++u) {
-                    if (live) {
-                        const u32x4 v = __builtin_nontemporal_load(reinterpret_cast<const u32x4*>(p[u] + (int64_t)c * 16));
-                        raw[j][u] = make_uint4(v.x, v.y, v.z, v.w);
-                    } else {
-                        raw[j][u] = make_uint4(0u, 0u, 0u, 0u);
-                    }
-                }
-            }
-            __builtin_amdgcn_sched_barrier(0);
-#pragma unroll
-            for (int j = 0; j < G; ++j) {
-                const int c = l16 + 16 * (j0 + j);
-                const int cc = c < nch ? c : 0;
-#pragma unroll
-                for (int q = 0; q < NQ; ++q) {
-                    const int4 qv = qs[q * nch + cc];
-#pragma unroll
-                    for (int u = 0; u < 4; ++u) {
-                        int s = acc[u][q];
-                        s = __builtin_amdgcn_sdot4((int)raw[j][u].x, qv.x, s, false);
-                        s = __builtin_amdgcn_sdot4((int)raw[j][u].y, qv.y, s, false);
-                        s = __builtin_amdgcn_sdot4((int)raw[j][u].z, qv.z, s, false);
-                        s = __builtin_amdgcn_sdot4((int)raw[j][u].w, qv.w, s, false);
-                        acc[u][q] = s;
-                    }
-                }
-            }
-        }
+        const int64_t rr[4] = {r0, r0 + 1, r0 + 2, r0 + 3};
         const int u_own = hdb_owned_row(l16);
-        const int64_t row = LIST ? (u_own == 0 ? rr[0] : u_own == 1 ? rr[1] : u_own == 2 ? rr[2] : rr[3]) : r0 + u_own;
-        int C[NQ];
-#pragma unroll
-        for (int q = 0; q < NQ; ++q) C[q] = hq_rows4_sum(acc[0][q], acc[1][q], acc[2][q], acc[3][q], l16);
-        if ((l16 & 3) != 0) continue;
+        const int64_t row = r0 + u_own;
         const int64_t out_i = t * 16 + 4 * g + u_own;
-        if (row >= a.n) {
-            if (MODE == 0 && a.nsub == 0)
-#pragma unroll
-                for (int q = 0; q < NQ; ++q) a.scores[(int64_t)q * a.ld + out_i] = -INFINITY;
-            continue;
-        }
-        const float s_r = a.aux[3 * row + HDB_QROW_S], e_r = a.aux[3 * row + HDB_QROW_E], t_r = a.aux[3 * row + HDB_QROW_T];
-        const bool masked = a.mask && !a.mask[row];
-        const float bias = a.bias ? a.bias[row] : 0.f;
-        const float invn = a.metric == HDB_COSINE ? a.inv_norm[row] : 1.f;
-        const float sqv = a.metric == HDB_EUCLIDEAN ? a.sqnorm[row] : 0.f;
-#pragma unroll
-        for (int q = 0; q < NQ; ++q) {
-            float lo = -INFINITY, hi = -INFINITY;
-            if (!q_bad[q] && !masked) {
-                const float A = (q_s[q] * s_r) * (float)C[q];
-                const float aA = fabsf(A);
-                const float B = (q_n[q] * e_r + q_d[q] * t_r) * (1.f + 0x1p-10f) + aA * 0x1p-10f + absmin;
-                if (a.metric == HDB_EUCLIDEAN) {
-                    const float ctr = sqv + q_sq[q] - 2.f * A;
-                    const float err = g2 * sqv + 2.f * B + 0x1p-10f * (sqv + q_sq[q] + 2.f * aA) + absmin;
-                    const float elo = fmaxf(ctr - err, 0.f) * (1.f - g2 - 0x1p-10f);
-                    const float ehi = (ctr + err) * (1.f + g2 + 0x1p-10f);
-                    hi = (float)(1.f / (1.f + sqrt(elo)));
-                    lo = (float)(1.f / (1.f + sqrt(ehi)));
-                } else {
-                    lo = A - B; hi = A + B;
-                    if (a.metric == HDB_COSINE) { lo = lo * invn * q_inv[q]; hi = hi * invn * q_inv[q]; }
-                }
-                if (a.bias) { lo += bias; hi += bias; }
-                lo = lo - fabsf(lo) * 0x1p-20f - 1e-30f;
-                hi = hi + fabsf(hi) * 0x1p-20f + 1e-30f;
-                if (lo != lo) lo = -INFINITY;
-                if (hi != hi) hi = INFINITY;
-            }
+        const bool live = hq_rows4_bounds<NQ, NJ, (NJ > 0 ? NJ : 2)>(a, qs, qc, rr, l16, row, [&](int q, float lo, float hi, bool masked) {
             if (MODE == 2) {
                 a.dbg[row] = hi;
             } else if (MODE == 0) {
                 if (a.nsub > 0) wbest[q] = max(wbest[q], hdb_f2key(lo));
                 else a.scores[(int64_t)q * a.ld + out_i] = lo;
-            } else if (!masked && !q_bad[q] && hi >= q_thr[q]) {
-                const unsigned long long ent = hdb_pack(hi, (uint32_t)row);
-                const unsigned int lp = atomicAdd(&stage.cnt[q], 1u);
-                if (lp < HQ_STAGE_CAP) stage.buf[q][lp] = ent;
-                else {
-                    const uint32_t pos = atomicAdd(&a.cnt[q * HDB_CNT_STRIDE], 1u);
-                    if (pos < a.cap) a.cand[(int64_t)q * a.cap + pos] = ent;
-                }
-            }
-        }
+            } else if (!masked && !qc.bad[q] && hi >= q_thr[q]) {
+                hq_emit(stage, q, hi, row);
+            }
+        });
+        if (MODE == 0 && a.nsub == 0 && !live && (l16 & 3) == 0)
+#pragma unroll
+            for (int q = 0; q < NQ; ++q) a.scores[(int64_t)q * a.ld + out_i] = -INFINITY;
     }
     if (MODE == 0 && a.nsub > 0) {
 #pragma unroll
@@ -455,19 +509,7 @@
             if (lane == 0) a.wmax[(int64_t)q * a.nsub + blockIdx.x * 4 + wave] = wm;
         }
     }
-    if (MODE == 1) {
-        __syncthreads();
-        for (int q = 0; q < NQ; ++q) {
-            const unsigned int have = min(stage.cnt[q], (unsigned int)HQ_STAGE_CAP);
-            if (have == 0u) continue;
-            if (threadIdx.x == 0) stage.base = atomicAdd(&a.cnt[q * HDB_CNT_STRIDE], have);
-            __syncthreads();
-            const unsigned int base = stage.base;
-            for (unsigned int e = threadIdx.x; e < have; e += blockDim.x)
-                if (base + e < a.cap) a.cand[(int64_t)q * a.cap + base + e] = stage.buf[q][e];
-            __syncthreads();
-        }
-    }
+    if (MODE == 1) hq_stage_flush<NQ>(stage);
 }
 
 __global__ __launch_bounds__(256) void hdb_quant_plane_rows_kernel(const int8_t* codes, const float* aux, int64_t row0, int64_t m, int d, int P,
@@ -511,16 +553,18 @@
     }
 }
 
-#define HQ_PL_STAGE 1024
+#define HQ_PL_QUEUE 48
 template <int J, bool DBG>
-__global__ __launch_bounds__(256) void hdb_quant_plane_scan_kernel(QuantArgs a) {
+__global__ __launch_bounds__(256) __attribute__((amdgpu_num_sgpr(96))) void hdb_quant_plane_scan_kernel(QuantArgs a) {
     extern __shared__ __attribute__((aligned(16))) char smem[];
     int4* qs = reinterpret_cast<int4*>(smem);
     __shared__ int part[4][2][64 * J];
-    __shared__ uint32_t st_buf[HQ_PL_STAGE];
-    __shared__ uint32_t st_cnt, st_base;
+    __shared__ HqStage stage;
+    __shared__ uint32_t queue[4][HQ_PL_QUEUE];
+    __shared__ uint32_t surv_cnt;
     const int U = a.pl_units, nch = a.P >> 4;
-    if (threadIdx.x == 0) st_cnt = 0u;
+    if (threadIdx.x < 4) stage.cnt[threadIdx.x] = 0u;
+    if (threadIdx.x == 0) surv_cnt = 0u;
     for (int i = threadIdx.x; i < 2 * U; i += 256) qs[i] = i < nch ? reinterpret_cast<const int4*>(a.qcodes)[i] : make_int4(0, 0, 0, 0);
     const float* qo = a.qaux;
     const float q_s = qo[HDB_QQ_S], q_n = qo[HDB_QQ_N], q_d = qo[HDB_QQ_D], q_cn = qo[HDB_QQ_CN];
@@ -533,39 +577,59 @@
     if (!DBG && a.nsub > 0) hq_fold_thr<1>(a, thr1);
     const float q_thr = thr1[0];
 
-    const int lane = threadIdx.x & 63, wave = threadIdx.x >> 6;
+    const int lane = threadIdx.x & 63, wave = __builtin_amdgcn_readfirstlane(threadIdx.x >> 6);
     const int npieces = 16 * U;
     int qw[J][8];
-    int prow[J];
-#pragma unroll
-    for (int j = 0; j < J; ++j) {
-        const int f = lane + 64 * j;
-        const int unit = f < npieces ? f % U : 0;
-        prow[j] = f < npieces ? f / U : 16;
-        const int4 x = qs[2 * unit], y = qs[2 * unit + 1];
-        qw[j][0] = x.x; qw[j][1] = x.y; qw[j][2] = x.z; qw[j][3] = x.w;
-        qw[j][4] = y.x; qw[j][5] = y.y; qw[j][6] = y.z; qw[j][7] = y.w;
-    }
+    auto load_qw = [&]() {
+#pragma unroll
+        for (int j = 0; j < J; ++j) {
+            const int f = lane + 64 * j;
+            const int unit = f < npieces ? f % U : 0;
+            const int4 x = qs[2 * unit], y = qs[2 * unit + 1];
+            qw[j][0] = x.x; qw[j][1] = x.y; qw[j][2] = x.z; qw[j][3] = x.w;
+            qw[j][4] = y.x; qw[j][5] = y.y; qw[j][6] = y.z; qw[j][7] = y.w;
+        }
+    };
+    load_qw();
     const float absmin = 0x1p-100f * (float)(a.d + 8);
     typedef unsigned int u32x4 __attribute__((ext_vector_type(4)));
     typedef float f32x4 __attribute__((ext_vector_type(4)));
     const int64_t ntiles = a.ntiles;
     const int et = lane >> 4, er = lane & 15;
+    int qn = 0;
+    uint32_t nsurv = 0u;
+    auto drain = [&](int base, int m) {
+        const QuantArgs& a = hq_args_in_memory();
+        HqQuery<1> qc;
+        qc.s[0] = q_s; qc.n[0] = q_n; qc.d[0] = q_d; qc.sq[0] = 0.f; qc.inv[0] = q_inv; qc.bad[0] = q_bad;
+        int ln = lane;
+        asm volatile("" : "+v"(ln));
+        const int g = ln >> 4, l16 = ln & 15;
+        int64_t rr[4];
+#pragma unroll
+        for (int u = 0; u < 4; ++u) rr[u] = 4 * g + u < m ? (int64_t)queue[wave][base + 4 * g + u] : a.n;
+        const int own = 4 * g + hdb_owned_row(l16);
+        const int64_t row = own < m ? (int64_t)queue[wave][base + own] : a.n;
+        hq_rows4_bounds<1, 0, 1>(a, qs, qc, rr, l16, row, [&](int, float, float hi, bool masked) {
+            if (!masked && !q_bad && hi >= q_thr) hq_emit(stage, 0, hi, row);
+        });
+    };
 
     for (int64_t t = ((int64_t)blockIdx.x * 4 + wave) * 2; t < ntiles; t += (int64_t)gridDim.x * 8) {
         u32x4 nv[2][J];
         uint32_t bv[2][J];
+        int ln = lane;
+        asm volatile("" : "+v"(ln));
 #pragma unroll
         for (int tt = 0; tt < 2; ++tt) {
-            const int64_t rows_left = a.n - (t + tt) * 16;
+            const int pieces_left = (int)min((int64_t)16, max((int64_t)0, a.n - (t + tt) * 16)) * U;
             const uint8_t* nb = a.pl_nib + (t + tt) * (int64_t)npieces * 16;
             const uint32_t* bb = a.pl_bit + (t + tt) * (int64_t)npieces;
 #pragma unroll
             for (int j = 0; j < J; ++j) {
-                const int f = lane + 64 * j;
-                if ((int64_t)prow[j] < rows_left && prow[j] < 16) {
-                    nv[tt][j] = __builtin_nontemporal_load(reinterpret_cast<const u32x4*>(nb + (int64_t)f * 16));
-                    bv[tt][j] = __builtin_nontemporal_load(bb + f);
+                if (ln < pieces_left - 64 * j) {
+                    nv[tt][j] = __builtin_nontemporal_load(reinterpret_cast<const u32x4*>(nb + (uint32_t)ln * 16u) + 64 * j);
+                    bv[tt][j] = __builtin_nontemporal_load(bb + (uint32_t)ln + 64 * j);
                 } else {
                     nv[tt][j] = u32x4{0u, 0u, 0u, 0u};
                     bv[tt][j] = 0u;
@@ -609,9 +673,8 @@
             for (int i = 0; i < U; ++i) S += part[wave][et][er * U + i];
         __builtin_amdgcn_fence(__ATOMIC_RELEASE, "wavefront");
         __builtin_amdgcn_wave_barrier();
-        if (!rvalid) continue;
         float hi5 = -INFINITY;
-        const bool dead = masked || q_bad;
+        const bool dead = !rvalid || masked || q_bad;
         if (!dead) {
             const float fc = (float)(8 * S - 124 * q_cs);
             const float Uf = q_cn * rc.w;
@@ -635,25 +698,34 @@
             if (hi5 != hi5) hi5 = INFINITY;
         }
         if (DBG) {
-            a.dbg[row] = hi5;
-        } else if (!dead && !(hi5 < q_thr)) {
-            const unsigned int lp = atomicAdd(&st_cnt, 1u);
-            if (lp < HQ_PL_STAGE) st_buf[lp] = (uint32_t)row;
-            else {
-                const uint32_t pos = atomicAdd(&a.pl_cnt[0], 1u);
-                if (pos < a.pl_cap) a.pl_list[pos] = (uint32_t)row;
-            }
+            if (rvalid) a.dbg[row] = hi5;
+            continue;
+        }
+        const bool keep = !dead && !(hi5 < q_thr);
+        const unsigned long long km = __ballot(keep);
+        if (km == 0ull) continue;
+        if (keep) queue[wave][qn + __popcll(km & ((1ull << lane) - 1ull))] = (uint32_t)row;
+        const int nk = __popcll(km);
+        qn += nk; nsurv += (uint32_t)nk;
+        __builtin_amdgcn_fence(__ATOMIC_RELEASE, "wavefront");
+        __builtin_amdgcn_wave_barrier();
+        __builtin_amdgcn_fence(__ATOMIC_ACQUIRE, "wavefront");
+        if (qn >= 16) {
+            do { qn -= 16; drain(qn, 16); } while (qn >= 16);
+            __builtin_amdgcn_fence(__ATOMIC_RELEASE, "wavefront");
+            __builtin_amdgcn_wave_barrier();
+            asm volatile("" ::: "memory");
+            load_qw();
         }
     }
     if (!DBG) {
-        __syncthreads();
-        const unsigned int have = min(st_cnt, (unsigned int)HQ_PL_STAGE);
-        if (have != 0u) {
-            if (threadIdx.x == 0) st_base = atomicAdd(&a.pl_cnt[0], have);
-            __syncthreads();
-            const unsigned int base = st_base;
-            for (unsigned int e = threadIdx.x; e < have; e += blockDim.x)
-                if (base + e < a.pl_cap) a.pl_list[base + e] = st_buf[e];
+        if (qn > 0) drain(0, qn);
+        if (lane == 0 && nsurv != 0u) atomicAdd(&surv_cnt, nsurv);
+        hq_stage_flush<1>(stage);
+        if (threadIdx.x == 0 && surv_cnt != 0u) {
+            const QuantArgs& a = hq_args_in_memory();
+            const uint32_t before = atomicAdd(&a.pl_cnt[0], surv_cnt);
+            if (before <= a.pl_cap && before + surv_cnt > a.pl_cap) atomicAdd(&a.pl_cnt[1], 1u);
         }
     }
 }
@@ -731,24 +803,6 @@
     }
 }
 
-__global__ __launch_bounds__(256) void hdb_quant_cgather_kernel(const char* V, int row_bytes, const float* inv_norm, const float* bias,
-                                                                const uint8_t* mask, const unsigned long long* cand, const uint32_t* cnt,
-                                                                uint32_t cap, char* G, float* ginv, float* gbias) {
-    const int q = blockIdx.y, lane = threadIdx.x & 63, wave = threadIdx.x >> 6;
-    const uint32_t total = min(cnt[q * HDB_CNT_STRIDE], cap);
-    for (uint32_t i = blockIdx.x * 4 + wave; i < total; i += gridDim.x * 4) {
-        const int64_t slot = (int64_t)q * cap + i;
-        const uint32_t row = 0xFFFFFFFFu - (uint32_t)(cand[slot] & 0xFFFFFFFFull);
-        const char* src = V + (int64_t)row * row_bytes;
-        char* dst = G + slot * row_bytes;
-        for (int c = lane * 16; c < row_bytes; c += 64 * 16) *reinterpret_cast<uint4*>(dst + c) = *reinterpret_cast<const uint4*>(src + c);
-        if (lane == 0) {
-            if (ginv) ginv[slot] = inv_norm[row];
-            if (gbias) gbias[slot] = mask ? (mask[row] ? (bias ? bias[row] : 0.f) : -INFINITY) : bias[row];
-        }
-    }
-}
-
 __global__ __launch_bounds__(1024) void hdb_quant_finalize_kernel(const unsigned long long* cand, const uint32_t* cnt, uint32_t cap, uint32_t k,
                                                                   uint32_t kk, int64_t row_base, int64_t* idx_out, float* score_out,
                                                                   int32_t* status, const int* qnan, const float* qaux, const float* thr,
@@ -804,15 +858,6 @@
     return (int)hipGetLastError();
 }
 
-extern "C" int hdb_launch_quant_cgather(const void* V, int row_bytes, const float* inv_norm, const float* bias, const uint8_t* mask,
-                                        const unsigned long long* cand, const uint32_t* cnt, uint32_t cap, int nq, void* G, float* ginv,
-                                        float* gbias, void* stream) {
-    if (row_bytes % 16 != 0 || (reinterpret_cast<uintptr_t>(V) & 15) != 0) return (int)hipErrorInvalidValue;
-    hipLaunchKernelGGL(hdb_quant_cgather_kernel, dim3(256, nq), dim3(256), 0, (hipStream_t)stream, (const char*)V, row_bytes, inv_norm, bias,
-                       mask, cand, cnt, cap, (char*)G, ginv, gbias);
-    return (int)hipGetLastError();
-}
-
 template <int MODE, int NQ>
 static void hq_launch_scan_nq(const QuantArgs& a, int blocks, size_t lds, hipStream_t st) {
     const int nch = a.P >> 4;
@@ -831,6 +876,9 @@
     default: hq_launch_scan_nq<MODE, 4>(a, blocks, lds, st); break;
     }
 }
+static bool hq_copy_args_ok(const QuantArgs& a) {
+    return !a.G || (a.V && a.row_bytes > 0 && a.row_bytes % 16 == 0 && (reinterpret_cast<uintptr_t>(a.V) & 15) == 0 && (reinterpret_cast<uintptr_t>(a.G) & 15) == 0);
+}
 extern "C" int hdb_launch_quant_scan(const QuantArgs* args, int mode, int max_blocks, void* stream) {
     const QuantArgs& a = *args;
     if (a.nq < 1 || a.nq > 4 || (a.P & 15) != 0) return (int)hipErrorInvalidValue;
@@ -838,7 +886,10 @@
     const int blocks = hdb_quant_scan_blocks(a.ntiles, max_blocks);
     if (a.nsub != 0 && (a.nsub > HDB_QUANT_NSUB_MAX || !a.wmax || (mode == 0 ? a.nsub != 4 * blocks : !a.thr_out))) return (int)hipErrorInvalidValue;
     if (mode == 0) hq_launch_scan_mode<0>(a, blocks, lds, (hipStream_t)stream);
-    else hq_launch_scan_mode<1>(a, blocks, lds, (hipStream_t)stream);
+    else {
+        if (!hq_copy_args_ok(a)) return (int)hipErrorInvalidValue;
+        hq_launch_scan_mode<1>(a, blocks, lds, (hipStream_t)stream);
+    }
     return (int)hipGetLastError();
 }
 
@@ -856,6 +907,7 @@
     const int U = a.pl_units;
     if (a.nq != 1 || U < 1 || U > 16 || U != hdb_quant_plane_units(a.P) || (a.metric != HDB_DOT && a.metric != HDB_COSINE)) return (int)hipErrorInvalidValue;
     if (!dbg && a.nsub != 0 && (a.nsub > HDB_QUANT_NSUB_MAX || !a.wmax || !a.thr_out)) return (int)hipErrorInvalidValue;
+    if (!dbg && (!a.cnt || !a.cand || !a.pl_cnt || !hq_copy_args_ok(a))) return (int)hipErrorInvalidValue;
     const size_t lds = (size_t)U * 32;
     const int blocks = hdb_grid_for((a.ntiles + 1) / 2, 4, max_blocks > 0 ? max_blocks : 1024);
     hipStream_t st = (hipStream_t)stream;
@@ -868,13 +920,12 @@
 }
 extern "C" int hdb_launch_quant_scan_one(const QuantArgs* args, int mode, int max_blocks, void* stream) {
     const QuantArgs& a = *args;
-    if (a.nq != 1 || (a.P & 15) != 0 || a.nsub != 0 || (mode != 1 && mode != 2)) return (int)hipErrorInvalidValue;
+    if (a.nq != 1 || (a.P & 15) != 0 || a.nsub != 0 || mode != 2 || !a.dbg) return (int)hipErrorInvalidValue;
     const size_t lds = (size_t)a.P;
     const int blocks = hdb_quant_scan_blocks(a.ntiles, max_blocks);
     const int nj = ((a.P >> 4) + 15) >> 4;
     hipStream_t st = (hipStream_t)stream;
-#define HQ_ONE(NJ_) do { if (mode == 1) hipLaunchKernelGGL((hdb_quant_scan_kernel<1, 1, NJ_, true>), dim3(blocks), dim3(256), lds, st, a); \
-                         else hipLaunchKernelGGL((hdb_quant_scan_kernel<2, 1, NJ_, false>), dim3(blocks), dim3(256), lds, st, a); } while (0)
+#define HQ_ONE(NJ_) hipLaunchKernelGGL((hdb_quant_scan_kernel<2, 1, NJ_>), dim3(blocks), dim3(256), lds, st, a)
     if (nj == 1) HQ_ONE(1); else if (nj == 2) HQ_ONE(2); else if (nj == 3) HQ_ONE(3); else HQ_ONE(0);
 #undef HQ_ONE
     return (int)hipGetLastError();
```

Measured after the change: 1897 queries/s (median of 6 runs). +3.4%, better.
